# drscotthawley/flocoder

Measured on AMD Instinct MI355X. Metric: latent samples/sec (64-step Euler, SD-VAE 4x32x32), higher is better.
Workload: dtype f32; 1 GPU; flowers_sd.yaml shape: 64-step legacy Euler, batch 64 per GPU, latents 4x32x32, U-Net dim=32 dim_mults [1,2,4,8] n_classes=102, class-conditional, no CFG, ODE loop only (no VAE decode); global_batch=64, parallelism=sample-shard x1, weights broadcast once, plan_entries_per_forward=59, kernel_launches_per_forward=68, kernel_launches_per_euler_step=66, plan=exclusive device (cross-workgroup Block tails)

## Files before the change

### flocoder_amd/_binding.py

```python
from __future__ import annotations

import ctypes as C
import os
from typing import Optional

_HERE = os.path.dirname(os.path.abspath(__file__))
LIB_PATH = os.environ.get("FLOCODER_AMD_LIB") or os.path.join(_HERE, "_lib", "libflocoder_amd.so")

FC_OK, FC_E_ARG, FC_E_SHAPE, FC_E_ARCH, FC_E_HIP, FC_E_STATE = 0, -1, -2, -3, -4, -5
FC_METHOD_EULER, FC_METHOD_RK4 = 0, 1
FC_JACOBIAN_IDENTITY, FC_JACOBIAN_EXACT = 0, 1
FC_SDE_EULER_MARUYAMA, FC_SDE_HEUN = 0, 1
FC_LL_MAX_PROBES = 64
FC_PROBE_RADEMACHER, FC_PROBE_GAUSSIAN = 0, 1
FC_HIST_LDS_BINS = 8192
TILE_AUTO = -1
TILES = {"M128N32": 0, "M128N64": 1, "M64N32K2": 2, "M32N32K4": 3, "M64N64K2": 4, "M256N64": 5}


class fc_unet_config(C.Structure):
    _fields_ = [("dim", C.c_int), ("channels", C.c_int), ("n_levels", C.c_int), ("dim_mults", C.c_int * 8),
                ("groups", C.c_int), ("n_classes", C.c_int), ("mask_cond", C.c_int)]


_vp, _i, _f, _i64 = C.c_void_p, C.c_int, C.c_float, C.c_int64
_pi, _pf = C.POINTER(C.c_int), C.POINTER(C.c_float)

SIGNATURES = {
    "fc_abi_version": (_i, []),
    "fc_last_error": (C.c_char_p, []),
    "fc_check_device": (_i, [_i]),
    "fc_unet_create": (_i, [C.POINTER(fc_unet_config), _i, C.POINTER(_vp)]),
    "fc_unet_destroy": (None, [_vp]),
    "fc_unet_param_count": (_i, [_vp]),
    "fc_unet_param_info": (_i, [_vp, _i, C.POINTER(C.c_char_p), C.POINTER(_i64 * 4), C.POINTER(_i64)]),
    "fc_unet_param_numel": (_i64, [_vp]),
    "fc_unet_load_params": (_i, [_vp, _vp, _i64, _i, _vp]),
    "fc_unet_reserve": (_i, [_vp, _i, _i, _i]),
    "fc_unet_reserved": (_i, [_vp, _pi, _pi, _pi]),
    "fc_unet_forward": (_i, [_vp, _vp, _vp, _vp, _vp, _i, _vp, _i, _i, _i, _vp]),
    "fc_unet_integrate": (_i, [_vp, _i, _vp, _i, _i, _i, _pf, _i, _f, _f, _vp, _f, _vp, _i, _vp]),
    "fc_unet_integrate_rk45": (_i, [_vp, _vp, _i, _i, _i, C.c_double, C.c_double, C.c_double, C.c_double, _f, _vp, _f, _vp, _i, _pi, _vp]),
    "fc_unet_integrate_rk45_per_sample": (_i, [_vp, _vp, _i, _i, _i, C.c_double, C.c_double, C.c_double, C.c_double, _f, _vp, _f, _vp, _i,
                                              _pi, _vp]),
    "fc_unet_integrate_rk45_dense": (_i, [_vp, _i, _vp, _i, _i, _i, C.c_double, C.c_double, C.c_double, C.c_double, _f, _vp, _f, _vp, _i,
                                         C.POINTER(C.c_double), _i, _vp, _pi, _vp]),
    "fc_unet_chains": (_i, [_vp, _pi]),
    "fc_unet_plan_launches": (_i, [_vp]),
    "fc_unet_flops_per_sample": (C.c_double, [_vp]),
    "fc_unet_op_info": (_i, [_vp, _i, C.POINTER(C.c_char_p), C.POINTER(C.c_char_p), C.POINTER(C.c_double)]),
    "fc_unet_profile_ops": (_i, [_vp, _i, _i, _pf, _i, _vp]),
    "fc_unet_set_time_freqs": (_i, [_vp, _pf, _i]),
    "fc_unet_debug_tensor": (_i, [_vp, C.c_char_p, C.POINTER(_vp), _pi, _pi, _pi]),
    "fc_debug_copy": (_i, [_vp, _vp, _i64, _vp]),
    "fc_debug_set_poison": (_i, [_i]),
    "fc_debug_poison_check": (_i, [_pi, _pi]),
    "fc_debug_set_conv_stamps": (_i, [_vp]),
    "fc_debug_set_stamp_op": (_i, [_i, _vp]),
    "fc_debug_conv_routes": (_i, [_i]),
    "fc_debug_conv_routes_read": (_i, [C.c_char_p, _i]),
    "fc_debug_conv": (_i, [_vp, _i, _vp, _i, _vp, _vp, _vp, _vp, _vp, _i, _pi, _pf, _i, _i, _i, _i, _i, _i, _i, _i, _i, _i, _i, _pf, _vp]),
    "fc_debug_set_fused_tail": (_i, [_i]),
    "fc_unet_fused_tail_errors": (_i, [_vp, C.POINTER(_i)]),
    "fc_unet_set_shared": (_i, [_vp, _i]),
    "fc_unet_meeting_launches": (_i, [_vp]),
    "fc_unet_check": (_i, [_vp, _vp, _i]),
    "fc_debug_unet_break_meeting": (_i, [_vp]),
    "fc_debug_unet_break_meeting_kind": (_i, [_vp, _i]),
    "fc_unet_train_reserve": (_i, [_vp, _i, _i, _i]),
    "fc_unet_backward": (_i, [_vp, _vp, _vp, _vp, _vp, _vp, _i64, _i, _i, _i, _vp]),
    "fc_unet_backward_ex": (_i, [_vp, _vp, _vp, _vp, _vp, _i, _vp, _vp, _i64, _vp, _vp, _i, _i, _i, _vp]),
    "fc_unet_backward_parts": (_i, [_vp, _vp, _vp, _vp, _vp, _i, _vp, _vp, _i64, _vp, _vp, _i, _i, _i, _i, _i, _vp]),
    "fc_unet_backward_accumulate": (_i, [_vp, _vp, _vp, _vp, _vp, _i, _vp, _vp, _i64, _vp, _vp, _i, _i, _i, _i, _i, _vp]),
    "fc_unet_grad_buckets": (_i, [_vp, C.POINTER(_i64)]),
    "fc_unet_set_grad_buckets": (_i, [_vp, _i]),
    "fc_unet_backward_launches": (_i, [_vp]),
    "fc_unet_backward_op_info": (_i, [_vp, _i, C.POINTER(C.c_char_p), C.POINTER(C.c_char_p)]),
    "fc_unet_vjp_x": (_i, [_vp, _vp, _vp, _vp, _vp, _i, _vp, _vp, _i, _i, _i, _vp]),
    "fc_unet_vjp_launches": (_i, [_vp]),
    "fc_unet_train_form": (_i, [_vp]),
    "fc_unet_train_release": (_i, [_vp]),
    "fc_unet_vjp_op_info": (_i, [_vp, _i, C.POINTER(C.c_char_p), C.POINTER(C.c_char_p)]),
    "fc_unet_log_likelihood": (_i, [_vp, _vp, _i, _i, _i, _pf, _i, _f, _vp, _vp, _i, _vp, _vp, _vp, _vp]),
    "fc_unet_log_likelihood_rk45": (_i, [_vp, _vp, _i, _i, _i, C.c_double, C.c_double, C.c_double, C.c_double, _f, _vp, _vp, _i, _vp, _i, _vp,
                                         _vp, _pi, _vp]),
    "fc_unet_log_likelihood_probes": (_i, [_vp, _vp, _i, _i, _i, _pf, _i, _f, _vp, _vp, _i, _vp, _i, _vp, _vp, _vp, _vp, _vp]),
    "fc_unet_log_likelihood_rk45_probes": (_i, [_vp, _vp, _i, _i, _i, C.c_double, C.c_double, C.c_double, C.c_double, _f, _vp, _vp, _i, _vp,
                                                _i, _i, _vp, _vp, _vp, _vp, _pi, _vp]),
    "fc_ode_probe_field": (_i, [_vp, _i, C.c_uint64, _i64, _vp, _i, _i64, _vp]),
    "fc_debug_probe_dot": (_i, [_vp, _vp, _vp, _i, _i64, _vp]),
    "fc_unet_integrate_guided": (_i, [_vp, _vp, _i, _i, _i, _pf, _i, _f, _vp, _f, _vp, _i, _vp, _vp, _f, _f, _i, _vp]),
    "fc_ode_guided_correct": (_i, [_vp, _vp, _vp, _vp, _i64, _f, _f, _f, _vp, _vp]),
    "fc_unet_integrate_sde": (_i, [_vp, _i, _vp, _i, _i, _i, _pf, _i, _f, _vp, _f, _vp, _i, _f, C.c_uint64, _vp, _vp, _vp]),
    "fc_ode_normal_field": (_i, [_vp, C.c_uint64, _i64, _vp, _i, _i64, _vp]),
    "fc_inpaint_masks": (_i, [_vp, _vp, C.c_uint64, _vp, _i, _i, _i, _pi, C.POINTER(C.c_double), _i, _i, _vp]),
    "fc_note_confusion": (_i, [_vp, _i, _vp, _i, _vp, _i, _i, _i, _f, C.c_double, _i, C.c_double, _i, _i, _vp, _vp, _vp, _vp, _vp]),
    "fc_index_histogram": (_i, [_vp, _i64, _i, _i, _vp, _vp, _vp, _vp]),
    "fc_debug_unet_guided_buffers": (_i, [_vp, C.POINTER(_vp), C.POINTER(_vp), C.POINTER(_vp), C.POINTER(_vp)]),
    "fc_unet_arena_serial": (C.c_uint64, [_vp]),
    "fc_unet_class_param_range": (_i, [_vp, C.POINTER(_i64), C.POINTER(_i64)]),
    "fc_flow_interp": (_i, [_vp, _vp, _vp, _vp, _vp, _i, _i64, _vp]),
    "fc_flow_prepare": (_i, [_vp, _vp, _vp, _vp, _f, _f, _f, _vp, _i, _vp, _vp, _vp, _vp, _vp, _i, _i64, _vp]),
    "fc_flow_prepare_rows": (_i, [_vp, _vp, _vp, _vp, _f, _f, _f, _vp, _i, _vp, _vp, _vp, _vp, _vp, _i, _i, _i, _i64, _vp]),
    "fc_mse_loss_grad_scaled": (_i, [_vp, _vp, _vp, _vp, _vp, _i64, _f, _vp]),
    "fc_mse_loss_grad": (_i, [_vp, _vp, _vp, _vp, _vp, _i64, _vp]),
    "fc_grad_clip_coef": (_i, [_vp, _i64, _vp, _i64, C.c_float, _vp, _vp, _vp]),
    "fc_adam_ema_step": (_i, [_vp, _vp, _vp, _vp, _vp, _i64, _vp, C.c_float, C.c_float, C.c_float, C.c_float, _i, C.c_float, _i, _vp]),
    "fc_adam_ema_step_guarded": (_i, [_vp, _vp, _vp, _vp, _vp, _i64, _vp, C.c_float, C.c_float, C.c_float, C.c_float, _i, C.c_float, _i, _vp, _vp]),
    "fc_debug_conv_wgrad": (_i, [_vp, _i, _vp, _i, _vp, _i, _i, _i, _i, _i, _i, _i, _i, _vp, _vp, _vp]),
    "fc_vae_create": (_i, [_i, C.POINTER(_vp)]),
    "fc_vae_destroy": (None, [_vp]),
    "fc_vae_param_count": (_i, [_vp]),
    "fc_vae_param_numel": (_i64, [_vp]),
    "fc_vae_param_info": (_i, [_vp, _i, C.POINTER(C.c_char_p), C.POINTER(_i64 * 4), C.POINTER(_i64)]),
    "fc_vae_load_params": (_i, [_vp, _vp, _i64, _i, _vp]),
    "fc_vae_reserve_encode": (_i, [_vp, _i, _i, _i]),
    "fc_vae_reserve_decode": (_i, [_vp, _i, _i, _i]),
    "fc_vae_encode": (_i, [_vp, _vp, _vp, _i, _i, _i, _vp]),
    "fc_vae_decode": (_i, [_vp, _vp, _vp, _i, _i, _i, _vp]),
    "fc_vae_flops_per_sample": (C.c_double, [_vp, _i]),
    "fc_vae_plan_launches": (_i, [_vp, _i]),
    "fc_vqvae_create": (_i, [_i, _i, _i, _i, _i, _i, _i, C.POINTER(_vp)]),
    "fc_vqvae_create_ex": (_i, [_i, _i, _i, _i, _i, _i, _i, _i, C.POINTER(_vp)]),
    "fc_na2d": (_i, [_vp, _vp, _vp, _i, _i, _i, _i, _i, _i, _i, _vp]),
    "fc_vqvae_destroy": (None, [_vp]),
    "fc_vqvae_param_count": (_i, [_vp]),
    "fc_vqvae_param_numel": (_i64, [_vp]),
    "fc_vqvae_param_info": (_i, [_vp, _i, C.POINTER(C.c_char_p), C.POINTER(_i64 * 4), C.POINTER(_i64)]),
    "fc_vqvae_load_params": (_i, [_vp, _vp, _i64, _i, _vp]),
    "fc_vqvae_reserve_encode": (_i, [_vp, _i, _i, _i]),
    "fc_vqvae_reserve_decode": (_i, [_vp, _i, _i, _i]),
    "fc_vqvae_encode": (_i, [_vp, _vp, _vp, _i, _i, _i, _vp]),
    "fc_vqvae_decode": (_i, [_vp, _vp, _vp, _i, _i, _i, _vp]),
    "fc_vqvae_flops_per_sample": (C.c_double, [_vp, _i]),
    "fc_vae_op_info": (_i, [_vp, _i, _i, C.POINTER(C.c_char_p), C.POINTER(C.c_char_p), C.POINTER(C.c_double)]),
    "fc_vae_set_precision": (_i, [_vp, _i]),
    "fc_vqvae_set_precision": (_i, [_vp, _i]),
    "fc_vae_debug_taps": (_i, [_vp, _i]),
    "fc_vae_debug_tensor": (_i, [_vp, _i, C.c_char_p, C.POINTER(_vp), _pi, _pi, _pi]),
    "fc_vqvae_debug_taps": (_i, [_vp, _i]),
    "fc_vqvae_debug_tensor": (_i, [_vp, _i, C.c_char_p, C.POINTER(_vp), _pi, _pi, _pi]),
    "fc_debug_set_conv_precision": (_i, [_i]),
    "fc_vae_op_bytes": (_i, [_vp, _i, _i, C.POINTER(C.c_double), C.POINTER(C.c_double)]),
# ... 68 lines not shown
```

### flocoder_amd/csrc/common.h

```cpp
#pragma once
#include <hip/hip_runtime.h>
#include <stdint.h>
#include <string>
#include <vector>

#include "../../include/flocoder_amd.h"

namespace fc {

void set_error(const std::string& msg);
int fail(int code, const std::string& msg);

#define FC_HIP(expr)                                                                              \
    do {                                                                                          \
        hipError_t _e = (expr);                                                                   \
        if (_e != hipSuccess)                                                                     \
            return ::fc::fail(FC_E_HIP, std::string(#expr) + ": " + hipGetErrorString(_e));       \
    } while (0)

#define FC_TRY(expr)                \
    do {                            \
        int _r = (expr);            \
        if (_r != FC_OK) return _r; \
    } while (0)
// ... 99 lines not shown
    float* y = nullptr;
    float* stats_out = nullptr;
    int B = 0, HW = 0, C = 0;
};
int finalize_blocks_per_sample(int HW, int C);
int finalize_launch(const FinalizeArgs& a, hipStream_t s);
size_t finalize_lds_bytes(const FinalizeArgs& a);
int finalize_table_launch(const FinalizeArgs* jobs_dev, const int* bps_dev, const int2* blocks_dev, int nblocks, size_t lds_bytes, hipStream_t s);
int gn_stats_launch(const float* x_nhwc, float* stats , int B, int HW, int C, int G, hipStream_t s);
int gn_fold_launch(const float* in, float* out, int B, int G, int T, float n_t, hipStream_t s);

struct CondFetch {
    const float* all = nullptr;
    const int* evalc = nullptr;
    float* dst = nullptr;
    int n4 = 0;
};

int init_conv_launch(const CondFetch& fetch, const float* x_nchw, int x_batch_mod, const float* w , const float* bias, float* out_nhwc,
                     int B, int Cin, int HW, int Cout, hipStream_t s);
struct EulerTail {
    int* evalc = nullptr;
    float* y = nullptr;
    float dt = 0.f;
    int* step = nullptr;
    const float* ts = nullptr;
    float t_scale = 1.f;
    float* sc = nullptr;
    float* tvec = nullptr;
    int rows = 0;
};
int final_conv_launch(const float* x_nhwc, const float* w , const float* bias, float* out_nchw, int B, int Cin,
                      int HW, int Cout, const EulerTail& tail, hipStream_t s);
int nchw_to_nhwc_launch(const float* src, float* dst, int B, int C, int HW, int Cpad, int src_batch_mod, hipStream_t s);
int nhwc_to_nchw_launch(const float* src, float* dst, int B, int C, int HW, int Cpad, hipStream_t s);
int pixel_shuffle2_nhwc_launch(const float* src, float* dst, int B, int H, int W, int C, hipStream_t s);
int bilinear_nhwc_launch(const float* src, float* dst, int B, int C, int Hs, int Ws, int Hd, int Wd, hipStream_t s);

struct TembArgs {
    const float* time = nullptr;
    const int64_t* class_ids = nullptr;
    int class_batch_mod = 0;
    int null_from = 0;
    int rows_per_eval = 0;
    const float* freqs = nullptr;
    const float *w1t, *b1, *w2t, *b2;
    const float *emb, *cw1t, *cb1, *cw2t, *cb2;
    int n_classes = 0;
    float* t_out = nullptr;
    int B = 0, dim = 0, td = 0;
};
int temb_init();
int temb_launch(const TembArgs& a, float* h, float* c1, hipStream_t s);
int ss_launch(const float* t, const float* wt, const float* bias, float* ss, int B, int td, int S, hipStream_t s);

int linattn_ctx_launch(const float* qkv, float* ctx , int B, int n, int heads, hipStream_t s);
int linattn_apply_launch(const float* qkv, const float* ctx, float* out , int B, int n, int heads,
                         hipStream_t s);
struct LaArgs {
    const float* x = nullptr;
    SrcXform xf;
    const float* wqkv = nullptr;
    const float* wout = nullptr;
    const float* wqkv4 = nullptr;
    const float* bout = nullptr;
    float* ctx = nullptr;
    float* y = nullptr;
    float* stats_out = nullptr;
    int B = 0, n = 0, C = 0, heads = 4;
    const float* g2 = nullptr;
    const float* b2 = nullptr;
    float eps2 = 1e-5f;
    float* out = nullptr;
    float* part = nullptr;
    unsigned long long* gran = nullptr;
    unsigned* sync = nullptr;
    int* err = nullptr;
};
int linattn_fused_init();
bool linattn_fused_supported(int n, int C, int heads);
int linattn_fused_tiles(int n);
float linattn_fused_nt(int n, int C);
int linattn_fused_launch(const LaArgs& a, hipStream_t s);
bool linattn_fused_meeting_ok(int B, int n, int C);
int linattn_sample_init();
bool linattn_sample_supported(int n, int C, int heads);
int linattn_sample_launch(const LaArgs& a, hipStream_t s);
bool attn_sample_supported(int n, int C, int heads);
int attn_sample_launch(const LaArgs& a, hipStream_t s);
int rope_attn_launch(const float* x, const float* wq, const float* bq, const float* wk, const float* bk, const float* wv, const float* bv,
                     const float* wo, const float* bo, float* out, int B, int n, int C, int Cr, hipStream_t s);
int attn_small_launch(const float* qkv, float* out, int B, int n, int heads, hipStream_t s);

int na2d_launch(const float* qkv, float* out, const float* gamma, int B, int H, int W, int C, int heads, int ksize, int mode, hipStream_t s);

int ode_all_times_launch(const float* ts, int n_steps, int rk4 , float t_scale, float* tv_out, hipStream_t s);
int ode_time_launch(int* step, const float* ts, float t_scale, int rk4, float* sc, float* tvec, int rows, hipStream_t s);
int ode_euler_update_launch(float* x, const float* v2, int n, int cfg_on, float cfg, float dt, hipStream_t s);
struct Rk4Guide { const float *gsc, *xin, *ym, *keep, *q; int tcur; };
int ode_rk4_stage_launch(const float* sc, const float* y, float* xs, float* k_out, const float* v2, int n, int cfg_on, float cfg,
                         int full, int tsel, float t_scale, float* tvec, int rows, const Rk4Guide* g, hipStream_t s);
int ode_rk4_final_launch(const float* sc, float* y, const float* k1, const float* k2, const float* k3, const float* v2, int n,
                         int cfg_on, float cfg, const Rk4Guide* g, hipStream_t s);
int ode_guide_w_launch(const float* sc, const float* gsc, const float* v, const float* xin, const float* ym, const float* keep, float* w,
                       int n, int tcur, hipStream_t s);
int ode_guided_correct_launch(const float* v, const float* x, const float* ym, const float* keep, float* out, int n, float t, float s2,
                              float gamma, hipStream_t s);
int ode_ll_stage_launch(const float* sc, const float* y, float* xs, float* k_out, const float* v, const float* g, const float* eps,
                        double* dst, int slot, int B, int m, int full, int tsel, float t_scale, float* tvec, int K, hipStream_t s);
int ode_ll_final_launch(const float* sc, float* y, const float* k1, const float* k2, const float* k3, const float* v, const float* g,
                        const float* eps, const double* dst, double* a, int B, int m, int K, hipStream_t s);
int ode_ll_logp_launch(const float* z, const double* a, double* logp, int B, int m, hipStream_t s);
int ode_ll_dot_launch(const float* eps, const float* g, double* out, double* dk, int B, int m, int K, hipStream_t s);
int ode_ll_mean_launch(const double* ak, int K, int B, double* abar, double* se, int mean_given, hipStream_t s);
int ode_probe_normal_field_launch(float* out, unsigned long long seed, unsigned probe, const int64_t* sids, int n, int m, hipStream_t s);
int ode_rademacher_field_launch(float* out, unsigned long long seed, unsigned probe, const int64_t* sids, int n, int m, hipStream_t s);
struct SdeParams { unsigned long long seed; const float* noise; };
int ode_sde_update_launch(const int* step, const float* ts, const SdeParams* prm, const int64_t* sids, float* y, float* xs, float* b1,
                          const float* v2, int n, int m, int cfg_on, float cfg, float sigma, int stage, int use_noise, float t_scale,
                          float* tvec, int rows, hipStream_t s);
int ode_normal_field_launch(float* out, unsigned long long seed, unsigned draw, const int64_t* sids, int n, int m, hipStream_t s);
int ode_iota_launch(int64_t* ids, int B, hipStream_t s);

struct Rk45State {
    double t, t_new, t_bound, dir, h, h_abs, rtol, atol, h0, d1, err, t_old;
    int nfev, accepted, rejected, attempts, done, failed, step_rejected, accepted_last, max_attempts, ev_cursor, ev_first, ev_end;
};
struct Rk45K { float* k[7]; };
struct Rk45Eval { float* frames; int n_eval, pad; };
__host__ __device__ inline const double* rk45_eval_times(const Rk45Eval* ev) { return reinterpret_cast<const double*>(ev + 1); }
struct Rk45Status { int unfinished, failed, pad0, pad1; };
struct Rk45Groups { int G, spg, m, chunks; };
struct Rk45LL { double *a, *d; int B; int K = 1; double *dk = nullptr, *ak = nullptr; };
int rk45_chunks(int m, int cap);
int rk45_setup_launch(const Rk45Groups& g, const float* x, double* y, float* xs, Rk45State* st, double t0, double t1, double rtol,
                      double atol, int max_attempts, float t_scale, float* tvec, int cfg_on, hipStream_t s);
int rk45_d01_launch(const Rk45Groups& g, const Rk45State* st, const double* y, float* k0, const float* v2, int cfg_on, float cfg,
                    double* part, hipStream_t s);
int rk45_h0_launch(const Rk45Groups& g, Rk45State* st, const double* part, float t_scale, float* tvec, int cfg_on, const Rk45LL* ll,
                   hipStream_t s);
int rk45_y1_launch(const Rk45Groups& g, const Rk45State* st, const double* y, const float* k0, float* xs, hipStream_t s);
int rk45_d2_launch(const Rk45Groups& g, const Rk45State* st, const double* y, const float* k0, const float* v2, int cfg_on, float cfg,
                   double* part, hipStream_t s);
int rk45_h1_launch(const Rk45Groups& g, Rk45State* st, const double* part, const Rk45LL* ll, hipStream_t s);
int rk45_stage_launch(const Rk45Groups& g, const Rk45State* st, int stage, const double* y, Rk45K kk, const float* v2, int cfg_on,
                      float cfg, float* xs, float t_scale, float* tvec, hipStream_t s);
int rk45_finish_launch(const Rk45Groups& g, const Rk45State* st, const double* y, double* y_new, Rk45K kk, const float* v2, int cfg_on,
                       float cfg, float* xs, float t_scale, float* tvec, hipStream_t s);
int rk45_error_launch(const Rk45Groups& g, const Rk45State* st, const double* y, const double* y_new, Rk45K kk, const float* v2,
                      int cfg_on, float cfg, double* part, hipStream_t s);
int rk45_control_launch(const Rk45Groups& g, Rk45State* st, const double* part, const Rk45Eval* ev, const Rk45LL* ll, hipStream_t s);
int rk45_dense_launch(const Rk45Groups& g, const Rk45State* st, const Rk45Eval* ev, const double* y, Rk45K kk, hipStream_t s);
int rk45_commit_launch(const Rk45Groups& g, const Rk45State* st, double* y, const double* y_new, float* k0, const float* k6,
                       hipStream_t s);
int rk45_status_launch(const Rk45Groups& g, const Rk45State* st, Rk45Status* out, hipStream_t s);
int rk45_out_launch(const double* y, float* x, int n, hipStream_t s);

struct PackJob { const float* src; float* dst; int kind, a, b, c, d, e; size_t total; };
constexpr int kPackPerBlock = 4096;
struct PackTable {
    PackJob* jobs = nullptr;
    int2* blocks = nullptr;
    int nblocks = 0;
    void release();
};
int pack_conv_launch(const float* oihw, float* dst , int O, int I, int KH, int KW, hipStream_t s);
// ... 105 lines not shown
```

### flocoder_amd/csrc/conv_dev.h

```cpp
#pragma once
#include "common.h"

namespace fc {

typedef float f32x16 __attribute__((ext_vector_type(16)));
typedef __attribute__((address_space(1))) unsigned long long gu64;
typedef __attribute__((address_space(1))) unsigned gu32;

struct ConvDev {
    ConvArgs a;
    int TWl, THl, TB, PH, PW, P;
    int tiles_x, tiles_y, ntiles, nblocks;
    int cpg, cpgt, NPG, rps;
    int gsz, o_fin;
    int fin_local;
    int act0, act1, any_xf;
    int o_pixoff, o_pixtb, o_gstat, o_aff, o_patch, o_wl, o_wres, o_red, o_part;
    int txl, tyl;
    unsigned magic_nt;
    int loader_prio;
    int o_out;
    int o_epoch, o_gran;
    const float* zeros16;
    int patch_stride, wl_stride;
    int nchunks, nwb;
    unsigned magic_phw, magic_pw;
    unsigned long long* stamps;
    int bf3;
};

__device__ __forceinline__ void conv_stamp(const ConvDev& p, int slot) {
    if (p.stamps) {
        const unsigned long long t = __builtin_amdgcn_s_memtime();
        if ((threadIdx.x & 63) == 0 && (threadIdx.x >> 6) < 8) {
            p.stamps[((size_t)blockIdx.x * 8 + (threadIdx.x >> 6)) * 16 + slot] = t;
            if (slot == 0) p.stamps[((size_t)blockIdx.x * 8 + (threadIdx.x >> 6)) * 16 + 15] = __builtin_amdgcn_s_memrealtime();
        }
    }
}

struct TileInfo { int BM, BN, CC, WK, MTNT, WMWN; };

__device__ __forceinline__ int fastdiv(int x, unsigned magic) { return magic ? (int)__umulhi((unsigned)x, magic) : x; }

__device__ __forceinline__ float silu_f(float z) { return z / (1.0f + __expf(-z)); }
__device__ __forceinline__ void lds_only_barrier() { asm volatile("s_waitcnt lgkmcnt(0)\n\ts_barrier" ::: "memory"); }

__device__ __forceinline__ int xcd_remap(int bid, int nwg) {
    const int q = nwg >> 3, r = nwg & 7, xcd = bid & 7;
    return (xcd < r ? xcd * (q + 1) : r * (q + 1) + (xcd - r) * q) + (bid >> 3);
}
__device__ __forceinline__ int conv_parity_select(ConvDev& p, int bid) {
    if (!p.a.par4) return bid;
    const int nb1 = p.nblocks >> 2, par = bid >= 2 * nb1 ? (bid >= 3 * nb1 ? 3 : 2) : (bid >= nb1 ? 1 : 0);
    p.a.w += (size_t)par * 4 * p.a.Cin * p.a.Cout;
    if (p.a.w_b3) p.a.w_b3 += (size_t)par * 4 * (16 * p.nchunks) * p.a.Cout;
    p.a.pad_y = 1 - (par >> 1); p.a.pad_x = 1 - (par & 1);
    p.a.out_oy = par >> 1; p.a.out_ox = par & 1;
    p.a.stats_toff = par;
    return bid - par * nb1;
}


template <class T>
__device__ __forceinline__ T* as_global(T* q) {
    typedef __attribute__((address_space(1))) T* gp;
    return (T*)(gp)(size_t)q;
}
__device__ __forceinline__ void conv_params_from_lanes(ConvDev& p) {
    constexpr int ND = (int)(sizeof(ConvDev) / 4);
    static_assert(sizeof(ConvDev) % 4 == 0 && ND <= 256, "ConvDev must fit four lane-loads");
    const unsigned* ka = (const unsigned*)as_global((const unsigned*)__builtin_amdgcn_kernarg_segment_ptr());
    const int lane = threadIdx.x & 63;
    unsigned w[(ND + 63) / 64];
#pragma unroll
    for (int j = 0; j < (ND + 63) / 64; ++j) w[j] = (64 * j + lane < ND) ? ka[64 * j + lane] : 0u;
    unsigned* d = reinterpret_cast<unsigned*>(&p);
#pragma unroll
    for (int i = 0; i < ND; ++i) d[i] = __builtin_amdgcn_readlane(w[i / 64], i % 64);
    ConvArgs& a = p.a;
    a.s0.p = as_global(a.s0.p); a.s0.xf.stats = as_global(a.s0.xf.stats); a.s0.xf.gamma = as_global(a.s0.xf.gamma);
    a.s0.xf.beta = as_global(a.s0.xf.beta); a.s0.xf.ss = as_global(a.s0.xf.ss);
    a.s1.p = as_global(a.s1.p); a.s1.xf.stats = as_global(a.s1.xf.stats); a.s1.xf.gamma = as_global(a.s1.xf.gamma);
    a.s1.xf.beta = as_global(a.s1.xf.beta); a.s1.xf.ss = as_global(a.s1.xf.ss);
    a.w4 = as_global(a.w4); a.res_w4 = as_global(a.res_w4);
    a.w = as_global(a.w); a.bias = as_global(a.bias); a.out = as_global(a.out); a.add = as_global(a.add);
    a.stats_out = as_global(a.stats_out); a.res_w = as_global(a.res_w); a.res_b = as_global(a.res_b); a.res_out = as_global(a.res_out);
    a.fin.gamma = as_global(a.fin.gamma); a.fin.beta = as_global(a.fin.beta); a.fin.res = as_global(a.fin.res);
    a.fin.gn1_out = as_global(a.fin.gn1_out); a.fin.sync = as_global(a.fin.sync); a.fin.gran = as_global(a.fin.gran); a.fin.err = as_global(a.fin.err);
    p.zeros16 = as_global(p.zeros16); p.stamps = as_global(p.stamps);
}

constexpr int FL_FIN = 1, FL_RES = 2, FL_POST = 4, FL_XF = 8, FL_CAT = 16, FL_STAMP = 32, FL_STATS = 64, FL_GN1 = 128, FL_POSTOP = 256,
              FL_NARROW = 512, FL_MULTI = 1024, FL_MEET = 2048, FL_ALL = 4095, FL_W4 = 4096;
constexpr int FL_WW = 8192;
constexpr int GEO_PAIR = 1, GEO_FAST = 2;
constexpr int geo_log2(int v) { return v <= 1 ? 0 : 1 + geo_log2(v >> 1); }
constexpr int geo_key(int form, int TB, int TW, int cpg, int Tst) { return form | ((TB == 2 ? 1 : 0) << 2) | (geo_log2(TW) << 3) | (geo_log2(cpg) << 6) | (Tst << 10); }
constexpr int geo_form(int k) { return k & 3; }
constexpr int geo_TB(int k) { return 1 + ((k >> 2) & 1); }
constexpr int geo_TWl(int k) { return (k >> 3) & 7; }
constexpr int geo_cpg(int k) { return 1 << ((k >> 6) & 15); }
constexpr int geo_Tst(int k) { return (k >> 10) & 63; }

template <int WM, int WN, int WK, int MT, int NT, int FL = FL_ALL, int GEO = 0>
__device__ __forceinline__ void conv_epilogue(const ConvDev& p, f32x16 (&acc)[MT][NT], f32x16 (&accr)[MT][NT], float* smem, int tid, int lane,
                                              int wave, int b0, int y0, int x0, int n0, int tx, int ty, bool active = true,
                                              int nthr = 256, const float* pre = nullptr, bool staged_dead = false) {
    constexpr int BM = 32 * MT * WM, BN = 32 * NT * WN;
    const ConvArgs& a = p.a;
    const int half = lane >> 5, l31 = lane & 31;
    const int wk = wave % WK, wn = (wave / WK) % WN, wm = wave / (WK * WN);
    constexpr bool GEOC = GEO != 0;
    static_assert(!GEOC || (FL != FL_ALL && (FL & FL_FIN) && (FL & FL_STATS) && !(FL & (FL_MULTI | FL_POST | FL_RES))), "a geometry key belongs to a lean Block-closing flavour");
    static_assert(!GEOC || (geo_Tst(GEO) >= 1 && geo_TB(GEO) * (geo_cpg(GEO) >= BN ? 1 : BN / geo_cpg(GEO)) * geo_Tst(GEO) * 2 <= 512), "one granule per thread");
    const int g_TB = GEOC ? geo_TB(GEO) : p.TB;
    const int g_TWl = GEOC ? geo_TWl(GEO) : p.TWl;
    const int g_tbsh = GEOC ? geo_log2(BM / geo_TB(GEO)) : p.TWl + p.THl;
    const int g_THl = GEOC ? geo_log2(BM / geo_TB(GEO)) - geo_TWl(GEO) : p.THl;
    const int g_rps = GEOC ? BM / geo_TB(GEO) : p.rps;
    const int g_cpg = GEOC ? geo_cpg(GEO) : p.cpg;
    const int g_cpgt = GEOC ? (geo_cpg(GEO) < BN ? geo_cpg(GEO) : BN) : p.cpgt;
    const int g_NPG = GEOC ? (geo_cpg(GEO) >= BN ? geo_cpg(GEO) / BN : 1) : p.NPG;
    const int g_mt = GEOC ? (geo_TB(GEO) > 1 ? 1 : geo_Tst(GEO) / (geo_cpg(GEO) >= BN ? geo_cpg(GEO) / BN : 1)) : (p.TB > 1 ? 1 : p.tiles_x * p.tiles_y);
    const int TW = 1 << g_TWl, TH = 1 << g_THl, Cout = a.Cout;
    constexpr bool LEAN = FL != FL_ALL;
    const bool has_res = LEAN ? bool(FL & FL_RES) : a.res_out != nullptr;
    const bool stats_post = (FL & FL_POST) && a.stats_post;
    if (WK > 1) {
        if (!staged_dead) __syncthreads();
        float* red = smem + p.o_red;
        constexpr int TILE = 16 * 64;
        const int slot = ((wm * WN + wn) * (WK - 1) + (wk - 1)) * MT * NT * (has_res ? 2 : 1);
        if (active && wk > 0) {
#pragma unroll
            for (int mt = 0; mt < MT; ++mt)
#pragma unroll
                for (int nt = 0; nt < NT; ++nt) {
                    float* d = red + (size_t)(slot + mt * NT + nt) * TILE + lane;
#pragma unroll
                    for (int r = 0; r < 16; ++r) d[r * 64] = acc[mt][nt][r];
                    if (has_res) {
                        float* dr = red + (size_t)(slot + MT * NT + mt * NT + nt) * TILE + lane;
#pragma unroll
                        for (int r = 0; r < 16; ++r) dr[r * 64] = accr[mt][nt][r];
                    }
                }
        }
        __syncthreads();
        if (active && wk == 0) {
            for (int k2 = 1; k2 < WK; ++k2) {
                const int sl = ((wm * WN + wn) * (WK - 1) + (k2 - 1)) * MT * NT * (has_res ? 2 : 1);
#pragma unroll
                for (int mt = 0; mt < MT; ++mt)
#pragma unroll
                    for (int nt = 0; nt < NT; ++nt) {
                        const float* d = red + (size_t)(sl + mt * NT + nt) * TILE + lane;
#pragma unroll
                        for (int r = 0; r < 16; ++r) acc[mt][nt][r] += d[r * 64];
                        if (has_res) {
                            const float* dr = red + (size_t)(sl + MT * NT + mt * NT + nt) * TILE + lane;
#pragma unroll
                            for (int r = 0; r < 16; ++r) accr[mt][nt][r] += dr[r * 64];
                        }
                    }
            }
        }
    }

    auto pix_of = [&](int mt, int r) {
        const int m = (wm * MT + mt) * 32 + (r & 3) + 8 * (r >> 2) + 4 * half;
        const int tw = m & (TW - 1), th = (m >> g_TWl) & (TH - 1), tb = m >> g_tbsh;
        const int b = b0 + tb;
        return b < a.B ? (b * (a.H << a.out_sh) + ((y0 + th) << a.out_sh) + a.out_oy) * (a.W << a.out_sh) + ((x0 + tw) << a.out_sh) + a.out_ox : -1;
    };
    if (FL & FL_STAMP) conv_stamp(p, 6);
    const bool owner = active && (wk == 0);
    const bool fin = LEAN ? bool(FL & FL_FIN) : a.fin.gamma != nullptr;
    const bool meeting = LEAN ? bool(FL & FL_MEET) : (fin && !p.fin_local);
    const unsigned epoch = meeting ? __float_as_uint(smem[p.o_epoch]) : 0u;
    float* partS = smem + p.o_part;
    float* partQ = partS + (BM / 16) * BN;
    const bool do_stats = LEAN ? bool(FL & FL_STATS) : a.stats_out != nullptr;
    if (do_stats && !staged_dead) __syncthreads();

    auto block_sums = [&]() {
        if (owner) {
#pragma unroll
            for (int mt = 0; mt < MT; ++mt)
#pragma unroll
                for (int nt = 0; nt < NT; ++nt) {
                    const int ncol = (wn * NT + nt) * 32 + l31;
#pragma unroll
                    for (int hh = 0; hh < 2; ++hh) {
                        float s = 0.f, q = 0.f;
#pragma unroll
                        for (int r = 8 * hh; r < 8 * hh + 8; ++r) { const float v = acc[mt][nt][r]; s += v; q += v * v; }
                        s += __shfl_xor(s, 32);
                        q += __shfl_xor(q, 32);
                        if (half == 0) {
                            const int hb = (wm * MT + mt) * 2 + hh;
                            partS[hb * BN + ncol] = s;
                            partQ[hb * BN + ncol] = q;
                        }
                    }
                }
        }
    };
    auto publish = [&](float* dst, int G, int cpg, int cpgt, int NPG, bool coherent, bool ltab_on, int tb, int gl, float s, float q, bool whole = false) {
        const int b = b0 + tb;
        const float n = (float)(g_rps * cpgt), mean = s / n;
        const int g = whole ? 0 : n0 / cpg + (cpg >= BN ? 0 : gl);
        const int nsub = whole ? n0 / BN : ((cpg >= BN) ? (n0 % cpg) / BN : 0);
        const int msub = (g_TB > 1) ? 0 : ty * p.tiles_x + tx;
        const int T = g_mt * NPG;
        float* d = dst + (((size_t)(b * G + g) * a.stats_tmul + a.stats_toff) * T + msub * NPG + nsub) * 2;
        if (ltab_on) {
            float* ltab = smem + p.o_fin;
            const int ngt = cpg >= BN ? 1 : BN / cpg;
            ltab[2 * (tb * ngt + gl)] = mean;
            ltab[2 * (tb * ngt + gl) + 1] = 1.0f / sqrtf((q - s * mean) / n + a.fin.eps);
        }
        if (coherent) {
            gu64* gp = (gu64*)(a.fin.gran + (size_t)(d - dst));
            const unsigned long long tag = (unsigned long long)epoch << 32;
            __hip_atomic_store(gp, tag | __float_as_uint(mean), __ATOMIC_RELAXED, __HIP_MEMORY_SCOPE_AGENT);
            __hip_atomic_store(gp + 1, tag | __float_as_uint(q - s * mean), __ATOMIC_RELAXED, __HIP_MEMORY_SCOPE_AGENT);
        } else {
            d[0] = mean;
            d[1] = q - s * mean;
        }
    };
    auto emit = [&](float* dst, int G, int cpg, int cpgt, int NPG, bool coherent, bool ltab) {
        const int hb_per = p.rps >> 4;
        const int ncols = min(BN, Cout - n0);
        for (int i0 = 0; i0 < p.TB * BN; i0 += nthr) {
            const int i = i0 + tid;
            const bool live = i < p.TB * BN;
            const int tb = live ? i / BN : 0, col = live ? i - tb * BN : 0;
            float s = 0.f, q = 0.f;
            if (live) {
#pragma unroll 8
                for (int h = 0; h < hb_per; ++h) { s += partS[(tb * hb_per + h) * BN + col]; q += partQ[(tb * hb_per + h) * BN + col]; }
            }
            for (int o = cpgt >> 1; o > 0; o >>= 1) { s += __shfl_xor(s, o); q += __shfl_xor(q, o); }
            if (live && (col & (cpgt - 1)) == 0 && col < ncols && b0 + tb < a.B) publish(dst, G, cpg, cpgt, NPG, coherent, ltab, tb, col / cpgt, s, q);
        }
    };
    auto stats_fast = [&](float* dst, int G, int cpg, int cpgt, int NPG, bool coherent, bool ltab, bool whole = false) {
        const int lanes = cpgt < 32 ? cpgt : 32;
        const int per = cpgt <= 32 ? 1 : cpgt / 32;
        if (owner) {
            float sv[NT], qv[NT];
#pragma unroll
            for (int nt = 0; nt < NT; ++nt) {
                float s_ = 0.f, q_ = 0.f;
// ... 181 lines not shown
        }
        if ((FL & FL_STAMP) && active) conv_stamp(p, 2);
        if (LEAN ? bool(FL & FL_GN1) : a.fin.gn1_out != nullptr) {
            lds_only_barrier();
            const int cpg1 = Cout, cpgt1 = GEOC ? BN : (Cout < BN ? Cout : BN), NPG1 = GEOC ? p.ntiles : (Cout >= BN ? Cout / BN : 1);
            if (pair_stats) stats_pair(a.fin.gn1_out, 1, cpg1, cpgt1, NPG1, false, false, GEOC);
            else if (fast_stats) stats_fast(a.fin.gn1_out, 1, cpg1, cpgt1, NPG1, false, false, GEOC);
            else {
                block_sums();
                lds_only_barrier();
                emit(a.fin.gn1_out, 1, cpg1, cpgt1, NPG1, false, false);
            }
        }
        if ((FL & FL_STAMP) && active) conv_stamp(p, 13);
    }

    const bool post = !stats_post && !fin;
    const bool act = (FL & FL_POSTOP) && post && a.out_act;
    const float* addp = ((FL & FL_POSTOP) && post) ? a.add : nullptr;
    if (owner) {
#pragma unroll
        for (int mt = 0; mt < MT; ++mt) {
            int pix[16];
#pragma unroll
            for (int r = 0; r < 16; ++r) pix[r] = pix_of(mt, r);
#pragma unroll
            for (int nt = 0; nt < NT; ++nt) {
                const int ncol = (wn * NT + nt) * 32 + l31, n = n0 + ncol;
                if (n >= Cout) continue;
                float* op = a.out + n;
                if (addp) {
                    float ad[16];
#pragma unroll
                    for (int r = 0; r < 16; ++r) ad[r] = pix[r] >= 0 ? addp[(size_t)pix[r] * Cout + n] : 0.f;
#pragma unroll
                    for (int r = 0; r < 16; ++r) acc[mt][nt][r] = (act ? silu_f(acc[mt][nt][r]) : acc[mt][nt][r]) + ad[r];
                } else if (act) {
#pragma unroll
                    for (int r = 0; r < 16; ++r) acc[mt][nt][r] = silu_f(acc[mt][nt][r]);
                }
                if (!LEAN && p.o_out < 0) {
#pragma unroll
                    for (int r = 0; r < 16; ++r)
                        if (pix[r] >= 0) op[(size_t)pix[r] * Cout] = acc[mt][nt][r];
                    if (has_res) {
                        const float rbias = pre ? pre[NT + nt] : (a.res_b ? a.res_b[n] : 0.f);
                        float* rp = a.res_out + n;
#pragma unroll
                        for (int r = 0; r < 16; ++r)
                            if (pix[r] >= 0) rp[(size_t)pix[r] * Cout] = accr[mt][nt][r] + rbias;
                    }
                }
            }
        }
    }
    if ((FL & FL_STAMP) && active) conv_stamp(p, 3);
    if (LEAN || p.o_out >= 0) {
        constexpr int OS = BN + 4, Q4 = BN / 4;
        float* ot = smem + p.o_out;
        for (int pass = 0; pass < (has_res ? 2 : 1); ++pass) {
            if (pass) lds_only_barrier();
            if (owner) {
#pragma unroll
                for (int mt = 0; mt < MT; ++mt)
#pragma unroll
                    for (int nt = 0; nt < NT; ++nt) {
                        const int ncol = (wn * NT + nt) * 32 + l31;
                        const float rbias = pass ? (pre ? pre[NT + nt] : ((a.res_b && n0 + ncol < Cout) ? a.res_b[n0 + ncol] : 0.f)) : 0.f;
#pragma unroll
                        for (int r = 0; r < 16; ++r) {
                            const int m = (wm * MT + mt) * 32 + (r & 3) + 8 * (r >> 2) + 4 * half;
                            ot[m * OS + ncol] = pass ? accr[mt][nt][r] + rbias : acc[mt][nt][r];
                        }
                    }
            }
            if (active && !pass) conv_stamp(p, 9);
            lds_only_barrier();
            if (active && !pass) conv_stamp(p, 10);
            float* gout = pass ? a.res_out : a.out;
            for (int i = tid; i < BM * Q4; i += nthr) {
                const int m = i / Q4, c4 = (i - m * Q4) * 4, n = n0 + c4;
                const int tw = m & (TW - 1), th = (m >> g_TWl) & (TH - 1), tb = m >> g_tbsh;
                const int b = b0 + tb;
                if (b < a.B && n < Cout) {
                    const float4 v = *reinterpret_cast<const float4*>(ot + m * OS + c4);
                    *reinterpret_cast<float4*>(gout + (size_t)((b * (a.H << a.out_sh) + ((y0 + th) << a.out_sh) + a.out_oy) * (a.W << a.out_sh) + ((x0 + tw) << a.out_sh) + a.out_ox) * Cout + n) = v;
                }
            }
        }
    }
    if (FL & FL_STAMP) conv_stamp(p, 8);
}

int conv_pipe_launch(const ConvDev& d, int tile, int grid, size_t lds, hipStream_t s);
int conv_pipe_blocks_per_cu(const ConvDev& d, int tile, size_t lds);
int conv_pipe_init();
bool conv_pipe_supports_ks(int ks);
const float* conv_zeros16();

}
```

### flocoder_amd/csrc/conv_pipe.hip

```cpp
#include <cstdlib>
#include <map>
#include <mutex>
#include <string>
#include <tuple>
#include "conv_dev.h"
#include "stats_dev.h"

namespace fc {

typedef __attribute__((address_space(3))) void* lptr_t;

__device__ __forceinline__ void lds_dma16(const float* gsrc, unsigned lds_byte) {
    const unsigned dst = __builtin_amdgcn_readfirstlane(lds_byte);
    unsigned keep;
    asm volatile("s_mov_b32 %0, m0\n\ts_mov_b32 m0, %2\n\ts_nop 0\n\tglobal_load_lds_dwordx4 %1, off\n\ts_mov_b32 m0, %0"
                 : "=&s"(keep) : "v"(gsrc), "s"(dst) : "memory");
}
typedef float f32x4 __attribute__((ext_vector_type(4)));
__device__ __forceinline__ void hidden_load16(f32x4& dst, const float* gsrc) {
    asm volatile("global_load_dwordx4 %0, %1, off" : "=v"(dst) : "v"(gsrc) : "memory");
}
__device__ __forceinline__ void wait_vmcnt(int n) {
    switch (__builtin_amdgcn_readfirstlane(n)) {
        case 0: asm volatile("s_waitcnt vmcnt(0)" ::: "memory"); break;
        case 1: asm volatile("s_waitcnt vmcnt(1)" ::: "memory"); break;
        case 2: asm volatile("s_waitcnt vmcnt(2)" ::: "memory"); break;
        case 3: asm volatile("s_waitcnt vmcnt(3)" ::: "memory"); break;
        case 4: asm volatile("s_waitcnt vmcnt(4)" ::: "memory"); break;
        case 5: asm volatile("s_waitcnt vmcnt(5)" ::: "memory"); break;
        case 6: asm volatile("s_waitcnt vmcnt(6)" ::: "memory"); break;
        case 7: asm volatile("s_waitcnt vmcnt(7)" ::: "memory"); break;
        case 8: asm volatile("s_waitcnt vmcnt(8)" ::: "memory"); break;
        case 9: asm volatile("s_waitcnt vmcnt(9)" ::: "memory"); break;
        case 10: asm volatile("s_waitcnt vmcnt(10)" ::: "memory"); break;
        case 11: asm volatile("s_waitcnt vmcnt(11)" ::: "memory"); break;
        case 12: asm volatile("s_waitcnt vmcnt(12)" ::: "memory"); break;
        case 13: asm volatile("s_waitcnt vmcnt(13)" ::: "memory"); break;
        case 14: asm volatile("s_waitcnt vmcnt(14)" ::: "memory"); break;
        case 15: asm volatile("s_waitcnt vmcnt(15)" ::: "memory"); break;
        case 16: asm volatile("s_waitcnt vmcnt(16)" ::: "memory"); break;
        case 17: asm volatile("s_waitcnt vmcnt(17)" ::: "memory"); break;
        case 18: asm volatile("s_waitcnt vmcnt(18)" ::: "memory"); break;
        case 19: asm volatile("s_waitcnt vmcnt(19)" ::: "memory"); break;
        case 20: asm volatile("s_waitcnt vmcnt(20)" ::: "memory"); break;
        default: asm volatile("s_waitcnt vmcnt(0)" ::: "memory"); break;
    }
    __builtin_amdgcn_sched_barrier(0);
}
__device__ __forceinline__ void loader_handover() {
    asm volatile("s_waitcnt lgkmcnt(0)\n\ts_barrier" ::: "memory");
}

typedef __bf16 bf16x8_t __attribute__((ext_vector_type(8)));
typedef __bf16 bf16x2_t __attribute__((ext_vector_type(2)));
typedef float f32x2_t __attribute__((ext_vector_type(2)));

__device__ __forceinline__ void split_bf16x4(const f32x4& x, uint2& hi, uint2& lo) {
    union { bf16x2_t p; unsigned u; } H0, H1, L0, L1;
    f32x2_t a; a[0] = x.x; a[1] = x.y;
    f32x2_t b; b[0] = x.z; b[1] = x.w;
    H0.p = __builtin_convertvector(a, bf16x2_t);
    H1.p = __builtin_convertvector(b, bf16x2_t);
    f32x2_t ra; ra[0] = x.x - __uint_as_float(H0.u << 16); ra[1] = x.y - __uint_as_float(H0.u & 0xffff0000u);
    f32x2_t rb; rb[0] = x.z - __uint_as_float(H1.u << 16); rb[1] = x.w - __uint_as_float(H1.u & 0xffff0000u);
    L0.p = __builtin_convertvector(ra, bf16x2_t);
    L1.p = __builtin_convertvector(rb, bf16x2_t);
    hi = make_uint2(H0.u, H1.u); lo = make_uint2(L0.u, L1.u);
}

constexpr int kFinGeomGroups = 4, kWWSlots = 8;

template <int WM, int WN, int WK, int MT, int NT, int CC, int NPL, int KS, int NL, int FL = FL_ALL, int PREC = 0, int GEO = 0>
__global__ void __launch_bounds__(256 + 64 * NL) conv_pipe_kernel(const ConvDev p_kernarg) {
    ConvDev p;
    conv_params_from_lanes(p);
    constexpr int NTHR = 256 + 64 * NL, LT = 64 * NL;
    constexpr int BN = 32 * NT * WN, KSTEPS = CC / 2, KPW = KSTEPS / WK, Q = CC / 4, PIXSTEP = LT / Q, KK = KS * KS;
    static_assert(WM * WN * WK == 4, "4 consumer waves per workgroup");
    constexpr bool DB = (WM * WN == 1 && MT == 1 && NT == 1 && KS == 3);
    constexpr bool DB4 = DB && (FL & FL_W4) != 0;
#ifndef FC_DB4_CHAINS
#define FC_DB4_CHAINS 2
#endif
    constexpr int DB4_CHAINS = FC_DB4_CHAINS;
    constexpr bool WW = (FL & FL_WW) != 0;
    static_assert(!WW || (DB4 && FL != FL_ALL && (FL & FL_FIN) && (FL & FL_XF) && !(FL & (FL_CAT | FL_RES))), "whole-window staging: register-fed Block-closing flavours");
    constexpr bool BF3 = PREC == 1;
    static_assert(!BF3 || (!DB && CC == 16 && FL == FL_ALL), "split-bf16: LDS-fed tiles, one 16-channel k-step per chunk, the all-in-one flavour");
    constexpr int CS = (DB4 || BF3) ? CC + 4 : CC + 1;
    extern __shared__ __attribute__((aligned(16))) float smem[];
    const ConvArgs& a = p.a;
    float* gstat = smem + p.o_gstat;
    float2* aff = reinterpret_cast<float2*>(smem + p.o_aff);
    float* patch0 = smem + p.o_patch;
    float* wl0 = smem + p.o_wl;
    const unsigned smem_lds = (unsigned)(size_t)(lptr_t)smem;

    const int tid = threadIdx.x, lane = tid & 63, wave8 = tid >> 6;
    const bool consumer = wave8 < 4;
    const int wave = wave8 & 3;
    const int lw = (wave8 - 4) & (NL - 1), ltid = (tid - 256) & (LT - 1);
    const int half = lane >> 5, l31 = lane & 31;
    const int wk = wave % WK, wn = (wave / WK) % WN, wm = wave / (WK * WN);

    const int bid = conv_parity_select(p, xcd_remap(blockIdx.x, p.nblocks));
    const int mt_i = p.ntiles == 1 ? bid : (p.magic_nt ? (int)__umulhi((unsigned)bid, p.magic_nt) : bid / p.ntiles);
    const int nt_i = bid - mt_i * p.ntiles;
    const int tx = mt_i & (p.tiles_x - 1), ty = (mt_i >> p.txl) & (p.tiles_y - 1), bg = mt_i >> (p.txl + p.tyl);
    constexpr bool GEOC = GEO != 0;
    constexpr int BM = 32 * MT * WM;
    static_assert(!GEOC || (!(FL & FL_CAT) && (FL & FL_XF) && geo_Tst(GEO) <= kPartPre), "geometry flavours: transform loader, one source");
    const int g_TB = GEOC ? geo_TB(GEO) : p.TB;
    const int g_TWl = GEOC ? geo_TWl(GEO) : p.TWl;
    const int g_tbsh = GEOC ? geo_log2(BM / geo_TB(GEO)) : p.TWl + p.THl;
    const int g_THl = GEOC ? geo_log2(BM / geo_TB(GEO)) - geo_TWl(GEO) : p.THl;
    const int TW = 1 << g_TWl, TH = 1 << g_THl;
    const int b0 = bg * g_TB, y0 = ty * TH, x0 = tx * TW, n0 = nt_i * BN;
    const int PW = p.PW, PHW = p.PH * p.PW;
    const int C0 = a.s0.C, C1 = a.s1.C, Cin = a.Cin, Cout = a.Cout;
    constexpr bool LEAN = FL != FL_ALL;
    const bool has_res = LEAN ? bool(FL & FL_RES) : a.res_out != nullptr;
    const bool xf_on = LEAN ? bool(FL & FL_XF) : p.any_xf != 0;
    const int nchunks = p.nchunks;
    if (FL & FL_STAMP) conv_stamp(p, 0);
    const bool meet = LEAN ? bool(FL & FL_MEET) : (a.fin.gamma != nullptr && !p.fin_local);
    unsigned arrival = 0;
    if (meet && tid == 0) {
        const gu32* cnt = (const gu32*)(a.fin.sync + b0 / g_TB);
        asm volatile("global_atomic_add %0, %1, %2, off sc0" : "=v"(arrival) : "v"(cnt), "v"(1u) : "memory");
    }

    auto gn_tables = [&](const bool worker, const int id, const int nthr) {
      if (xf_on) {
        const int G0 = a.s0.xf.mode ? a.s0.xf.G : 0, G1 = ((FL & FL_CAT) && a.s1.xf.mode) ? a.s1.xf.G : 0;
        float pg = 1.f, pbt = 0.f, psc = 0.f, psh = 0.f;
        bool p_on = false, p_ss = false;
        int p_gs = 0;
       if (worker) {
        if (id < g_TB * Cin) {
            const int tb = GEOC ? ((geo_TB(GEO) > 1 && id >= Cin) ? 1 : 0) : id / Cin, c = id - tb * Cin, b = b0 + tb;
            const bool first = !(FL & FL_CAT) || c < C0;
            const SrcXform& xf = first ? a.s0.xf : a.s1.xf;
            if (b < a.B && xf.mode) {
                const int cs = first ? c : c - C0, Cs = first ? C0 : C1;
                p_on = true;
                p_gs = 2 * ((first ? 0 : p.TB * G0) + tb * xf.G + (GEOC ? cs / geo_cpg(GEO) : cs / (Cs / xf.G)));
                pg = xf.gamma[cs];
                pbt = xf.beta[cs];
                if (xf.ss) {
                    p_ss = true;
                    psc = xf.ss[(size_t)b * xf.ss_stride + cs];
                    psh = xf.ss[(size_t)b * xf.ss_stride + Cs + cs];
                }
            }
        }
        for (int i = id; i < g_TB * (G0 + G1); i += nthr) {
            const bool first = !(FL & FL_CAT) || i < p.TB * G0;
            const SrcXform& xf = first ? a.s0.xf : a.s1.xf;
            const int j = first ? i : i - p.TB * G0;
            const int tb = GEOC ? ((geo_TB(GEO) > 1 && j >= xf.G) ? 1 : 0) : j / xf.G, g = j - tb * xf.G, b = b0 + tb;
            float mean = 0.f, rstd = 0.f;
            if (b < a.B) {
                if constexpr (GEOC) combine_partials_fixed<geo_Tst(GEO)>(xf, b, g, &mean, &rstd);
                else combine_partials(xf, b, g, &mean, &rstd);
            }
            gstat[2 * i] = mean;
            gstat[2 * i + 1] = rstd;
            if (GEOC) break;
        }
       }
        if ((FL & FL_STAMP) && worker) conv_stamp(p, 2);
        lds_only_barrier();
        if ((FL & FL_STAMP) && worker) conv_stamp(p, 4);
       if (worker) {
        if (id < g_TB * Cin) {
            float A = 1.f, Bv = 0.f;
            if (p_on) {
                A = gstat[p_gs + 1] * pg;
                Bv = pbt - gstat[p_gs] * A;
                if (p_ss) {
                    const float sc = psc + 1.0f;
                    A *= sc;
                    Bv = Bv * sc + psh;
                }
            }
            aff[id] = make_float2(A, Bv);
        }
        if (!GEOC)
        for (int i = id + nthr; i < p.TB * Cin; i += nthr) {
            const int tb = i / Cin, c = i - tb * Cin, b = b0 + tb;
            float A = 1.f, Bv = 0.f;
            const bool first = !(FL & FL_CAT) || c < C0;
            const SrcXform& xf = first ? a.s0.xf : a.s1.xf;
            if (b < a.B && xf.mode) {
                const int cs = first ? c : c - C0, Cs = first ? C0 : C1;
                const float* gs = gstat + 2 * ((first ? 0 : p.TB * G0) + tb * xf.G + cs / (Cs / xf.G));
                A = gs[1] * xf.gamma[cs];
                Bv = xf.beta[cs] - gs[0] * A;
                if (xf.ss) {
                    const float sc = xf.ss[(size_t)b * xf.ss_stride + cs] + 1.0f;
                    A *= sc;
// ... 22 lines not shown
    if (consumer) {
#pragma unroll
        for (int nt = 0; nt < NT; ++nt) {
            const int n = n0 + (wn * NT + nt) * 32 + l31;
            if (n < Cout) {
                if (a.bias) pre[nt] = a.bias[n];
                if (has_res && a.res_b) pre[NT + nt] = a.res_b[n];
                if (a.fin.gamma) { pre[2 * NT + nt] = a.fin.gamma[n]; pre[3 * NT + nt] = a.fin.beta[n]; }
            }
        }
    }

    constexpr int WW_CQ = GEOC ? geo_cpg(GEO) * kFinGeomGroups / 4 : 0, WW_PW = GEOC ? (1 << geo_TWl(GEO)) + 2 : 0;
    constexpr int WW_PHW = GEOC ? (BM / geo_TB(GEO) / (1 << geo_TWl(GEO)) + 2) * WW_PW : 0, WW_E = GEOC ? geo_TB(GEO) * WW_PHW * WW_CQ : 0;
    constexpr int WWK = !WW ? 1 : (GEOC ? (WW_E + NTHR - 1) / NTHR : kWWSlots);
    f32x4 wv[WWK];
    int w_lds[WWK], w_aff[WWK];
    const int ww_cq = GEOC ? WW_CQ : Cin >> 2, ww_pw = GEOC ? WW_PW : PW, ww_phw = GEOC ? WW_PHW : PHW, ww_E = GEOC ? WW_E : p.P * (Cin >> 2);
    const int ww_nk = GEOC ? WWK : __builtin_amdgcn_readfirstlane((ww_E + NTHR - 1) / NTHR);
    auto ww_request = [&]() {
        const int Hin = a.Hs << a.ups, Win = a.Ws << a.ups;
        const float rcq = __builtin_amdgcn_rcpf((float)ww_cq);
#pragma unroll
        for (int k = 0; k < WWK; ++k) {
            if (!GEOC && k >= ww_nk) break;
            const int e = tid + k * NTHR;
            w_lds[k] = -1; w_aff[k] = -1;
            const float* src = p.zeros16;
            if (e < ww_E) {
                const int pix = GEOC ? e / ww_cq : (int)(((float)e + 0.5f) * rcq), cq = e - pix * ww_cq;
                const int tb = GEOC ? pix / ww_phw : fastdiv(pix, p.magic_phw), r = pix - tb * ww_phw;
                const int py = GEOC ? r / ww_pw : fastdiv(r, p.magic_pw), px = r - py * ww_pw;
                const int iy = y0 * a.stride - (a.pad_y >= 0 ? a.pad_y : a.pad) + py, ix = x0 * a.stride - (a.pad_x >= 0 ? a.pad_x : a.pad) + px, b = b0 + tb;
                if (b < a.B && iy >= 0 && iy < Hin && ix >= 0 && ix < Win) {
                    src = a.s0.p + (size_t)((b * a.Hs + (iy >> a.ups)) * a.Ws + (ix >> a.ups)) * C0 + 4 * cq;
                    w_aff[k] = tb * Cin + 4 * cq;
                }
                w_lds[k] = (cq >> 3) * p.patch_stride + pix * CS + 8 * ((cq & 7) >> 1) + 2 * (cq & 1);
            }
            wv[k] = *reinterpret_cast<const f32x4*>(src);
        }
    };
    auto ww_store = [&]() {
#pragma unroll
        for (int k = 0; k < WWK; ++k) {
            if (!GEOC && k >= ww_nk) break;
            if (w_lds[k] < 0) continue;
            f32x4 x = wv[k];
            if (w_aff[k] >= 0) {
                const float2* ab = aff + w_aff[k];
                x.x = ab[0].x * x.x + ab[0].y; x.y = ab[1].x * x.y + ab[1].y;
                x.z = ab[2].x * x.z + ab[2].y; x.w = ab[3].x * x.w + ab[3].y;
                if (p.act0) { x.x = silu_f(x.x); x.y = silu_f(x.y); x.z = silu_f(x.z); x.w = silu_f(x.w); }
            }
            float* d = patch0 + w_lds[k];
            d[0] = x.x; d[1] = x.z; d[4] = x.y; d[5] = x.w;
        }
    };

    if (!consumer) {
      if constexpr (WW) {
        ww_request();
        if (FL & FL_STAMP) conv_stamp(p, 1);
        gn_tables(true, ltid, LT);
        ww_store();
        if (FL & FL_STAMP) conv_stamp(p, 3);
        loader_handover();
      } else {
        {
            const int lp = __builtin_amdgcn_readfirstlane(p.loader_prio);
            if (lp == 1) __builtin_amdgcn_s_setprio(1);
            else if (lp == 2) __builtin_amdgcn_s_setprio(2);
            else if (lp == 3) __builtin_amdgcn_s_setprio(3);
        }
        const float* wbase = a.w + (size_t)b0 * a.w_batch_stride;
        const int q4 = (ltid % Q) * 4;
        int e_po[NPL], e_lds[NPL], e_tb[NPL];
        {
            const int Hin = a.Hs << a.ups, Win = a.Ws << a.ups;
#pragma unroll
            for (int k = 0; k < NPL; ++k) {
                const int pix = ltid / Q + k * PIXSTEP;
                e_po[k] = -1; e_lds[k] = -1; e_tb[k] = 0;
                if (pix < p.P) {
                    const int tb = fastdiv(pix, p.magic_phw), r = pix - tb * PHW, py = fastdiv(r, p.magic_pw), px = r - py * PW;
                    const int iy = y0 * a.stride - (a.pad_y >= 0 ? a.pad_y : a.pad) + py, ix = x0 * a.stride - (a.pad_x >= 0 ? a.pad_x : a.pad) + px, b = b0 + tb;
                    if (b < a.B && iy >= 0 && iy < Hin && ix >= 0 && ix < Win) e_po[k] = (b * a.Hs + (iy >> a.ups)) * a.Ws + (ix >> a.ups);
                    e_lds[k] = pix * CS + (DB4 ? 8 * ((ltid % Q) >> 1) + 2 * ((ltid % Q) & 1) : q4);
                    e_tb[k] = tb;
                }
            }
        }
        if (FL & FL_STAMP) conv_stamp(p, 1);
        const int nwb = p.nwb;
        constexpr int MAXP = ((KK + 1) * CC * BN / 256 + NL - 1) / NL;
        const int rows_main = KK * CC, npieces = (rows_main + (has_res ? CC : 0)) * BN / 256;
        const int my_pieces = __builtin_amdgcn_readfirstlane(npieces > lw ? (npieces - lw + NL - 1) / NL : 0);
        const float* d_ptr[MAXP];
        int d_row[MAXP];
#pragma unroll
        for (int m = 0; m < MAXP; ++m) {
            const int j = lw + NL * m, f = j * 256 + lane * 4, row = f / BN, n = n0 + (f % BN);
            if constexpr (BF3) {
                const int e = j * 64 + lane, r = e / BN, nn = n0 + e % BN, part = r / (2 * KK), tap = (r >> 1) % KK, c8l = r & 1;
                d_row[m] = 0;
                d_ptr[m] = (nn >= Cout || part > 1) ? nullptr
                         : a.w_b3 + (size_t)part * ((size_t)KK * nchunks * 8 * Cout) + ((size_t)(tap * 2 * nchunks + c8l) * Cout + nn) * 4;
                continue;
            }
            const bool res = row >= rows_main;
            d_row[m] = res ? row - rows_main : row % CC;
            d_ptr[m] = n >= Cout ? nullptr : (res ? a.res_w + (size_t)d_row[m] * Cout + n : wbase + ((size_t)(row / CC) * Cin + d_row[m]) * Cout + n);
        }
        auto dma_weights = [&](int i) {
            const int c0 = i * CC;
            const size_t adv = BF3 ? (size_t)i * 8 * Cout : (size_t)c0 * Cout;
            const unsigned wb = smem_lds + 4u * (unsigned)(p.o_wl + (i % nwb) * p.wl_stride + lw * 256);
            const bool tail = !BF3 && c0 + CC > Cin;
#pragma unroll
            for (int m = 0; m < MAXP; ++m) {
                if (m >= my_pieces) break;
                const bool ok = d_ptr[m] != nullptr && (!tail || c0 + d_row[m] < Cin);
                lds_dma16(ok ? d_ptr[m] + adv : p.zeros16, wb + 4u * (unsigned)(m * (NL * 256)));
            }
        };
        f32x4 pv[NPL];
        const int nk = __builtin_amdgcn_readfirstlane((p.P * Q + LT - 1) / LT);
        auto issue_patch = [&](int i, f32x4 (&pv)[NPL]) {
            const int c = i * CC + q4;
            const bool live = c < Cin, first = !(FL & FL_CAT) || c < C0;
            const float* base = first ? a.s0.p + c : a.s1.p + (c - C0);
            const int Cs = first ? C0 : C1;
#pragma unroll
            for (int k = 0; k < NPL; ++k) {
                if (k >= nk) break;
                hidden_load16(pv[k], (live && e_po[k] >= 0) ? base + (size_t)e_po[k] * Cs : p.zeros16);
            }
        };
        auto store_patch = [&](int i, f32x4 (&pv)[NPL]) {
            const int c = i * CC + q4;
            float* pb = patch0 + (i & 1) * p.patch_stride;
            const bool live = c < Cin, act = (c < C0) ? p.act0 : p.act1;
#pragma unroll
            for (int k = 0; k < NPL; ++k) {
                if (k >= nk) break;
                if (e_lds[k] < 0) continue;
                f32x4 x = pv[k];
                if (xf_on && live && e_po[k] >= 0) {
                    const float2* ab = aff + e_tb[k] * Cin + c;
                    x.x = ab[0].x * x.x + ab[0].y; x.y = ab[1].x * x.y + ab[1].y;
                    x.z = ab[2].x * x.z + ab[2].y; x.w = ab[3].x * x.w + ab[3].y;
                    if (act) { x.x = silu_f(x.x); x.y = silu_f(x.y); x.z = silu_f(x.z); x.w = silu_f(x.w); }
                }
                float* d = pb + e_lds[k];
                if (BF3) {
                    uint2 h2, l2;
                    split_bf16x4(x, h2, l2);
                    char* pc = reinterpret_cast<char*>(pb + (e_lds[k] - q4)) + 2 * q4;
                    *reinterpret_cast<uint2*>(pc) = h2;
                    *reinterpret_cast<uint2*>(pc + 2 * CC) = l2;
                }
                else if (DB4) { d[0] = x.x; d[1] = x.z; d[4] = x.y; d[5] = x.w; }
                else { d[0] = x.x; d[1] = x.y; d[2] = x.z; d[3] = x.w; }
            }
        };
        unsigned long long dbg_mem = 0, dbg_store = 0, dbg_bar = 0, dbg_issue = 0, dbg_dma = 0;
        if (!DB) {
            dma_weights(0);
            if (nwb == 3 && nchunks > 1) dma_weights(1);
        }
        {
            const int c = q4;
            const bool live = c < Cin, first = !(FL & FL_CAT) || c < C0;
            const float* base = first ? a.s0.p + c : a.s1.p + (c - C0);
            const int Cs = first ? C0 : C1;
#pragma unroll
            for (int k = 0; k < NPL; ++k) {
                if (k >= nk) break;
                pv[k] = *reinterpret_cast<const f32x4*>((live && e_po[k] >= 0) ? base + (size_t)e_po[k] * Cs : p.zeros16);
            }
        }
        gn_tables(true, ltid, LT);
        store_patch(0, pv);
        if (FL & FL_STAMP) conv_stamp(p, 3);
        __builtin_amdgcn_s_waitcnt(0x0F70);
        loader_handover();
        for (int g = 0; g < nchunks; ++g) {
            const bool next = g + 1 < nchunks;
            int ahead = 0;
            unsigned long long ta = ((FL & FL_STAMP) && p.stamps) ? __builtin_amdgcn_s_memtime() : 0ull;
            if (!DB && next && nwb == 2) dma_weights(g + 1);
            if (next) issue_patch(g + 1, pv);
            unsigned long long tb_ = ((FL & FL_STAMP) && p.stamps) ? __builtin_amdgcn_s_memtime() : 0ull;
            if (!DB && nwb == 3 && g + 2 < nchunks) { dma_weights(g + 2); ahead = my_pieces; }
            unsigned long long t0 = ((FL & FL_STAMP) && p.stamps) ? __builtin_amdgcn_s_memtime() : 0ull;
            if ((FL & FL_STAMP) && p.stamps) { dbg_issue += tb_ - ta; dbg_dma += t0 - tb_; }
            wait_vmcnt(ahead);
            unsigned long long t1 = ((FL & FL_STAMP) && p.stamps) ? __builtin_amdgcn_s_memtime() : 0ull;
            if (next) store_patch(g + 1, pv);
            unsigned long long t2 = ((FL & FL_STAMP) && p.stamps) ? __builtin_amdgcn_s_memtime() : 0ull;
            loader_handover();
            if ((FL & FL_STAMP) && p.stamps) { dbg_mem += t1 - t0; dbg_store += t2 - t1; dbg_bar += __builtin_amdgcn_s_memtime() - t2; }
        }
        if ((FL & FL_STAMP) && p.stamps && lane == 0) {
            unsigned long long* d = p.stamps + ((size_t)blockIdx.x * 8 + (wave8 < 8 ? wave8 : 7)) * 16;
            d[9] = dbg_mem; d[10] = dbg_store; d[11] = dbg_bar; d[12] = dbg_issue; d[13] = dbg_dma;
        }
        __builtin_amdgcn_s_setprio(0);
      }
    } else {
        int abase[MT];
#pragma unroll
        for (int mt = 0; mt < MT; ++mt) {
            const int m = (wm * MT + mt) * 32 + l31;
            const int tw = m & (TW - 1), th = (m >> g_TWl) & (TH - 1), tb = m >> g_tbsh;
            abase[mt] = (tb * PHW + th * a.stride * PW + tw * a.stride) * CS + half;
        }
        const int bbase = half * BN + wn * NT * 32 + l31;
        const int kk0 = wk * KPW;
        const int abase4 = abase[0] - half + 8 * wk + 4 * half;
        unsigned long long dbg_cbar = 0;
        constexpr int NB = (DB && !DB4) ? KK * KPW : 1, NR = (DB && !DB4) ? KPW : 1;
        float wcur[NB], wnxt[NB], rcur[NR], rnxt[NR];
        const int ncol = n0 + l31;
        const bool colok = ncol < Cout;
        const float* wq = colok ? a.w + (size_t)b0 * a.w_batch_stride + ncol : p.zeros16;
        const float* rq = (colok && has_res) ? a.res_w + ncol : p.zeros16;
        const size_t wcs = colok ? (size_t)Cout : 0, wts = colok ? (size_t)Cin * Cout : 0;
        auto fetch_w = [&](int i, float (&w)[NB], float (&r)[NR]) {
#pragma unroll
            for (int kk = 0; kk < KPW; ++kk) {
                int c = i * CC + 2 * (kk0 + kk) + half;
                c = c < Cin ? c : Cin - 1;
                const float* q = wq + (size_t)c * wcs;
#pragma unroll
                for (int tap = 0; tap < KK; ++tap) w[tap * KPW + kk] = q[(size_t)tap * wts];
                if (has_res) r[kk] = rq[(size_t)c * wcs];
            }
        };
        constexpr int NQ = DB4 ? KK : 1;
        f32x4 wA[NQ], wB[NQ], rA, rB;
        const unsigned lane_off4 = DB4 ? (unsigned)(half * Cout + ncol) * 4u : 0u;
        const int wk_u = __builtin_amdgcn_readfirstlane(wk);
        auto fetch4 = [&](int i, f32x4 (&w)[NQ], f32x4& r) {
            const size_t blk = (size_t)((i * (CC / 8) + wk_u) * 2) * (size_t)Cout * 4;
            const float* ub = a.w4 + blk;
#pragma unroll
            for (int tap = 0; tap < NQ; ++tap) w[tap] = *reinterpret_cast<const f32x4*>(ub + (size_t)tap * ((size_t)Cin * Cout) + lane_off4);
            if (has_res) r = *reinterpret_cast<const f32x4*>(a.res_w4 + blk + lane_off4);
        };
        if (DB4) fetch4(0, wA, rA);
        else if (DB) fetch_w(0, wcur, rcur);
        if constexpr (WW) ww_request();
        if (FL & FL_STAMP) conv_stamp(p, 1);
        gn_tables(false, 0, 1);
        if constexpr (WW) ww_store();
        if (meet && tid == 0) {
            asm volatile("s_waitcnt vmcnt(0)" : "+v"(arrival) :: "memory");
            smem[p.o_epoch] = __uint_as_float(arrival / (unsigned)p.gsz + 1u);
        }
        __syncthreads();
        if (FL & FL_STAMP) conv_stamp(p, 4);
        f32x16 acc2;
#pragma unroll
        for (int r = 0; r < 16; ++r) acc2[r] = 0.f;
        if constexpr (DB4) {
            auto chunk = [&](int i, f32x4 (&wc)[NQ], f32x4& rc, f32x4 (&wn)[NQ], f32x4& rn) {
                const float* patch = patch0 + (WW ? i : (i & 1)) * p.patch_stride;
                fetch4(i + 1 < nchunks ? i + 1 : i, wn, rn);
                __builtin_amdgcn_sched_barrier(0);
                static_assert(!DB4 || KPW == 4, "one 16-byte operand read = the four k-steps of a wave");
                (void)patch;
                const unsigned pl = smem_lds + 4u * (unsigned)(p.o_patch + (WW ? i : (i & 1)) * p.patch_stride + abase4);
                const unsigned prow = 4u * (unsigned)(PW * CS);
                auto lds_quad = [&](f32x4& dst, int tapn) {
                    const unsigned ad = pl + (unsigned)(tapn / KS) * prow;
                    switch (tapn % KS) {
                        case 0: asm volatile("ds_read_b128 %0, %1" : "=v"(dst) : "v"(ad) : "memory"); break;
                        case 1: asm volatile("ds_read_b128 %0, %1 offset:%2" : "=v"(dst) : "v"(ad), "n"(4 * CS) : "memory"); break;
                        default: asm volatile("ds_read_b128 %0, %1 offset:%2" : "=v"(dst) : "v"(ad), "n"(8 * CS) : "memory"); break;
                    }
                };
                f32x4 av, an;
                lds_quad(av, 0);
                asm volatile("s_waitcnt lgkmcnt(0)" : "+v"(av) :: "memory");
                an = av;
#pragma unroll
                for (int tap = 0; tap < KK; ++tap) {
                    if (tap + 1 < KK || has_res) lds_quad(an, tap + 1 < KK ? tap + 1 : KK / 2);
                    __builtin_amdgcn_sched_barrier(0);
                    if (DB4_CHAINS == 2) {
                        acc[0][0] = __builtin_amdgcn_mfma_f32_32x32x2f32(av[0], wc[tap][0], acc[0][0], 0, 0, 0);
                        acc2 = __builtin_amdgcn_mfma_f32_32x32x2f32(av[1], wc[tap][1], acc2, 0, 0, 0);
                        acc[0][0] = __builtin_amdgcn_mfma_f32_32x32x2f32(av[2], wc[tap][2], acc[0][0], 0, 0, 0);
                        acc2 = __builtin_amdgcn_mfma_f32_32x32x2f32(av[3], wc[tap][3], acc2, 0, 0, 0);
                    } else {
#pragma unroll
                        for (int kk = 0; kk < KPW; ++kk) acc[0][0] = __builtin_amdgcn_mfma_f32_32x32x2f32(av[kk], wc[tap][kk], acc[0][0], 0, 0, 0);
                    }
                    __builtin_amdgcn_sched_barrier(0);
                    if (tap + 1 < KK || has_res) asm volatile("s_waitcnt lgkmcnt(0)" : "+v"(an) :: "memory");
                    av = an;
                }
                if (has_res) {
#pragma unroll
                    for (int kk = 0; kk < KPW; ++kk) accr[0][0] = __builtin_amdgcn_mfma_f32_32x32x2f32(av[kk], rc[kk], accr[0][0], 0, 0, 0);
                }
                if constexpr (!WW) {
                unsigned long long t0 = ((FL & FL_STAMP) && p.stamps) ? __builtin_amdgcn_s_memtime() : 0ull;
                loader_handover();
                if ((FL & FL_STAMP) && p.stamps) dbg_cbar += __builtin_amdgcn_s_memtime() - t0;
                }
            };
            for (int i = 0; i < nchunks; i += 2) {
                chunk(i, wA, rA, wB, rB);
                if (i + 1 < nchunks) chunk(i + 1, wB, rB, wA, rA);
            }
            if (DB4_CHAINS == 2) {
#pragma unroll
                for (int r = 0; r < 16; ++r) acc[0][0][r] += acc2[r];
            }
        } else if constexpr (BF3) {
            int ab3[MT];
#pragma unroll
            for (int mt = 0; mt < MT; ++mt) ab3[mt] = abase[mt] - half + 4 * half;
            const int bb3 = 4 * (half * BN + wn * NT * 32 + l31);
            static_assert(CC == 16, "one k-step of sixteen channels per tap");
            typedef union { uint4 u; bf16x8_t v; } opnd_t;
            for (int i = 0; i < nchunks; ++i) {
                const float* patch = patch0 + (i & 1) * p.patch_stride;
                const float* wl = wl0 + (i % p.nwb) * p.wl_stride + bb3;
#pragma unroll
                for (int tap = 0; tap < KK; ++tap) {
                    const int tapoff = ((tap / KS) * PW + (tap % KS)) * CS;
                    opnd_t A[MT][2], Bq[NT][2];
#pragma unroll
                    for (int mt = 0; mt < MT; ++mt) {
                        const char* pc = reinterpret_cast<const char*>(patch + ab3[mt] + tapoff);
                        A[mt][0].u = *reinterpret_cast<const uint4*>(pc);
                        A[mt][1].u = *reinterpret_cast<const uint4*>(pc + 2 * CC);
                    }
#pragma unroll
                    for (int nt = 0; nt < NT; ++nt) {
                        Bq[nt][0].u = *reinterpret_cast<const uint4*>(wl + 4 * ((tap * 2) * BN + nt * 32));
                        Bq[nt][1].u = *reinterpret_cast<const uint4*>(wl + 4 * (((KK + tap) * 2) * BN + nt * 32));
                    }
#pragma unroll
                    for (int mt = 0; mt < MT; ++mt)
#pragma unroll
                        for (int nt = 0; nt < NT; ++nt) {
                            acc[mt][nt] = __builtin_amdgcn_mfma_f32_32x32x16_bf16(A[mt][1].v, Bq[nt][0].v, acc[mt][nt], 0, 0, 0);
                            acc[mt][nt] = __builtin_amdgcn_mfma_f32_32x32x16_bf16(A[mt][0].v, Bq[nt][1].v, acc[mt][nt], 0, 0, 0);
                            acc[mt][nt] = __builtin_amdgcn_mfma_f32_32x32x16_bf16(A[mt][0].v, Bq[nt][0].v, acc[mt][nt], 0, 0, 0);
                        }
                }
                __syncthreads();
            }
        } else {
        for (int i = 0; i < nchunks; ++i) {
            const float* patch = patch0 + (i & 1) * p.patch_stride;
            const float* wl = wl0 + (i % p.nwb) * p.wl_stride + bbase;
            if (DB && i + 1 < nchunks) fetch_w(i + 1, wnxt, rnxt);
#pragma unroll
            for (int tap = 0; tap < KK; ++tap) {
                const int tapoff = ((tap / KS) * PW + (tap % KS)) * CS;
#pragma unroll
                for (int kk = 0; kk < KPW; ++kk) {
                    const int k = 2 * (kk0 + kk);
                    float av[MT], bv[NT];
#pragma unroll
                    for (int mt = 0; mt < MT; ++mt) av[mt] = patch[abase[mt] + tapoff + k];
#pragma unroll
                    for (int nt = 0; nt < NT; ++nt) bv[nt] = DB ? wcur[tap * KPW + kk] : wl[(tap * CC + k) * BN + nt * 32];
#pragma unroll
                    for (int mt = 0; mt < MT; ++mt)
#pragma unroll
                        for (int nt = 0; nt < NT; ++nt)
                            acc[mt][nt] = __builtin_amdgcn_mfma_f32_32x32x2f32(av[mt], bv[nt], acc[mt][nt], 0, 0, 0);
                }
            }
            if (has_res) {
                const int tapoff = (a.pad * PW + a.pad) * CS;
#pragma unroll
                for (int kk = 0; kk < KPW; ++kk) {
                    const int k = 2 * (kk0 + kk);
                    float av[MT], bv[NT];
#pragma unroll
                    for (int mt = 0; mt < MT; ++mt) av[mt] = patch[abase[mt] + tapoff + k];
#pragma unroll
                    for (int nt = 0; nt < NT; ++nt) bv[nt] = DB ? rcur[kk] : wl[(KK * CC + k) * BN + nt * 32];
#pragma unroll
                    for (int mt = 0; mt < MT; ++mt)
#pragma unroll
                        for (int nt = 0; nt < NT; ++nt)
                            accr[mt][nt] = __builtin_amdgcn_mfma_f32_32x32x2f32(av[mt], bv[nt], accr[mt][nt], 0, 0, 0);
                }
            }
            unsigned long long t0 = ((FL & FL_STAMP) && p.stamps) ? __builtin_amdgcn_s_memtime() : 0ull;
            if (DB) {
                loader_handover();
#pragma unroll
                for (int j = 0; j < NB; ++j) wcur[j] = wnxt[j];
#pragma unroll
                for (int j = 0; j < NR; ++j) rcur[j] = rnxt[j];
            } else {
                __syncthreads();
            }
            if ((FL & FL_STAMP) && p.stamps) dbg_cbar += __builtin_amdgcn_s_memtime() - t0;
        }
        }
        if ((FL & FL_STAMP) && p.stamps && lane == 0) p.stamps[((size_t)blockIdx.x * 8 + wave8) * 16 + 11] = dbg_cbar;
        if (FL & FL_STAMP) conv_stamp(p, 5);
    }
    if constexpr (WW) loader_handover();
    conv_epilogue<WM, WN, WK, MT, NT, FL, GEO>(p, acc, accr, smem, tid, lane, wave, b0, y0, x0, n0, tx, ty, consumer, NTHR, pre, true);
}

static float* g_zeros16 = nullptr;
const float* conv_zeros16() { return g_zeros16; }

#define FC_PIPE_TILES(X, KS)               \
    X(TILE_M128N32, 4, 1, 1, 1, 1, 16, KS, 4)  \
    X(TILE_M128N64, 4, 1, 1, 1, 2, 16, KS, 4)  \
    X(TILE_M64N32K2, 2, 1, 2, 1, 1, 32, KS, (KS == 1 ? 4 : 8)) \
    X(TILE_M32N32K4, 1, 1, 4, 1, 1, 32, KS, (KS == 1 ? 4 : 8)) \
    X(TILE_M64N64K2, 2, 1, 2, 1, 2, 16, KS, 4) \
    X(TILE_M256N64, 4, 1, 1, 2, 2, 16, KS, 4)

template <int KS>
static int pipe_attr_ks() {
#define X(T, WM, WN, WK, MT, NT, CC, K, NL)                                                                               \
    FC_HIP(hipFuncSetAttribute(reinterpret_cast<const void*>(&conv_pipe_kernel<WM, WN, WK, MT, NT, CC, 8, K, NL>),        \
                               hipFuncAttributeMaxDynamicSharedMemorySize, 160 * 1024));
    FC_PIPE_TILES(X, KS)
#undef X
    return FC_OK;
}

#define FC_LEAN_TILES(X, KS)               \
    X(TILE_M128N32, 4, 1, 1, 1, 1, 16, KS, 4)  \
    X(TILE_M64N32K2, 2, 1, 2, 1, 1, 32, KS, (KS == 1 ? 4 : 8)) \
    X(TILE_M32N32K4, 1, 1, 4, 1, 1, 32, KS, (KS == 1 ? 4 : 8))

#define FC_LEAN_FLAVOURS_3(X) X(0) X(FL_POSTOP) X(FL_STATS) X(FL_STATS | FL_STAMP) X(FL_STATS | FL_CAT | FL_STAMP) X(FL_STATS | FL_RES) X(FL_STATS | FL_CAT) X(FL_STATS | FL_RES | FL_CAT) X(FL_STATS | FL_XF) \
    X(FL_STATS | FL_XF | FL_FIN) X(FL_STATS | FL_XF | FL_FIN | FL_GN1) X(FL_STATS | FL_XF | FL_FIN | FL_MEET) X(FL_STATS | FL_XF | FL_FIN | FL_GN1 | FL_MEET) \
    X(FL_STATS | FL_XF | FL_FIN | FL_STAMP) X(FL_STATS | FL_XF | FL_FIN | FL_GN1 | FL_STAMP) X(FL_STATS | FL_XF | FL_FIN | FL_MEET | FL_STAMP) X(FL_STATS | FL_XF | FL_FIN | FL_GN1 | FL_MEET | FL_STAMP)
#define FC_LEAN_FLAVOURS_1(X) X(0) X(FL_POSTOP) X(FL_XF) X(FL_STATS) X(FL_STATS | FL_XF)

#define FC_LEAN_TILES_WIDE1(X)             \
    X(TILE_M128N64, 4, 1, 1, 1, 2, 16, 1, 4)   \
    X(TILE_M256N64, 4, 1, 1, 2, 2, 16, 1, 4)

constexpr int kLeanNPL = 4;
template <int KS, int FL>
static int lean_attr() {
#define X(T, WM, WN, WK, MT, NT, CC, K, NL)                                                                               \
    FC_HIP(hipFuncSetAttribute(reinterpret_cast<const void*>(&conv_pipe_kernel<WM, WN, WK, MT, NT, CC, kLeanNPL, K, NL, FL>),  \
                               hipFuncAttributeMaxDynamicSharedMemorySize, 160 * 1024));
    FC_LEAN_TILES(X, KS)
#undef X
    return FC_OK;
}

constexpr bool ww_flavour(int FL) { return (FL & FL_FIN) && (FL & FL_XF) && !(FL & (FL_CAT | FL_RES)); }
template <int FL>
static int lean_attr_db4() {
    FC_HIP(hipFuncSetAttribute(reinterpret_cast<const void*>(&conv_pipe_kernel<1, 1, 4, 1, 1, 32, kLeanNPL, 3, 8, FL | FL_W4>),
                               hipFuncAttributeMaxDynamicSharedMemorySize, 160 * 1024));
    if constexpr (ww_flavour(FL))
        FC_HIP(hipFuncSetAttribute(reinterpret_cast<const void*>(&conv_pipe_kernel<1, 1, 4, 1, 1, 32, kLeanNPL, 3, 8, FL | FL_W4 | FL_WW>),
                                   hipFuncAttributeMaxDynamicSharedMemorySize, 160 * 1024));
    return FC_OK;
}

template <int FL>
static int lean_attr_wide1() {
#define X(T, WM, WN, WK, MT, NT, CC, K, NL)                                                                               \
    FC_HIP(hipFuncSetAttribute(reinterpret_cast<const void*>(&conv_pipe_kernel<WM, WN, WK, MT, NT, CC, kLeanNPL, K, NL, FL>),  \
                               hipFuncAttributeMaxDynamicSharedMemorySize, 160 * 1024));
    FC_LEAN_TILES_WIDE1(X)
#undef X
    return FC_OK;
}

template <class K>
static int launch_or_query(K kernel, int nthr, const ConvDev& d, int grid, size_t lds, hipStream_t s, int* occ) {
    if (occ) {
        FC_HIP(hipOccupancyMaxActiveBlocksPerMultiprocessor(occ, kernel, nthr, lds));
        return FC_OK;
    }
    hipLaunchKernelGGL(kernel, dim3(grid), dim3(nthr), lds, s, d);
    FC_HIP(hipGetLastError());
    return FC_OK;
}
static std::mutex g_route_mu;
static bool g_route_on = false;
static std::string g_route_log;
void conv_route_log_set(bool on) { std::lock_guard<std::mutex> lk(g_route_mu); g_route_on = on; if (on) g_route_log.clear(); }
std::string conv_route_log_get() { std::lock_guard<std::mutex> lk(g_route_mu); return g_route_log; }

template <int WM, int WN, int WK, int MT, int NT, int CC, int NPL, int KS, int NL, int FL = FL_ALL, int PREC = 0, int GEO = 0>
static int launch_pipe(const ConvDev& d, int grid, size_t lds, hipStream_t s, int* occ) {
    if (!occ && g_route_on) {
        std::lock_guard<std::mutex> lk(g_route_mu);
        const int v[12] = {WM, WN, WK, MT, NT, CC, NPL, KS, NL, FL, PREC, GEO};
        for (int i = 0; i < 12; ++i) g_route_log += std::to_string(v[i]) + (i < 11 ? " " : "\n");
    }
    return launch_or_query((conv_pipe_kernel<WM, WN, WK, MT, NT, CC, NPL, KS, NL, FL, PREC, GEO>), 256 + 64 * NL, d, grid, lds, s, occ);
}

template <int FL>
static int lean_launch_wide1(const ConvDev& d, int tile, int grid, size_t lds, hipStream_t s, int* occ) {
    switch (tile) {
#define X(T, WM, WN, WK, MT, NT, CC, K, NL)                                                                                       \
    case T:                                                                                                                       \
        if (d.P * (CC / 4) > 64 * NL * kLeanNPL) return -1;                                                                       \
        return launch_pipe<WM, WN, WK, MT, NT, CC, kLeanNPL, K, NL, FL>(d, grid, lds, s, occ);
        FC_LEAN_TILES_WIDE1(X)
#undef X
        default: return -1;
    }
}

template <int FL>
static int lean_launch_db4(const ConvDev& d, int tile, int grid, size_t lds, hipStream_t s, int* occ) {
    if (tile != TILE_M32N32K4 || d.P * (32 / 4) > 64 * 8 * kLeanNPL) return -1;
    return launch_pipe<1, 1, 4, 1, 1, 32, kLeanNPL, 3, 8, FL | FL_W4>(d, grid, lds, s, occ);
}

static int g_pipe_cus = 0;
static size_t ww_lds(const ConvDev& d, int tile, size_t lds) {
    const ConvArgs& a = d.a;
    if (tile != TILE_M32N32K4 || a.KS != 3 || !a.fin.gamma || a.s1.C || !a.s0.xf.mode || a.res_out || a.stride != 1) return 0;
    if ((long)d.P * (a.Cin / 4) > (long)kWWSlots * 768 || d.nblocks > g_pipe_cus) return 0;
    const size_t win = (size_t)(d.o_patch + d.nchunks * d.patch_stride) * sizeof(float), tot = win > lds ? win : lds;
    return tot <= 160 * 1024 ? tot : 0;
}

template <int FL>
static int lean_launch_ww(const ConvDev& d, int tile, int grid, size_t lds_ww, hipStream_t s, int* occ) {
    if constexpr (ww_flavour(FL)) return launch_pipe<1, 1, 4, 1, 1, 32, kLeanNPL, 3, 8, FL | FL_W4 | FL_WW>(d, grid, lds_ww, s, occ);
    else return -1;
}

template <int KS, int FL>
static int lean_launch(const ConvDev& d, int tile, int grid, size_t lds, hipStream_t s, int* occ) {
    switch (tile) {
#define X(T, WM, WN, WK, MT, NT, CC, K, NL)                                                                                       \
    case T:                                                                                                                       \
        if (d.P * (CC / 4) > 64 * NL * kLeanNPL) return -1;     \
        return launch_pipe<WM, WN, WK, MT, NT, CC, kLeanNPL, K, NL, FL>(d, grid, lds, s, occ);
        FC_LEAN_TILES(X, KS)
#undef X
        default: return -1;
    }
}

#define FC_FIN_GEOMS(X)                                                                                      \
    X(TILE_M128N32, 4, 1, 1, 1, 1, 16, 4, 0, FL_MEET, geo_key(GEO_FAST, 1, 16, 8, 8))         \
    X(TILE_M128N32, 4, 1, 1, 1, 1, 16, 4, 0, FL_MEET, geo_key(GEO_FAST, 1, 16, 16, 2))        \
    X(TILE_M64N32K2, 2, 1, 2, 1, 1, 32, 8, 0, FL_MEET, geo_key(GEO_FAST, 1, 16, 8, 4))        \
    X(TILE_M64N32K2, 2, 1, 2, 1, 1, 32, 8, 0, 0, geo_key(GEO_FAST, 1, 8, 32, 1))             \
    X(TILE_M32N32K4, 1, 1, 4, 1, 1, 32, 8, FL_W4, FL_MEET, geo_key(GEO_FAST, 1, 8, 16, 2))      \
    X(TILE_M32N32K4, 1, 1, 4, 1, 1, 32, 8, FL_W4, 0, geo_key(GEO_PAIR, 2, 4, 32, 1))         \
    X(TILE_M32N32K4, 1, 1, 4, 1, 1, 32, 8, FL_W4, FL_MEET, geo_key(GEO_PAIR, 2, 4, 64, 2))
#define FC_FIN_VARIANTS(Y) Y(0) Y(FL_GN1) Y(FL_STAMP) Y(FL_GN1 | FL_STAMP)
constexpr int kFinBase = FL_STATS | FL_XF | FL_FIN;

static int fin_geo_key(const ConvDev& d, int BM, int BN, int nthr, bool pair_tile) {
    const ConvArgs& a = d.a;
    if (!a.fin.gamma || !a.stats_out || a.par4 || a.stats_tmul != 1 || a.stats_toff != 0 || a.s1.C || !a.s0.xf.mode) return 0;
    if (d.TB != 1 && d.TB != 2) return 0;
    if (d.rps != BM / d.TB || (1 << (d.TWl + d.THl)) * d.TB != BM) return 0;
    const int form = (pair_tile && d.TB == 2 && d.rps == 16) ? GEO_PAIR : (d.TB == 1 ? GEO_FAST : 0);
    if (!form) return 0;
    const int cpg = d.cpg, NPG = cpg >= BN ? cpg / BN : 1, ngt = cpg >= BN ? 1 : BN / cpg;
    if (cpg < 1 || (cpg & (cpg - 1)) || cpg > (1 << 15) || d.cpgt != (cpg < BN ? cpg : BN) || d.NPG != NPG) return 0;
    const int Tst = (d.TB > 1 ? 1 : d.tiles_x * d.tiles_y) * NPG;
    if (Tst < 1 || Tst > kPartPre) return 0;
    if (a.Cout % BN || a.Cin != a.Cout || a.s0.xf.G <= 0 || a.s0.C != a.s0.xf.G * cpg || a.s0.xf.T != Tst) return 0;
    if (d.TB * a.Cin > nthr - 256 || d.TB * a.s0.xf.G > nthr - 256 || d.TB * ngt * Tst * 2 > nthr) return 0;
    return geo_key(form, d.TB, 1 << d.TWl, cpg, Tst);
}

template <int WM, int WN, int WK, int MT, int NT, int CC, int NL, int W4, int MEET, int GEO>
static int fin_geom_row_attr() {
#define Y(V) FC_HIP(hipFuncSetAttribute(reinterpret_cast<const void*>(&conv_pipe_kernel<WM, WN, WK, MT, NT, CC, kLeanNPL, 3, NL, kFinBase | W4 | MEET | (V), 0, GEO>), \
                                        hipFuncAttributeMaxDynamicSharedMemorySize, 160 * 1024));
    FC_FIN_VARIANTS(Y)
#undef Y
    if constexpr (W4 != 0) {
#define Y(V) FC_HIP(hipFuncSetAttribute(reinterpret_cast<const void*>(&conv_pipe_kernel<WM, WN, WK, MT, NT, CC, kLeanNPL, 3, NL, kFinBase | W4 | FL_WW | MEET | (V), 0, GEO>), \
                                        hipFuncAttributeMaxDynamicSharedMemorySize, 160 * 1024));
        FC_FIN_VARIANTS(Y)
#undef Y
    }
    return FC_OK;
}
static int fin_geom_attr() {
#define X(T, WM, WN, WK, MT, NT, CC, NL, W4, MEET, GEO) FC_TRY((fin_geom_row_attr<WM, WN, WK, MT, NT, CC, NL, W4, MEET, GEO>()));
    FC_FIN_GEOMS(X)
#undef X
    return FC_OK;
}

template <int WM, int WN, int WK, int MT, int NT, int CC, int NL, int W4, int MEET, int GEO>
static int fin_geom_row_launch(const ConvDev& d, int need, int grid, size_t lds, size_t lds_ww, hipStream_t s, int* occ) {
    if constexpr (W4 != 0) {
        if (lds_ww && d.a.Cin == kFinGeomGroups * geo_cpg(GEO)) {
#define Y(V) if (need == (kFinBase | MEET | (V))) return launch_pipe<WM, WN, WK, MT, NT, CC, kLeanNPL, 3, NL, kFinBase | W4 | FL_WW | MEET | (V), 0, GEO>(d, grid, lds_ww, s, occ);
            FC_FIN_VARIANTS(Y)
#undef Y
        }
    }
#define Y(V) if (need == (kFinBase | MEET | (V))) return launch_pipe<WM, WN, WK, MT, NT, CC, kLeanNPL, 3, NL, kFinBase | W4 | MEET | (V), 0, GEO>(d, grid, lds, s, occ);
    FC_FIN_VARIANTS(Y)
#undef Y
    return -1;
}

static int fin_geom_launch(const ConvDev& d, int tile, bool w4, int need, int grid, size_t lds, size_t lds_ww, hipStream_t s, int* occ) {
#define X(T, WM, WN, WK, MT, NT, CC, NL, W4, MEET, GEO)                                                         \
    if (tile == T && (w4 ? FL_W4 : 0) == (W4) && d.P * (CC / 4) <= 64 * NL * kLeanNPL &&                        \
        fin_geo_key(d, 32 * MT * WM, 32 * NT * WN, 256 + 64 * NL, WM * MT == 1 && WN * NT == 1) == (GEO))       \
        return fin_geom_row_launch<WM, WN, WK, MT, NT, CC, NL, W4, MEET, GEO>(d, need, grid, lds, lds_ww, s, occ);
    FC_FIN_GEOMS(X)
#undef X
    return -1;
}

#define FC_BF3_TILES(X, KS)                \
    X(TILE_M128N32, 4, 1, 1, 1, 1, 16, KS, 4)  \
    X(TILE_M128N64, 4, 1, 1, 1, 2, 16, KS, 4)  \
    X(TILE_M256N64, 4, 1, 1, 2, 2, 16, KS, 4)
template <int KS>
static int bf3_attr_ks() {
#define X(T, WM, WN, WK, MT, NT, CC, K, NL)                                                                                  \
    FC_HIP(hipFuncSetAttribute(reinterpret_cast<const void*>(&conv_pipe_kernel<WM, WN, WK, MT, NT, CC, 8, K, NL, FL_ALL, 1>), \
                               hipFuncAttributeMaxDynamicSharedMemorySize, 160 * 1024));
    FC_BF3_TILES(X, KS)
#undef X
    return FC_OK;
}
template <int KS>
static int bf3_launch_ks(const ConvDev& d, int tile, int grid, size_t lds, hipStream_t s, int* occ) {
    switch (tile) {
#define X(T, WM, WN, WK, MT, NT, CC, K, NL) \
    case T: return launch_pipe<WM, WN, WK, MT, NT, CC, 8, K, NL, FL_ALL, 1>(d, grid, lds, s, occ);
        FC_BF3_TILES(X, KS)
#undef X
        default: return fail(FC_E_ARG, "conv: no split-bf16 form of this tile");
    }
}

int conv_pipe_init() {
    static bool done = false;
    if (done) return FC_OK;
    FC_TRY(bf3_attr_ks<1>());
    FC_TRY(bf3_attr_ks<2>());
    FC_TRY(bf3_attr_ks<3>());
    {
        int dev = 0;
        hipDeviceProp_t prop;
        FC_HIP(hipGetDevice(&dev));
        FC_HIP(hipGetDeviceProperties(&prop, dev));
        g_pipe_cus = prop.multiProcessorCount;
    }
    FC_HIP(hipMalloc(reinterpret_cast<void**>(&g_zeros16), 256));
    FC_HIP(hipMemset(g_zeros16, 0, 256));
    FC_TRY(pipe_attr_ks<1>());
    FC_TRY(pipe_attr_ks<2>());
    FC_TRY(pipe_attr_ks<3>());
    FC_TRY(pipe_attr_ks<5>());
#define X(F) FC_TRY((lean_attr<3, (F)>())); FC_TRY((lean_attr_db4<(F)>()));
    FC_LEAN_FLAVOURS_3(X)
#undef X
#define X(F) FC_TRY((lean_attr<1, (F)>())); FC_TRY((lean_attr_wide1<(F)>()));
    FC_LEAN_FLAVOURS_1(X)
#undef X
    FC_TRY((lean_attr<2, 0>()));
    FC_TRY(fin_geom_attr());
    done = true;
    return FC_OK;
}

bool conv_pipe_supports_ks(int ks) { return ks == 1 || ks == 2 || ks == 3 || ks == 5; }

template <int KS>
static int pipe_launch_ks(const ConvDev& d, int tile, int grid, size_t lds, hipStream_t s, int* occ) {
    switch (tile) {
#define X(T, WM, WN, WK, MT, NT, CC, K, NL) \
    case T: return launch_pipe<WM, WN, WK, MT, NT, CC, 8, K, NL>(d, grid, lds, s, occ);
        FC_PIPE_TILES(X, KS)
#undef X
        default: return fail(FC_E_ARG, "conv: bad tile id");
    }
}

static int conv_pipe_dispatch(const ConvDev& d, int tile, int grid, size_t lds, hipStream_t s, int* occ) {
    if (d.bf3) return d.a.KS == 1 ? bf3_launch_ks<1>(d, tile, grid, lds, s, occ) : d.a.KS == 2 ? bf3_launch_ks<2>(d, tile, grid, lds, s, occ) : bf3_launch_ks<3>(d, tile, grid, lds, s, occ);
    static const bool lean = [] { const char* e = std::getenv("FLOCODER_AMD_LEAN_KERNELS"); return !(e && std::string(e) == "0"); }();
    if (lean) {
        const bool small_tile = tile == TILE_M32N32K4;
        const int need = (d.a.fin.gamma ? FL_FIN : 0) | (d.a.res_out ? FL_RES : 0) | (d.a.stats_post ? FL_POST : 0) | (d.any_xf ? FL_XF : 0) |
                         (d.a.s1.C ? FL_CAT : 0) | (d.stamps ? FL_STAMP : 0) | (d.a.stats_out ? FL_STATS : 0) | (d.a.fin.gn1_out ? FL_GN1 : 0) |
                         ((d.a.out_act || d.a.add) ? FL_POSTOP : 0) | (d.o_out < 0 ? FL_NARROW : 0) |
                         ((d.TB > 1 && !small_tile) ? FL_MULTI : 0) |
                         ((d.a.fin.gamma && !d.fin_local) ? FL_MEET : 0);
        int r = -1;
        if (d.a.KS == 3) {
            const bool w4 = small_tile && d.a.w4 && d.a.Cin % 32 == 0 && d.a.Cout % 32 == 0 && d.a.pad == 1 && !d.a.w_batch_stride &&
                            (!d.a.res_out || d.a.res_w4);
            const size_t lds_ww = (w4 && (need & FL_FIN)) ? ww_lds(d, tile, lds) : 0;
            if (need & FL_FIN) r = fin_geom_launch(d, tile, w4, need, grid, lds, lds_ww, s, occ);
            if (lds_ww) {
#define X(F) if (r == -1 && need == (F)) r = lean_launch_ww<(F)>(d, tile, grid, lds_ww, s, occ);
                FC_LEAN_FLAVOURS_3(X)
#undef X
            }
            if (w4) {
#define X(F) if (r == -1 && need == (F)) r = lean_launch_db4<(F)>(d, tile, grid, lds, s, occ);
                FC_LEAN_FLAVOURS_3(X)
#undef X
            }
#define X(F) if (r == -1 && need == (F)) r = lean_launch<3, (F)>(d, tile, grid, lds, s, occ);
            FC_LEAN_FLAVOURS_3(X)
#undef X
        } else if (d.a.KS == 1) {
#define X(F) if (r == -1 && need == (F)) { r = lean_launch<1, (F)>(d, tile, grid, lds, s, occ); if (r == -1) r = lean_launch_wide1<(F)>(d, tile, grid, lds, s, occ); }
            FC_LEAN_FLAVOURS_1(X)
#undef X
        } else if (d.a.KS == 2 && need == 0) {
            r = lean_launch<2, 0>(d, tile, grid, lds, s, occ);
        }
        if (r != -1) return r;
    }
    switch (d.a.KS) {
        case 1: return pipe_launch_ks<1>(d, tile, grid, lds, s, occ);
        case 2: return pipe_launch_ks<2>(d, tile, grid, lds, s, occ);
        case 3: return pipe_launch_ks<3>(d, tile, grid, lds, s, occ);
        case 5: return pipe_launch_ks<5>(d, tile, grid, lds, s, occ);
    }
    return fail(FC_E_SHAPE, "conv: kernel size not instantiated in the pipelined kernel");
}

int conv_pipe_launch(const ConvDev& d, int tile, int grid, size_t lds, hipStream_t s) { return conv_pipe_dispatch(d, tile, grid, lds, s, nullptr); }

int conv_pipe_blocks_per_cu(const ConvDev& d, int tile, size_t lds) {
    static std::map<std::tuple<int, int, int, size_t, int, int>, int> cache;
    static std::mutex mu;
    const int mask = (d.a.fin.gamma ? FL_FIN : 0) | (d.a.res_out ? FL_RES : 0) | (d.a.stats_post ? FL_POST : 0) | (d.any_xf ? FL_XF : 0) |
                     (d.a.s1.C ? FL_CAT : 0) | (d.stamps ? FL_STAMP : 0) | (d.a.stats_out ? FL_STATS : 0) | (d.a.fin.gn1_out ? FL_GN1 : 0) |
                     ((d.a.out_act || d.a.add) ? FL_POSTOP : 0) | (d.o_out < 0 ? FL_NARROW : 0) | (d.TB > 1 ? FL_MULTI : 0) |
                     ((d.a.fin.gamma && !d.fin_local) ? FL_MEET : 0);
    const int ww = (d.a.KS == 3 && d.a.w4 && ww_lds(d, tile, lds)) ? d.a.Cin : 0;
    const auto key = std::make_tuple(tile, d.a.KS, mask | (d.a.w4 ? FL_W4 : 0), lds, d.cpg, d.TB * 4096 + (d.TWl << 8) + d.tiles_x * d.tiles_y * d.NPG + (ww << 13));
    std::lock_guard<std::mutex> lk(mu);
    auto it = cache.find(key);
    if (it != cache.end()) return it->second;
    int occ = 0;
    if (conv_pipe_dispatch(d, tile, 1, lds, nullptr, &occ) != FC_OK) occ = 0;
    cache[key] = occ;
    return occ;
}

}
```

### flocoder_amd/csrc/linattn_fused.hip

```cpp
#include <cstdlib>
#include <string>

#include "common.h"
#include "stats_dev.h"

namespace fc {

typedef float f32x16 __attribute__((ext_vector_type(16)));
#define FC_MFMA(a, b, c) __builtin_amdgcn_mfma_f32_32x32x2f32((a), (b), (c), 0, 0, 0)

constexpr int LDH = 32, LHEADS = 4, LHID = LHEADS * LDH, LC3 = 3 * LHID, PS = 33;

__device__ __forceinline__ int acc_row(int r, int half) { return (r & 3) + 8 * (r >> 2) + 4 * half; }

__device__ __forceinline__ void stage_x(const LaArgs& a, const float* Ab, const float* Bb, float* xw, int XS, int b, int r0, int c0, int cl, int lane) {
    const int q4 = cl >> 2;
    for (int idx = lane; idx < 32 * q4; idx += 64) {
        const int row = idx / q4, q = idx - row * q4, nn = r0 + row, c = c0 + 4 * q;
        float4 v = make_float4(0.f, 0.f, 0.f, 0.f);
        if (nn < a.n) {
            v = *reinterpret_cast<const float4*>(a.x + ((size_t)b * a.n + nn) * a.C + c);
            v.x = Ab[c] * v.x + Bb[c]; v.y = Ab[c + 1] * v.y + Bb[c + 1]; v.z = Ab[c + 2] * v.z + Bb[c + 2]; v.w = Ab[c + 3] * v.w + Bb[c + 3];
        }
        float* d = xw + row * XS + 4 * q;
        d[0] = v.x; d[1] = v.y; d[2] = v.z; d[3] = v.w;
    }
}

__global__ void __launch_bounds__(256) la_ctx_kernel(const LaArgs a) {
    extern __shared__ __attribute__((aligned(16))) float sm[];
    const int C = a.C, CC = C < 64 ? C : 64, XS = CC + 1;
    float* Ab = sm;
    float* Bb = Ab + C;
    float* Wl = Bb + C;
    float* xt = Wl + C * 64;
    float* Et = xt + 4 * 32 * XS;
    float* Vt = Et + 4 * 32 * PS;
    float* sct = Vt + 4 * 32 * PS;
    float* mz = sct + 128;
    const int h = blockIdx.x, b = blockIdx.y, tid = threadIdx.x, lane = tid & 63, wave = tid >> 6, half = lane >> 5, l31 = lane & 31;
    float mean, rstd;
    combine_partials(a.xf, b, 0, &mean, &rstd);
    for (int c = tid; c < C; c += 256) {
        const float s = rstd * a.xf.gamma[c];
        Ab[c] = s;
        Bb[c] = a.xf.beta[c] - mean * s;
    }
    for (int i = tid; i < C * 64; i += 256) {
        const int c = i >> 6, j = i & 63;
        Wl[i] = a.wqkv[(size_t)c * LC3 + (j < 32 ? LHID + h * LDH + j : 2 * LHID + h * LDH + (j - 32))];
    }
    float* xw = xt + wave * 32 * XS;
    float* Ew = Et + wave * 32 * PS;
    float* Vw = Vt + wave * 32 * PS;
    float* scw = sct + wave * 32;
    const int nblk = (a.n + 31) >> 5, iters = (nblk + 3) >> 2;
    f32x16 cacc;
#pragma unroll
    for (int r = 0; r < 16; ++r) cacc[r] = 0.f;
    float m_run = -INFINITY, z_run = 0.f;
    for (int it = 0; it < iters; ++it) {
        const int rb = it * 4 + wave, r0 = rb * 32;
        const bool active = rb < nblk;
        f32x16 ak, av;
#pragma unroll
        for (int r = 0; r < 16; ++r) { ak[r] = 0.f; av[r] = 0.f; }
        for (int c0 = 0; c0 < C; c0 += CC) {
            const int cl = C - c0 < CC ? C - c0 : CC;
            __syncthreads();
            if (active) stage_x(a, Ab, Bb, xw, XS, b, r0, c0, cl, lane);
            __syncthreads();
            if (active) {
                for (int s = 0; s < (cl >> 1); ++s) {
                    const float xa = xw[l31 * XS + 2 * s + half];
                    const float* wr = Wl + (c0 + 2 * s + half) * 64 + l31;
                    ak = FC_MFMA(xa, wr[0], ak);
                    av = FC_MFMA(xa, wr[32], av);
                }
            }
        }
        if (active) {
            float bm = -INFINITY;
#pragma unroll
// ... 89 lines not shown
            const float xa = xw[l31 * XS + 2 * s + half];
            const float* wr = Wc + (2 * s + half) * LHID + l31;
#pragma unroll
            for (int hh = 0; hh < LHEADS; ++hh) q[hh] = FC_MFMA(xa, wr[hh * 32], q[hh]);
        }
    }
    const float scale = 0.17677669529663687f;
#pragma unroll
    for (int hh = 0; hh < LHEADS; ++hh)
#pragma unroll
        for (int r = 0; r < 16; ++r) {
            const float v = q[hh][r];
            float m = v;
            m = fmaxf(m, __shfl_xor(m, 1)); m = fmaxf(m, __shfl_xor(m, 2)); m = fmaxf(m, __shfl_xor(m, 4));
            m = fmaxf(m, __shfl_xor(m, 8)); m = fmaxf(m, __shfl_xor(m, 16));
            const float e = __expf(v - m);
            float s = e;
            s += __shfl_xor(s, 1); s += __shfl_xor(s, 2); s += __shfl_xor(s, 4); s += __shfl_xor(s, 8); s += __shfl_xor(s, 16);
            q[hh][r] = e * (scale / s);
        }
    f32x16 y[CT];
#pragma unroll
    for (int ct = 0; ct < CT; ++ct)
#pragma unroll
        for (int r = 0; r < 16; ++r) y[ct][r] = 0.f;
#pragma unroll
    for (int hh = 0; hh < LHEADS; ++hh) {
        __syncthreads();
        for (int i = tid; i < 32 * WO; i += 256) {
            const int k = i / WO, c = i - k * WO;
            Wc[i] = c < C ? a.wout[(size_t)(hh * LDH + k) * C + c] : 0.f;
        }
#pragma unroll
        for (int r = 0; r < 16; ++r) Pw[acc_row(r, half) * PS + l31] = q[hh][r];
        __syncthreads();
        f32x16 o;
#pragma unroll
        for (int r = 0; r < 16; ++r) o[r] = 0.f;
#pragma unroll 4
        for (int s = 0; s < 16; ++s) o = FC_MFMA(Pw[l31 * PS + 2 * s + half], ctxl[(hh * LDH + 2 * s + half) * PS + l31], o);
        __syncthreads();
#pragma unroll
        for (int r = 0; r < 16; ++r) Pw[acc_row(r, half) * PS + l31] = o[r];
        __syncthreads();
#pragma unroll 2
        for (int s = 0; s < 16; ++s) {
            const float oa = Pw[l31 * PS + 2 * s + half];
            const float* wr = Wc + (2 * s + half) * WO + l31;
#pragma unroll
            for (int ct = 0; ct < CT; ++ct) y[ct] = FC_MFMA(oa, wr[ct * 32], y[ct]);
        }
    }
    float S = 0.f, Q = 0.f;
#pragma unroll
    for (int ct = 0; ct < CT; ++ct) {
        const int c = ct * 32 + l31;
        const float bias = (c < C && a.bout) ? a.bout[c] : 0.f;
#pragma unroll
        for (int r = 0; r < 16; ++r) {
            const float v = y[ct][r] + bias;
            y[ct][r] = v;
            if (r0 + acc_row(r, half) < a.n && c < C) { S += v; Q += v * v; }
        }
    }
    const float St = block_sum(S, red);
    const float Qt = block_sum(Q, red);
    if (tid == 0) {
        const float mt = St / n_t;
        float* d = a.stats_out + ((size_t)b * T + tile) * 2;
        d[0] = mt;
        d[1] = Qt - St * mt;
    }
#pragma unroll
    for (int ct = 0; ct < CT; ++ct) {
        const int c = ct * 32 + l31;
#pragma unroll
        for (int r = 0; r < 16; ++r) {
            const int nn = r0 + acc_row(r, half);
            if (nn < a.n && c < C) a.y[((size_t)b * a.n + nn) * C + c] = y[ct][r];
        }
    }
}

template <int NQ>
__device__ __forceinline__ void fetch_xh(const LaArgs& a, int b, int r0, int lane, float4 (&pre)[NQ]) {
    const int nn = r0 + (lane & 31);
    const float* p = a.x + ((size_t)b * a.n + nn) * (NQ * 8) + (lane >> 5) * (NQ * 4);
#pragma unroll
    for (int j = 0; j < NQ; ++j) {
        pre[j] = make_float4(0.f, 0.f, 0.f, 0.f);
        if (nn < a.n) pre[j] = *reinterpret_cast<const float4*>(p + 4 * j);
    }
}
template <int NQ>
__device__ __forceinline__ void norm_xh(const LaArgs& a, const float* Ab, const float* Bb, int r0, int lane, const float4 (&pre)[NQ], float (&xn)[NQ * 4]) {
    const bool in = r0 + (lane & 31) < a.n;
    const float* ap = Ab + (lane >> 5) * (NQ * 4);
    const float* bp = Bb + (lane >> 5) * (NQ * 4);
#pragma unroll
    for (int j = 0; j < NQ; ++j) {
        const float4 A = *reinterpret_cast<const float4*>(ap + 4 * j), Bv = *reinterpret_cast<const float4*>(bp + 4 * j);
        float4 v = pre[j];
        if (in) { v.x = A.x * v.x + Bv.x; v.y = A.y * v.y + Bv.y; v.z = A.z * v.z + Bv.z; v.w = A.w * v.w + Bv.w; }
        xn[4 * j] = v.x; xn[4 * j + 1] = v.y; xn[4 * j + 2] = v.z; xn[4 * j + 3] = v.w;
    }
}

template <int NQ, int NW>
__global__ void __launch_bounds__(64 * NW) la_ctx_fast_kernel(const LaArgs a) {
    extern __shared__ __attribute__((aligned(16))) float sm[];
    constexpr int C = NQ * 8, H2 = C / 2, NT = 64 * NW;
    float* Ab = sm;
    float* Bb = Ab + C;
    float* Et = Bb + C;
    float* sct = Et + NW * 32 * PS;
    float* mz = sct + NW * 32;
    const int h = blockIdx.x, b = blockIdx.y, tid = threadIdx.x, lane = tid & 63, wave = tid >> 6, half = lane >> 5, l31 = lane & 31;
    const int nblk = (a.n + 31) >> 5;
    float4 pre[NQ];
    if (wave < nblk) fetch_xh<NQ>(a, b, wave * 32, lane, pre);
    PartPre pp;
    partials_request(a.xf, b, 0, pp);
    const float pg = tid < C ? a.xf.gamma[tid] : 0.f, pbt = tid < C ? a.xf.beta[tid] : 0.f;
    float wk[H2], wv[H2];
#pragma unroll
    for (int s = 0; s < H2; ++s) {
        const float* wr = a.wqkv + (size_t)(s + half * H2) * LC3 + h * LDH + l31;
        wk[s] = wr[LHID];
        wv[s] = wr[2 * LHID];
    }
    float mean, rstd;
    partials_finish(a.xf, b, 0, pp, &mean, &rstd);
    if (tid < C) {
        const float s = rstd * pg;
        Ab[tid] = s;
        Bb[tid] = pbt - mean * s;
    }
    __syncthreads();
    f32x16 cacc;
#pragma unroll
    for (int r = 0; r < 16; ++r) cacc[r] = 0.f;
    float m_run = -INFINITY, z_run = 0.f;
    for (int rb = wave; rb < nblk; rb += NW) {
        const int r0 = rb * 32;
        float xn[H2];
        norm_xh<NQ>(a, Ab, Bb, r0, lane, pre, xn);
        if (rb + NW < nblk) fetch_xh<NQ>(a, b, r0 + 32 * NW, lane, pre);
        f32x16 ak, av;
#pragma unroll
        for (int r = 0; r < 16; ++r) { ak[r] = 0.f; av[r] = 0.f; }
#pragma unroll
        for (int s = 0; s < H2; ++s) {
            ak = FC_MFMA(xn[s], wk[s], ak);
            av = FC_MFMA(xn[s], wv[s], av);
        }
        float bm = -INFINITY;
#pragma unroll
        for (int r = 0; r < 16; ++r) if (r0 + acc_row(r, half) < a.n) bm = fmaxf(bm, ak[r]);
        bm = fmaxf(bm, __shfl_xor(bm, 32));
        const float m_new = fmaxf(m_run, bm);
        const float sc = __expf(m_run - m_new);
        float zs = 0.f;
#pragma unroll
        for (int r = 0; r < 16; ++r) {
            const float e = (r0 + acc_row(r, half) < a.n) ? __expf(ak[r] - m_new) : 0.f;
            zs += e;
            ak[r] = e;
        }
        zs += __shfl_xor(zs, 32);
        z_run = z_run * sc + zs;
        m_run = m_new;
#pragma unroll
        for (int r = 0; r < 16; ++r) cacc[r] *= sc;
#pragma unroll
        for (int r = 0; r < 16; ++r) cacc = FC_MFMA(av[r], ak[r], cacc);
    }
    if (half == 0) { mz[(wave * 2) * 32 + l31] = m_run; mz[(wave * 2 + 1) * 32 + l31] = z_run; }
    __syncthreads();
    if (tid < 32 * NW) {
        const int w = tid >> 5, d = tid & 31;
        float M = mz[d];
        for (int k = 1; k < NW; ++k) M = fmaxf(M, mz[(k * 2) * 32 + d]);
        float Z = 0.f;
        for (int k = 0; k < NW; ++k) Z += mz[(k * 2 + 1) * 32 + d] * __expf(mz[(k * 2) * 32 + d] - M);
        sct[w * 32 + d] = __expf(mz[(w * 2) * 32 + d] - M) / Z;
    }
    __syncthreads();
    const float fw = sct[wave * 32 + l31];
#pragma unroll
    for (int r = 0; r < 16; ++r) Et[(wave * 32 + l31) * PS + acc_row(r, half)] = cacc[r] * fw;
    __syncthreads();
    for (int i = tid; i < LDH * LDH; i += NT) {
        const int d = i >> 5, e = i & 31;
        float v = (Et[d * PS + e] + Et[(32 + d) * PS + e]) + (Et[(64 + d) * PS + e] + Et[(96 + d) * PS + e]);
        if (NW == 8) v += (Et[(128 + d) * PS + e] + Et[(160 + d) * PS + e]) + (Et[(192 + d) * PS + e] + Et[(224 + d) * PS + e]);
        a.ctx[((size_t)(b * LHEADS + h) * LDH + d) * LDH + e] = v;
    }
}

constexpr int AS = 20;
__device__ __forceinline__ int acc_reg(int row) { return (row & 3) + 4 * (row >> 3); }
template <int NQ, int CT>
__global__ void __launch_bounds__(256) la_apply_fast_kernel(const LaArgs a, int T, float n_t) {
    extern __shared__ __attribute__((aligned(16))) float sm[];
    constexpr int C = NQ * 8, H2 = C / 2, SQ = H2 + 4, WO = CT * 32;
    float* Ab = sm;
    float* Bb = Ab + C;
    float* WqL = Bb + C;
    float* ctxL = WqL + LHEADS * 64 * SQ;
    float* WoL = ctxL + LHEADS * 64 * AS;
    __shared__ float red[4];
    __shared__ unsigned epoch_s;
    __shared__ float gv[2 * kPartPre];
    const int tile = blockIdx.x, b = blockIdx.y, tid = threadIdx.x, lane = tid & 63, wave = tid >> 6, half = lane >> 5, l31 = lane & 31;
    const int r0 = tile * 128 + wave * 32, nn = r0 + l31;
    const bool in = nn < a.n;
    unsigned arrival = 0;
    if (a.gran && tid == 0) arrival = __hip_atomic_fetch_add(a.sync + b, 1u, __ATOMIC_RELAXED, __HIP_MEMORY_SCOPE_AGENT);
    float4 pre[NQ];
    fetch_xh<NQ>(a, b, r0, lane, pre);
    PartPre pp;
    partials_request(a.xf, b, 0, pp);
    const float pg = tid < C ? a.xf.gamma[tid] : 0.f, pbt = tid < C ? a.xf.beta[tid] : 0.f;
    constexpr int NWO = WO / 2;
    float4 wq[NQ], cx[4];
    float wo[NWO];
#pragma unroll
    for (int k = 0; k < NQ; ++k) {
        const int i = tid + 256 * k, cc = (i >> 7) * 4 + (i & 3), j = ((i >> 2) & 31) * 4;
        wq[k] = *reinterpret_cast<const float4*>(a.wqkv + (size_t)cc * LC3 + j);
    }
#pragma unroll
    for (int k = 0; k < NWO; ++k) {
        const int i = tid + 256 * k, kk = i / WO, c = i - kk * WO;
        wo[k] = c < C ? a.wout[(size_t)kk * C + c] : 0.f;
    }
#pragma unroll
    for (int k = 0; k < 4; ++k) cx[k] = *reinterpret_cast<const float4*>(a.ctx + (size_t)b * LHEADS * LDH * LDH + 4 * (tid + 256 * k));
#pragma unroll
    for (int k = 0; k < NQ; ++k) {
        const int i = tid + 256 * k, cc = (i >> 7) * 4 + (i & 3), j = ((i >> 2) & 31) * 4;
        const int hf = cc / H2, s = cc - hf * H2;
        float* d = WqL + (((j >> 5) * 2 + hf) * 32 + (j & 31)) * SQ + s;
        d[0] = wq[k].x; d[SQ] = wq[k].y; d[2 * SQ] = wq[k].z; d[3 * SQ] = wq[k].w;
    }
#pragma unroll
    for (int k = 0; k < NWO; ++k) {
        const int i = tid + 256 * k, kk = i / WO, c = i - kk * WO, e = kk & 31;
        WoL[((((kk >> 5) * CT + (c >> 5)) * 2 + ((e >> 2) & 1)) * 32 + (c & 31)) * AS + acc_reg(e)] = wo[k];
    }
#pragma unroll
    for (int k = 0; k < 4; ++k) {
        const int i = 4 * (tid + 256 * k), d0 = (i >> 5) & 31;
        float* d = ctxL + (((i >> 10) * 2 + ((d0 >> 2) & 1)) * 32 + (i & 31)) * AS + acc_reg(d0);
        d[0] = cx[k].x; d[AS] = cx[k].y; d[2 * AS] = cx[k].z; d[3 * AS] = cx[k].w;
    }
    {
        float mean, rstd;
        partials_finish(a.xf, b, 0, pp, &mean, &rstd);
        if (tid < C) {
            const float s = rstd * pg;
            Ab[tid] = s;
            Bb[tid] = pbt - mean * s;
        }
        if (a.gran && tid == 0) epoch_s = arrival / (unsigned)T + 1u;
    }
    float4 pbias[CT][4], rs[CT][4];
#pragma unroll
    for (int ct = 0; ct < CT; ++ct)
#pragma unroll
        for (int g = 0; g < 4; ++g) {
            const int c = ct * 32 + 8 * g + 4 * half;
            const float4 z = make_float4(0.f, 0.f, 0.f, 0.f);
            pbias[ct][g] = z; rs[ct][g] = z;
            if (c < C && a.bout) pbias[ct][g] = *reinterpret_cast<const float4*>(a.bout + c);
            if (a.gran && c < C && in) rs[ct][g] = *reinterpret_cast<const float4*>(a.x + ((size_t)b * a.n + nn) * C + c);
        }
    __syncthreads();
    float xn[H2];
    norm_xh<NQ>(a, Ab, Bb, r0, lane, pre, xn);
    const float scale = 0.17677669529663687f;
    f32x16 y[CT];
#pragma unroll
    for (int ct = 0; ct < CT; ++ct)
#pragma unroll
        for (int r = 0; r < 16; ++r) y[ct][r] = 0.f;
#pragma unroll
    for (int hh = 0; hh < LHEADS; ++hh) {
        f32x16 q;
#pragma unroll
        for (int r = 0; r < 16; ++r) q[r] = 0.f;
        const float* wa = WqL + ((hh * 2 + half) * 32 + l31) * SQ;
#pragma unroll
        for (int j = 0; j < NQ; ++j) {
            const float4 w = *reinterpret_cast<const float4*>(wa + 4 * j);
            q = FC_MFMA(w.x, xn[4 * j], q);
            q = FC_MFMA(w.y, xn[4 * j + 1], q);
            q = FC_MFMA(w.z, xn[4 * j + 2], q);
            q = FC_MFMA(w.w, xn[4 * j + 3], q);
        }
        float m = q[0];
#pragma unroll
        for (int r = 1; r < 16; ++r) m = fmaxf(m, q[r]);
        m = fmaxf(m, __shfl_xor(m, 32));
        float sum = 0.f;
#pragma unroll
        for (int r = 0; r < 16; ++r) { q[r] = __expf(q[r] - m); sum += q[r]; }
        sum += __shfl_xor(sum, 32);
        const float f = scale / sum;
#pragma unroll
        for (int r = 0; r < 16; ++r) q[r] *= f;
        f32x16 o;
#pragma unroll
        for (int r = 0; r < 16; ++r) o[r] = 0.f;
        const float* ca = ctxL + ((hh * 2 + half) * 32 + l31) * AS;
#pragma unroll
        for (int j = 0; j < 4; ++j) {
            const float4 w = *reinterpret_cast<const float4*>(ca + 4 * j);
            o = FC_MFMA(w.x, q[4 * j], o);
            o = FC_MFMA(w.y, q[4 * j + 1], o);
            o = FC_MFMA(w.z, q[4 * j + 2], o);
            o = FC_MFMA(w.w, q[4 * j + 3], o);
        }
#pragma unroll
        for (int ct = 0; ct < CT; ++ct) {
            const float* oa = WoL + (((hh * CT + ct) * 2 + half) * 32 + l31) * AS;
#pragma unroll
            for (int j = 0; j < 4; ++j) {
                const float4 w = *reinterpret_cast<const float4*>(oa + 4 * j);
                y[ct] = FC_MFMA(w.x, o[4 * j], y[ct]);
                y[ct] = FC_MFMA(w.y, o[4 * j + 1], y[ct]);
                y[ct] = FC_MFMA(w.z, o[4 * j + 2], y[ct]);
                y[ct] = FC_MFMA(w.w, o[4 * j + 3], y[ct]);
            }
        }
    }
    float S = 0.f, Q = 0.f;
#pragma unroll
    for (int ct = 0; ct < CT; ++ct)
#pragma unroll
        for (int g = 0; g < 4; ++g) {
            const float4 bi = pbias[ct][g];
            const float v0 = y[ct][4 * g] + bi.x, v1 = y[ct][4 * g + 1] + bi.y, v2 = y[ct][4 * g + 2] + bi.z, v3 = y[ct][4 * g + 3] + bi.w;
            y[ct][4 * g] = v0; y[ct][4 * g + 1] = v1; y[ct][4 * g + 2] = v2; y[ct][4 * g + 3] = v3;
            if (in && ct * 32 + 8 * g + 4 * half < C) {
                S += v0; Q += v0 * v0; S += v1; Q += v1 * v1; S += v2; Q += v2 * v2; S += v3; Q += v3 * v3;
            }
        }
    const float St = block_sum(S, red);
    const float Qt = block_sum(Q, red);
    if (a.gran) {
        const unsigned epoch = epoch_s;
        float4 g2[CT][4], b2[CT][4];
#pragma unroll
        for (int ct = 0; ct < CT; ++ct)
#pragma unroll
            for (int g = 0; g < 4; ++g) {
                const int c = ct * 32 + 8 * g + 4 * half;
                g2[ct][g] = make_float4(0.f, 0.f, 0.f, 0.f); b2[ct][g] = g2[ct][g];
                if (c < C) { g2[ct][g] = *reinterpret_cast<const float4*>(a.g2 + c); b2[ct][g] = *reinterpret_cast<const float4*>(a.b2 + c); }
            }
        if (tid == 0) {
            const float mt = St / n_t;
            unsigned long long* gp = a.gran + ((size_t)b * T + tile) * 2;
            const unsigned long long tag = (unsigned long long)epoch << 32;
            __hip_atomic_store(gp, tag | __float_as_uint(mt), __ATOMIC_RELAXED, __HIP_MEMORY_SCOPE_AGENT);
            __hip_atomic_store(gp + 1, tag | __float_as_uint(Qt - St * mt), __ATOMIC_RELAXED, __HIP_MEMORY_SCOPE_AGENT);
        }
        if (tid < 2 * T) {
            const unsigned long long* gp = a.gran + (size_t)b * T * 2 + tid;
            unsigned long long v = __hip_atomic_load(gp, __ATOMIC_RELAXED, __HIP_MEMORY_SCOPE_AGENT);
            int spins = 0;
            while ((unsigned)(v >> 32) != epoch) {
                if (++spins > (1 << 20)) { if (a.err) *a.err = 1; v = 0x7fc00000ull; break; }
                __builtin_amdgcn_s_sleep(2);
                v = __hip_atomic_load(gp, __ATOMIC_RELAXED, __HIP_MEMORY_SCOPE_AGENT);
            }
            gv[tid] = __uint_as_float((unsigned)v);
        }
        __syncthreads();
        float sm2 = 0.f;
        for (int t = 0; t < T; ++t) sm2 += gv[2 * t];
        const float mean = sm2 / (float)T;
        float m2 = 0.f, dv = 0.f;
        for (int t = 0; t < T; ++t) {
            const float d = gv[2 * t] - mean;
            m2 += gv[2 * t + 1];
            dv += d * d;
        }
        const float rstd = 1.0f / sqrtf((m2 + n_t * dv) / (n_t * (float)T) + a.eps2);
#pragma unroll
        for (int ct = 0; ct < CT; ++ct)
#pragma unroll
            for (int g = 0; g < 4; ++g) {
                const int c = ct * 32 + 8 * g + 4 * half;
                const float4 gg = g2[ct][g], bb = b2[ct][g], rr = rs[ct][g];
                float4 ov;
                { const float A = rstd * gg.x, Bc = bb.x - mean * A; ov.x = (A * y[ct][4 * g] + Bc) + rr.x; }
                { const float A = rstd * gg.y, Bc = bb.y - mean * A; ov.y = (A * y[ct][4 * g + 1] + Bc) + rr.y; }
                { const float A = rstd * gg.z, Bc = bb.z - mean * A; ov.z = (A * y[ct][4 * g + 2] + Bc) + rr.z; }
                { const float A = rstd * gg.w, Bc = bb.w - mean * A; ov.w = (A * y[ct][4 * g + 3] + Bc) + rr.w; }
                if (in && c < C) *reinterpret_cast<float4*>(a.out + ((size_t)b * a.n + nn) * C + c) = ov;
            }
        return;
    }
    if (tid == 0) {
        const float mt = St / n_t;
        float* d = a.stats_out + ((size_t)b * T + tile) * 2;
        d[0] = mt;
        d[1] = Qt - St * mt;
    }
#pragma unroll
    for (int ct = 0; ct < CT; ++ct)
#pragma unroll
        for (int g = 0; g < 4; ++g) {
            const int c = ct * 32 + 8 * g + 4 * half;
            if (in && c < C) *reinterpret_cast<float4*>(a.y + ((size_t)b * a.n + nn) * C + c) = make_float4(y[ct][4 * g], y[ct][4 * g + 1], y[ct][4 * g + 2], y[ct][4 * g + 3]);
        }
}

static size_t la_ctx_fast_lds(int C, int NW) { return (size_t)(2 * C + NW * 32 * PS + 32 * NW + 64 * NW) * sizeof(float); }
static int la_ctx_waves(int n) { return n >= 256 ? 8 : 4; }
static size_t la_apply_fast_lds(int C, int CT) { return (size_t)(2 * C + LHEADS * 64 * (C / 2 + 4) + LHEADS * 64 * AS + LHEADS * CT * 64 * AS) * sizeof(float); }
template <int NQ>
static int launch_fast(const LaArgs& a, hipStream_t s) {
    if (la_ctx_waves(a.n) == 8) hipLaunchKernelGGL((la_ctx_fast_kernel<NQ, 8>), dim3(LHEADS, a.B), dim3(512), la_ctx_fast_lds(a.C, 8), s, a);
    else hipLaunchKernelGGL((la_ctx_fast_kernel<NQ, 4>), dim3(LHEADS, a.B), dim3(256), la_ctx_fast_lds(a.C, 4), s, a);
    FC_HIP(hipGetLastError());
    const int T = linattn_fused_tiles(a.n);
    const float n_t = linattn_fused_nt(a.n, a.C);
    const dim3 grid(cdiv(a.n, 128), a.B);
    if (a.C <= 32) hipLaunchKernelGGL((la_apply_fast_kernel<NQ, 1>), grid, dim3(256), la_apply_fast_lds(a.C, 1), s, a, T, n_t);
    else hipLaunchKernelGGL((la_apply_fast_kernel<NQ, 2>), grid, dim3(256), la_apply_fast_lds(a.C, 2), s, a, T, n_t);
    FC_HIP(hipGetLastError());
    return FC_OK;
}
template <int NQ>
static int init_fast() {
    FC_HIP(hipFuncSetAttribute(reinterpret_cast<const void*>(la_ctx_fast_kernel<NQ, 4>), hipFuncAttributeMaxDynamicSharedMemorySize, 160 * 1024));
    FC_HIP(hipFuncSetAttribute(reinterpret_cast<const void*>(la_ctx_fast_kernel<NQ, 8>), hipFuncAttributeMaxDynamicSharedMemorySize, 160 * 1024));
    FC_HIP(hipFuncSetAttribute(reinterpret_cast<const void*>(la_apply_fast_kernel<NQ, 1>), hipFuncAttributeMaxDynamicSharedMemorySize, 160 * 1024 - 256));
    FC_HIP(hipFuncSetAttribute(reinterpret_cast<const void*>(la_apply_fast_kernel<NQ, 2>), hipFuncAttributeMaxDynamicSharedMemorySize, 160 * 1024 - 256));
    return FC_OK;
}

static size_t la_ctx_lds(int C) {
    const int CC = C < 64 ? C : 64;
    return (size_t)(2 * C + C * 64 + 4 * 32 * (CC + 1) + 2 * 4 * 32 * PS + 128 + 256) * sizeof(float);
}
static size_t la_apply_lds(int C, int CT) {
    const int CC = C < 64 ? C : 64, WO = CT * 32;
    const int wc = CC * LHID > 32 * WO ? CC * LHID : 32 * WO;
    return (size_t)(2 * C + wc + 4 * 32 * (CC + 1) + 2 * 4 * 32 * PS) * sizeof(float);
}

int linattn_fused_tiles(int n) { return n >= 128 ? n / 128 : 1; }
float linattn_fused_nt(int n, int C) { return (float)((n >= 128 ? 128 : n) * C); }

int linattn_fused_init() {
    FC_HIP(hipFuncSetAttribute(reinterpret_cast<const void*>(la_ctx_kernel), hipFuncAttributeMaxDynamicSharedMemorySize, 160 * 1024));
    FC_HIP(hipFuncSetAttribute(reinterpret_cast<const void*>(la_apply_kernel<1>), hipFuncAttributeMaxDynamicSharedMemorySize, 160 * 1024 - 256));
    FC_HIP(hipFuncSetAttribute(reinterpret_cast<const void*>(la_apply_kernel<2>), hipFuncAttributeMaxDynamicSharedMemorySize, 160 * 1024 - 256));
    FC_HIP(hipFuncSetAttribute(reinterpret_cast<const void*>(la_apply_kernel<4>), hipFuncAttributeMaxDynamicSharedMemorySize, 160 * 1024 - 256));
    FC_HIP(hipFuncSetAttribute(reinterpret_cast<const void*>(la_apply_kernel<8>), hipFuncAttributeMaxDynamicSharedMemorySize, 160 * 1024 - 256));
    FC_TRY(init_fast<1>()); FC_TRY(init_fast<2>()); FC_TRY(init_fast<4>()); FC_TRY(init_fast<8>());
    return FC_OK;
}

bool linattn_fused_supported(int n, int C, int heads) {
    if (heads != LHEADS || (C & 3) || C > 256 || n < 1) return false;
    if (n >= 128 && (n & 127)) return false;
    return la_ctx_lds(C) <= 160 * 1024;
}

template <int NQ>
static int apply_blocks_per_cu(int C) {
    int nb = 0;
    const hipError_t e = C <= 32 ? hipOccupancyMaxActiveBlocksPerMultiprocessor(&nb, la_apply_fast_kernel<NQ, 1>, 256, la_apply_fast_lds(C, 1))
                                 : hipOccupancyMaxActiveBlocksPerMultiprocessor(&nb, la_apply_fast_kernel<NQ, 2>, 256, la_apply_fast_lds(C, 2));
    return e == hipSuccess ? nb : 0;
}
bool linattn_fused_meeting_ok(int B, int n, int C) {
    if (n < 256 || (n & 127) || !(C == 8 || C == 16 || C == 32 || C == 64)) return false;
    const int T = linattn_fused_tiles(n);
    if (T != n / 128 || T > kPartPre) return false;
    if (linattn_fused_init() != FC_OK) return false;
    int dev = 0, cus = 0;
    if (hipGetDevice(&dev) != hipSuccess || hipDeviceGetAttribute(&cus, hipDeviceAttributeMultiprocessorCount, dev) != hipSuccess) return false;
    const int per = C == 8 ? apply_blocks_per_cu<1>(C) : C == 16 ? apply_blocks_per_cu<2>(C) : C == 32 ? apply_blocks_per_cu<4>(C) : apply_blocks_per_cu<8>(C);
    return (long long)per * cus >= (long long)T * B;
}

int linattn_fused_launch(const LaArgs& a, hipStream_t s) {
    if (!linattn_fused_supported(a.n, a.C, a.heads)) return fail(FC_E_SHAPE, "linattn_fused: unsupported shape");
    if (a.xf.mode != 1 || a.xf.G != 1 || !a.xf.stats) return fail(FC_E_ARG, "linattn_fused: needs GroupNorm(1) statistics of x");
    if (a.gran && (!a.sync || !a.out || !a.g2 || !a.b2 || !(a.C == 8 || a.C == 16 || a.C == 32 || a.C == 64)))
        return fail(FC_E_ARG, "linattn_fused: the fused close needs the fast path, the arrival counters, to_out.1's parameters and the output");
    if (a.C <= 64 && (a.C & 7) == 0 && (a.C == 8 || a.C == 16 || a.C == 32 || a.C == 64)) {
        switch (a.C) {
            case 8: return launch_fast<1>(a, s);
            case 16: return launch_fast<2>(a, s);
            case 32: return launch_fast<4>(a, s);
            default: return launch_fast<8>(a, s);
        }
    }
    hipLaunchKernelGGL(la_ctx_kernel, dim3(LHEADS, a.B), dim3(256), la_ctx_lds(a.C), s, a);
    FC_HIP(hipGetLastError());
    const int T = linattn_fused_tiles(a.n);
    const float n_t = linattn_fused_nt(a.n, a.C);
    const int CT = a.C <= 32 ? 1 : a.C <= 64 ? 2 : a.C <= 128 ? 4 : 8;
    const dim3 grid(cdiv(a.n, 128), a.B);
    const size_t lds = la_apply_lds(a.C, CT);
    switch (CT) {
        case 1: hipLaunchKernelGGL(la_apply_kernel<1>, grid, dim3(256), lds, s, a, T, n_t); break;
        case 2: hipLaunchKernelGGL(la_apply_kernel<2>, grid, dim3(256), lds, s, a, T, n_t); break;
        case 4: hipLaunchKernelGGL(la_apply_kernel<4>, grid, dim3(256), lds, s, a, T, n_t); break;
        default: hipLaunchKernelGGL(la_apply_kernel<8>, grid, dim3(256), lds, s, a, T, n_t); break;
    }
    FC_HIP(hipGetLastError());
    return FC_OK;
}

}
```

### flocoder_amd/csrc/unet.hip

```cpp
#include <algorithm>
#include <cmath>
#include <cstdint>
#include <cstdlib>
#include <cstring>
#include <map>
#include <memory>
#include <mutex>
#include <string>
#include <unordered_map>
#include <vector>

#include "plan.h"
#include "unet_priv.h"
#include "unet_sample.h"

namespace fc {

static thread_local std::string g_err;
void set_error(const std::string& m) { g_err = m; }
int fail(int code, const std::string& m) { g_err = m; return code; }
const char* last_error() { return g_err.c_str(); }

}

// ... 948 lines not shown
    return FC_OK;
}

int fc_unet_op_bytes(const fc_unet* u, int i, double* bytes_per_sample, double* bytes_per_launch) {
    if (!u || i < 0 || i >= (int)u->plan.ops.size()) return fail(FC_E_ARG, "fc_unet_op_bytes: index out of range");
    if (bytes_per_sample) *bytes_per_sample = u->plan.op_bytes_ps[i];
    if (bytes_per_launch) *bytes_per_launch = u->plan.op_bytes_fixed[i];
    return FC_OK;
}

int fc_unet_chains(const fc_unet* u, int* rows_per_chain) {
    if (!u) return 0;
    if (rows_per_chain) *rows_per_chain = u->maxB;
    return 1;
}

int fc_unet_fused_tail_errors(const fc_unet* u, int* count) {
    if (!u || !count) return fail(FC_E_ARG, "fc_unet_fused_tail_errors: null argument");
    *count = 0;
    if (u->device < 0 || !u->dev_err) return FC_OK;
    int v = 0;
    FC_HIP(hipMemcpy(&v, u->dev_err, sizeof(int), hipMemcpyDeviceToHost));
    *count = (v != 0 || u->tail_failed) ? 1 : 0;
    return FC_OK;
}

int fc_unet_plan_launches(const fc_unet* u) { return u ? (int)u->plan.ops.size() : 0; }
double fc_unet_flops_per_sample(const fc_unet* u) { return u ? u->plan.flops : 0.0; }

int fc_unet_train_form(const fc_unet* u) { return (u && u->keep_all) ? 1 : 0; }

int fc_unet_train_release(fc_unet* u) {
    if (!u) return fail(FC_E_ARG, "fc_unet_train_release: null handle");
    if (u->device < 0 || !u->keep_all) return FC_OK;
    FC_HIP(hipSetDevice(u->device));
    FC_HIP(hipDeviceSynchronize());
    free_plan(u);
    u->keep_all = false;
    u->arena_touched(0);
    return FC_OK;
}

int fc_unet_debug_tensor(const fc_unet* u, const char* name, const float** ptr, int* C, int* H, int* W) {
    if (!u || !name) return fail(FC_E_ARG, "fc_unet_debug_tensor: null argument");
    auto it = u->plan.named.find(name);
    if (it == u->plan.named.end()) {
        it = u->bwd.named.find(name);
        if (it == u->bwd.named.end()) return fail(FC_E_ARG, std::string("fc_unet_debug_tensor: no tap named ") + name);
    }
    *ptr = it->second.p; *C = it->second.C; *H = it->second.H; *W = it->second.W;
    return FC_OK;
}

int fc_debug_unet_break_meeting(fc_unet* u) {
    if (!u || u->plan.fin_sync.empty()) return fail(FC_E_STATE, "fc_debug_unet_break_meeting: the plan has no meeting launch");
    FC_HIP(hipDeviceSynchronize());
    unsigned v = 0;
    FC_HIP(hipMemcpy(&v, u->plan.fin_sync[0], sizeof(unsigned), hipMemcpyDeviceToHost));
    ++v;
    FC_HIP(hipMemcpy(u->plan.fin_sync[0], &v, sizeof(unsigned), hipMemcpyHostToDevice));
    return FC_OK;
}

int fc_debug_unet_break_meeting_kind(fc_unet* u, int kind) {
    if (!u) return fail(FC_E_ARG, "fc_debug_unet_break_meeting_kind: null handle");
    const Plan& pl = u->plan;
    for (size_t i = 0; i < pl.fin_sync.size(); ++i)
        if (pl.fin_kind[i] == kind) {
            FC_HIP(hipDeviceSynchronize());
            unsigned v = 0;
            FC_HIP(hipMemcpy(&v, pl.fin_sync[i], sizeof(unsigned), hipMemcpyDeviceToHost));
            ++v;
            FC_HIP(hipMemcpy(pl.fin_sync[i], &v, sizeof(unsigned), hipMemcpyHostToDevice));
            return FC_OK;
        }
    return fail(FC_E_STATE, "fc_debug_unet_break_meeting_kind: the plan has no meeting launch of that kind");
}

int fc_debug_set_fused_tail(int on) {
    fc::g_fused_tail = on < 0 ? -1 : (on ? 1 : 0);
    return FC_OK;
}

int fc_debug_conv_routes(int on) { conv_route_log_set(on != 0); return FC_OK; }
int fc_debug_conv_routes_read(char* buf, int cap) {
    const std::string r = conv_route_log_get();
    if (buf && cap > 0) { const size_t n = r.size() < (size_t)cap - 1 ? r.size() : (size_t)cap - 1; memcpy(buf, r.data(), n); buf[n] = 0; }
    return (int)r.size();
}

int fc_debug_set_conv_stamps(void* buf_dev) {
    conv_set_stamp_buffer(static_cast<unsigned long long*>(buf_dev));
    return FC_OK;
}

int fc_debug_copy(void* dst_dev, const void* src_dev, int64_t bytes, void* stream) {
    FC_HIP(hipMemcpyAsync(dst_dev, src_dev, (size_t)bytes, hipMemcpyDeviceToDevice, static_cast<hipStream_t>(stream)));
    return FC_OK;
}

static int g_debug_conv_prec = 0;
int fc_debug_set_conv_precision(int mode) { g_debug_conv_prec = mode == 1 ? 1 : 0; return FC_OK; }

int fc_debug_conv(const float* src0, int c0, const float* src1, int c1, const float* w_oihw, const float* bias, const float* add,
                  float* out, float* stats_out, int groups_out, int* stats_T, float* stats_nt, int batch, int hs, int ws, int cout,
                  int ksize, int pad, int stride, int upsample, int out_act, int tile_cfg, int repeats, float* ms_out, void* stream) {
    hipStream_t s = static_cast<hipStream_t>(stream);
    FC_TRY(conv_init());
    ConvArgs a;
    a.s0.p = src0; a.s0.C = c0; a.s1.p = src1; a.s1.C = src1 ? c1 : 0;
    a.Cin = a.s0.C + a.s1.C; a.Cout = cout; a.B = batch; a.Hs = hs; a.Ws = ws;
    a.KS = ksize; a.pad = pad; a.stride = stride; a.ups = upsample;
    a.H = upsample ? hs * 2 : (hs + 2 * pad - ksize) / stride + 1;
    a.W = upsample ? ws * 2 : (ws + 2 * pad - ksize) / stride + 1;
    a.bias = bias; a.add = add; a.out = out; a.out_act = out_act;
    a.stats_out = stats_out; a.Gout = groups_out;
    a.prec = g_debug_conv_prec;
    float* wp = nullptr;
    FC_HIP(hipMalloc(reinterpret_cast<void**>(&wp), (size_t)cout * a.Cin * ksize * ksize * sizeof(float)));
    int r = pack_conv_launch(w_oihw, wp, cout, a.Cin, ksize, ksize, s);
    a.w = wp;
    float* wp8 = nullptr;
    if (r == FC_OK && ksize == 3 && a.Cin % 32 == 0 && cout % 32 == 0) {
        FC_HIP(hipMalloc(reinterpret_cast<void**>(&wp8), (size_t)cout * a.Cin * 9 * sizeof(float)));
        r = pack_conv_k8_launch(w_oihw, wp8, cout, a.Cin, 9, s);
        a.w4 = wp8;
    }
    float* wp3 = nullptr;
    if (r == FC_OK && a.prec == 1 && (ksize == 3 || ksize == 1)) {
        const int ipad = (a.Cin + 15) / 16 * 16;
        FC_HIP(hipMalloc(reinterpret_cast<void**>(&wp3), (size_t)cout * ipad * ksize * ksize * sizeof(float)));
        r = pack_conv_b3_launch(w_oihw, wp3, cout, a.Cin, ksize * ksize, ipad, s);
        a.w_b3 = wp3;
    }
    ConvGeom g;
    if (r == FC_OK) r = conv_plan(a, tile_cfg, &g);
    if (r == FC_OK) { if (stats_T) *stats_T = g.T; if (stats_nt) *stats_nt = g.n_t; r = conv_launch(a, g.tile, s); }
    if (r == FC_OK && repeats > 0 && ms_out) {
        hipEvent_t e0, e1;
        (void)hipEventCreate(&e0); (void)hipEventCreate(&e1);
        (void)hipEventRecord(e0, s);
        for (int i = 0; i < repeats && r == FC_OK; ++i) r = conv_launch(a, g.tile, s);
        (void)hipEventRecord(e1, s);
        (void)hipEventSynchronize(e1);
        float ms = 0.f;
        (void)hipEventElapsedTime(&ms, e0, e1);
        *ms_out = ms / repeats;
        (void)hipEventDestroy(e0); (void)hipEventDestroy(e1);
    }
    (void)hipStreamSynchronize(s);
    (void)hipFree(wp);
    if (wp8) (void)hipFree(wp8);
    if (wp3) (void)hipFree(wp3);
    return r;
}

int fc_debug_conv_wgrad(const float* src0, int c0, const float* src1, int c1, const float* dy, int cout, int batch, int hs, int ws, int ksize,
                        int pad, int stride, int upsample, float* dw_out, float* db_out, void* stream) {
    hipStream_t s = static_cast<hipStream_t>(stream);
    FC_TRY(conv_wgrad_init());
    WgradArgs a;
    a.x0 = src0; a.C0 = c0; a.x1 = src1; a.C1 = src1 ? c1 : 0; a.Cin = a.C0 + a.C1; a.Cout = cout; a.dy = dy;
    a.B = batch; a.Hs = hs; a.Ws = ws; a.KS = ksize; a.pad = pad; a.stride = stride; a.ups = upsample;
    a.H = upsample ? hs * 2 : (hs + 2 * pad - ksize) / stride + 1;
    a.W = upsample ? ws * 2 : (ws + 2 * pad - ksize) / stride + 1;
    a.dw = dw_out; a.db = db_out;
    const size_t need = conv_wgrad_workspace(a);
    float* wsp = nullptr;
    if (need) FC_HIP(hipMalloc(reinterpret_cast<void**>(&wsp), need * sizeof(float)));
// ... 63 lines not shown
```

### include/flocoder_amd.h

```cpp
#ifndef FLOCODER_AMD_H
#define FLOCODER_AMD_H

#include <stdint.h>

#ifdef __cplusplus
extern "C" {
#endif

#define FC_OK 0
#define FC_E_ARG (-1)
#define FC_E_SHAPE (-2)
#define FC_E_ARCH (-3)
#define FC_E_HIP (-4)
#define FC_E_STATE (-5)

#define FC_ABI_VERSION 1

int fc_abi_version(void);
const char* fc_last_error(void);
int fc_check_device(int device);

typedef struct fc_unet fc_unet;

typedef struct fc_unet_config {
// ... 46 lines not shown
int fc_unet_plan_launches(const fc_unet* u);
int fc_unet_fused_tail_errors(const fc_unet* u, int* count);
int fc_unet_set_shared(fc_unet* u, int shared);
int fc_unet_meeting_launches(const fc_unet* u);
int fc_unet_check(fc_unet* u, void* stream, int synchronize);
int fc_debug_unet_break_meeting(fc_unet* u);
int fc_debug_unet_break_meeting_kind(fc_unet* u, int kind);
int fc_debug_set_fused_tail(int on);
double fc_unet_flops_per_sample(const fc_unet* u);
int fc_unet_op_info(const fc_unet* u, int i, const char** kernel, const char** module, double* flops_per_sample);
int fc_unet_op_bytes(const fc_unet* u, int i, double* bytes_per_sample, double* bytes_per_launch);
int fc_unet_profile_ops(fc_unet* u, int batch, int repeats, float* ms_out, int n_out, void* stream);

int fc_unet_set_time_freqs(fc_unet* u, const float* freqs_host, int n);

int fc_unet_log_likelihood(fc_unet* u, float* x_inout_dev, int batch, int height, int width, const float* ts_host, int n_points,
                           float t_scale, const int64_t* class_ids_dev, const float* mask_dev, int mask_is_ones, const float* probe_dev,
                           double* a_out_dev, double* logp_out_dev, void* stream);

int fc_unet_log_likelihood_rk45(fc_unet* u, float* x_inout_dev, int batch, int height, int width, double t0, double t1, double rtol,
                                double atol, float t_scale, const int64_t* class_ids_dev, const float* mask_dev, int mask_is_ones,
                                const float* probe_dev, int per_sample, double* a_out_dev, double* logp_out_dev, int* counters,
                                void* stream);

#define FC_LL_MAX_PROBES 64
int fc_unet_log_likelihood_probes(fc_unet* u, float* x_inout_dev, int batch, int height, int width, const float* ts_host, int n_points,
                                  float t_scale, const int64_t* class_ids_dev, const float* mask_dev, int mask_is_ones,
                                  const float* probes_dev, int n_probes, double* a_out_dev, double* logp_out_dev,
                                  double* a_probes_out_dev, double* stderr_out_dev, void* stream);
int fc_unet_log_likelihood_rk45_probes(fc_unet* u, float* x_inout_dev, int batch, int height, int width, double t0, double t1, double rtol,
                                       double atol, float t_scale, const int64_t* class_ids_dev, const float* mask_dev, int mask_is_ones,
                                       const float* probes_dev, int n_probes, int per_sample, double* a_out_dev, double* logp_out_dev,
                                       double* a_probes_out_dev, double* stderr_out_dev, int* counters, void* stream);
#define FC_PROBE_RADEMACHER 0
#define FC_PROBE_GAUSSIAN 1
#define FC_PROBE_KEY_OFFSET 0x50524F4245464C44ULL
int fc_ode_probe_field(float* out_dev, int kind, uint64_t seed, int64_t probe_index, const int64_t* sample_ids_dev, int batch,
                       int64_t per_sample, void* stream);

#define FC_JACOBIAN_IDENTITY 0
#define FC_JACOBIAN_EXACT 1
int fc_unet_integrate_guided(fc_unet* u, float* x_dev, int batch, int height, int width, const float* ts_host, int n_points, float t_scale,
                             const int64_t* class_ids_dev, float cfg_strength, const float* mask_dev, int mask_is_ones,
                             const float* y_meas_dev, const float* keep_dev, float sigma_y, float gamma, int jacobian, void* stream);
int fc_ode_guided_correct(const float* v_dev, const float* x_dev, const float* y_dev, const float* a_dev, int64_t n, float t, float sigma_y,
                          float gamma, float* out_dev, void* stream);

#define FC_SDE_EULER_MARUYAMA 0
#define FC_SDE_HEUN 1
int fc_unet_integrate_sde(fc_unet* u, int scheme, float* x_dev, int batch, int height, int width, const float* ts_host, int n_points,
                          float t_scale, const int64_t* class_ids_dev, float cfg_strength, const float* mask_dev, int mask_is_ones,
                          float sigma, uint64_t seed, const int64_t* sample_ids_dev, const float* noise_dev, void* stream);
int fc_ode_normal_field(float* out_dev, uint64_t seed, int64_t draw_index, const int64_t* sample_ids_dev, int batch, int64_t per_sample,
                        void* stream);

#define FC_MASK_TOTAL 0
#define FC_MASK_BRUSH 1
#define FC_MASK_RECTANGLES 2
#define FC_MASK_NOISE 3
#define FC_MASK_NOTHING 4
#define FC_MASK_MIN_SIZE 16
#define FC_MASK_MAX_SIZE 1024
#define FC_MASK_KEY_OFFSET 0x4D41534B464C4431ULL
int fc_inpaint_masks(float* masks_out_dev, int* types_out_dev, uint64_t seed, const int64_t* sample_ids_dev, int batch, int height, int width,
                     const int* choice_types_host, const double* probs_host, int n_choices, int forced_type, void* stream);

int fc_note_confusion(const float* pred_dev, int pred_channels, const float* target_dev, int target_channels, const float* region_dev, int batch,
                      int height, int width, float threshold, double minval, int derive_min, double maxval, int derive_max, int keep_gray,
                      void* ws_dev, int64_t* counts_out_dev, float* masks_out_dev, float* overlay_out_dev, void* stream);

#define FC_HIST_LDS_BINS 8192
int fc_index_histogram(const int64_t* indices_dev, int64_t n, int levels, int codebook_size, int64_t* counts_inout_dev, int64_t* keys_out_dev,
                       int64_t* bad_rows_inout_dev, void* stream);

int fc_debug_unet_guided_buffers(const fc_unet* u, const float** stage_x, const float** stage_time, const float** w, const float** q);
int fc_debug_probe_dot(const float* probe_dev, const float* g_dev, double* out_dev, int batch, int64_t per_sample, void* stream);
int fc_unet_debug_tensor(const fc_unet* u, const char* name, const float** ptr, int* channels, int* height, int* width);
int fc_debug_copy(void* dst_dev, const void* src_dev, int64_t bytes, void* stream);
int fc_debug_set_poison(int on);
int fc_debug_poison_check(int* corrupted, int* live);
int fc_debug_set_conv_stamps(void* buf_dev);
int fc_debug_conv_routes(int on);
int fc_debug_conv_routes_read(char* buf, int cap);
int fc_debug_set_stamp_op(int op_index, void* buf_dev);
int fc_debug_set_conv_precision(int mode);
int fc_debug_conv(const float* src0_nhwc, int c0, const float* src1_nhwc, int c1, const float* w_oihw_dev, const float* bias_dev,
                  const float* add_nhwc, float* out_nhwc, float* stats_out, int groups_out, int* stats_T, float* stats_nt, int batch,
                  int hs, int ws, int cout, int ksize, int pad, int stride, int upsample, int out_act, int tile_cfg, int repeats,
                  float* ms_out, void* stream);

int fc_unet_train_reserve(fc_unet* u, int max_batch, int height, int width);
int fc_unet_backward(fc_unet* u, const float* x_dev, const float* time_dev, const int64_t* class_ids_dev, const float* d_out_dev,
                     float* grads_flat_dev, int64_t numel, int batch, int height, int width, void* stream);
int fc_unet_backward_ex(fc_unet* u, const float* x_dev, const float* time_dev, const int64_t* class_ids_dev, const float* mask_dev,
                        int mask_is_ones, const float* d_out_dev, float* grads_flat_dev, int64_t numel, float* dx_out_dev,
                        float* dmask_out_dev, int batch, int height, int width, void* stream);
int fc_unet_backward_parts(fc_unet* u, const float* x_dev, const float* time_dev, const int64_t* class_ids_dev, const float* mask_dev,
                           int mask_is_ones, const float* d_out_dev, float* grads_flat_dev, int64_t numel, float* dx_out_dev,
                           float* dmask_out_dev, int batch, int height, int width, int first_part, int last_part, void* stream);
int fc_unet_backward_accumulate(fc_unet* u, const float* x_dev, const float* time_dev, const int64_t* class_ids_dev, const float* mask_dev,
                                int mask_is_ones, const float* d_out_dev, float* grads_flat_dev, int64_t numel, float* dx_out_dev,
                                float* dmask_out_dev, int batch, int height, int width, int first_part, int last_part, void* stream);
int fc_unet_set_grad_buckets(fc_unet* u, int on);
int fc_unet_grad_buckets(const fc_unet* u, int64_t* split_offset);
int fc_unet_backward_launches(const fc_unet* u);
int fc_unet_backward_op_info(const fc_unet* u, int i, const char** kernel, const char** module);
int fc_unet_train_form(const fc_unet* u);
int fc_unet_train_release(fc_unet* u);
int fc_unet_vjp_x(fc_unet* u, const float* x_dev, const float* time_dev, const int64_t* class_ids_dev, const float* mask_dev,
                  int mask_is_ones, const float* d_out_dev, float* dx_out_dev, int batch, int height, int width, void* stream);
int fc_unet_vjp_launches(const fc_unet* u);
int fc_unet_vjp_op_info(const fc_unet* u, int i, const char** kernel, const char** module);
uint64_t fc_unet_arena_serial(const fc_unet* u);
int fc_unet_class_param_range(const fc_unet* u, int64_t* lo, int64_t* hi);
int fc_flow_interp(const float* source_dev, const float* target_dev, const float* t_dev, float* x_out_dev, float* v_out_dev, int batch,
                   int64_t per_sample, void* stream);
int fc_flow_prepare(const float* source_dev, const float* target_dev, const int64_t* pairing_dev, const float* u_dev, float t_eps, float warp_s,
                    float t_scale, const int64_t* class_ids_dev, int n_classes, float* t_out_dev, float* time_out_dev, float* x_out_dev,
                    float* v_out_dev, int* id_flag_dev, int batch, int64_t per_sample, void* stream);
int fc_flow_prepare_rows(const float* source_dev, const float* target_dev, const int64_t* pairing_dev, const float* u_dev, float t_eps, float warp_s,
                         float t_scale, const int64_t* class_ids_dev, int n_classes, float* t_out_dev, float* time_out_dev, float* x_out_dev,
                         float* v_out_dev, int* id_flag_dev, int batch, int first_row, int target_rows, int64_t per_sample, void* stream);
int fc_mse_loss_grad_scaled(const float* v_dev, const float* target_dev, float* dv_out_dev, float* loss_acc_dev, float* ws256_dev, int64_t numel,
                            float scale, void* stream);
int fc_mse_loss_grad(const float* v_dev, const float* target_dev, float* dv_out_dev, float* loss_out_dev, float* ws256_dev, int64_t numel,
                     void* stream);
int fc_grad_clip_coef(const float* grads_dev, int64_t numel, const float* grads2_dev, int64_t numel2, float max_norm, float* norm_coef_out_dev,
                      float* ws256_dev, void* stream);
int fc_adam_ema_step(float* params_dev, const float* grads_dev, float* exp_avg_dev, float* exp_avg_sq_dev, float* ema_dev, int64_t numel,
                     const float* clip_coef_dev, float lr, float beta1, float beta2, float eps, int step, float ema_decay, int apply_adam,
                     void* stream);
int fc_adam_ema_step_guarded(float* params_dev, const float* grads_dev, float* exp_avg_dev, float* exp_avg_sq_dev, float* ema_dev, int64_t numel,
                             const float* clip_coef_dev, float lr, float beta1, float beta2, float eps, int step, float ema_decay, int apply_adam,
                             const int* skip_flag_dev, void* stream);
int fc_debug_conv_wgrad(const float* src0, int c0, const float* src1, int c1, const float* dy, int cout, int batch, int hs, int ws, int ksize,
                        int pad, int stride, int upsample, float* dw_out, float* db_out, void* stream);

typedef struct fc_vae fc_vae;
int fc_vae_create(int device, fc_vae** out);
void fc_vae_destroy(fc_vae* v);
int fc_vae_param_count(const fc_vae* v);
int64_t fc_vae_param_numel(const fc_vae* v);
int fc_vae_param_info(const fc_vae* v, int i, const char** name, int64_t shape[4], int64_t* offset);
int fc_vae_load_params(fc_vae* v, const float* flat, int64_t numel, int on_device, void* stream);
int fc_vae_reserve_encode(fc_vae* v, int max_batch, int height, int width);
int fc_vae_reserve_decode(fc_vae* v, int max_batch, int lat_height, int lat_width);
int fc_vae_encode(fc_vae* v, const float* x_dev, float* mean_out_dev, int batch, int height, int width, void* stream);
int fc_vae_decode(fc_vae* v, const float* z_dev, float* x_out_dev, int batch, int lat_height, int lat_width, void* stream);
int fc_vae_set_precision(fc_vae* v, int mode);
double fc_vae_flops_per_sample(const fc_vae* v, int decode);
int fc_vae_plan_launches(const fc_vae* v, int decode);
int fc_vae_op_info(const fc_vae* v, int decode, int i, const char** kernel, const char** module, double* flops_per_sample);
int fc_vae_profile_ops(fc_vae* v, int decode, const float* in_dev, float* out_dev, int batch, int repeats, float* ms_out, int n_out,
                       void* stream);
int fc_vae_op_bytes(const fc_vae* v, int decode, int i, double* bytes_per_sample, double* bytes_per_launch);
int fc_vae_debug_taps(fc_vae* v, int on);
int fc_vae_debug_tensor(const fc_vae* v, int decode, const char* name, const float** ptr, int* channels, int* height, int* width);

typedef struct fc_vqvae fc_vqvae;
int fc_vqvae_create(int in_channels, int hidden_channels, int num_downsamples, int internal_dim, int vq_embedding_dim, int decoder_nonlocal,
                    int device, fc_vqvae** out);
int fc_vqvae_create_ex(int in_channels, int hidden_channels, int num_downsamples, int internal_dim, int vq_embedding_dim,
                       int decoder_nonlocal, int natten_layout, int device, fc_vqvae** out);
int fc_na2d(const float* qkv_nhwc_dev, float* out_nhwc_dev, const float* gamma_dev, int batch, int height, int width, int channels,
            int heads, int kernel_size, int layout_mode, void* stream);
void fc_vqvae_destroy(fc_vqvae* v);
// ... 57 lines not shown
```

Before: 894.0 samples/s.

## Add compile-time geometry conv1 flavours and planned linear-attention block counts

Adds compile-time geometry keys for lean conv1 flavours (3x3, stride 1, stats, optional concat and residual) so patch size, indexing and output addressing become constants rather than runtime magic divisions. Separately, the linear-attention context and apply kernels get shape-specific template variants (NB/TT splits) for C=32/64 at n=256/1024, plus route logging for debugging. This is meant to cut integer index overhead and pick better work splits, at the cost of more kernel instantiations and more complex dispatch matching.

```diff
diff --git a/flocoder_amd/_binding.py b/flocoder_amd/_binding.py
--- a/flocoder_amd/_binding.py
+++ b/flocoder_amd/_binding.py
@@ -59,6 +59,7 @@
     "fc_debug_set_stamp_op": (_i, [_i, _vp]),
     "fc_debug_conv_routes": (_i, [_i]),
     "fc_debug_conv_routes_read": (_i, [C.c_char_p, _i]),
+    "fc_debug_linattn_routes_read": (_i, [C.c_char_p, _i]),
     "fc_debug_conv": (_i, [_vp, _i, _vp, _i, _vp, _vp, _vp, _vp, _vp, _i, _pi, _pf, _i, _i, _i, _i, _i, _i, _i, _i, _i, _i, _i, _pf, _vp]),
     "fc_debug_set_fused_tail": (_i, [_i]),
     "fc_unet_fused_tail_errors": (_i, [_vp, C.POINTER(_i)]),
diff --git a/flocoder_amd/csrc/common.h b/flocoder_amd/csrc/common.h
--- a/flocoder_amd/csrc/common.h
+++ b/flocoder_amd/csrc/common.h
@@ -205,6 +205,8 @@
 int linattn_fused_tiles(int n);
 float linattn_fused_nt(int n, int C);
 int linattn_fused_launch(const LaArgs& a, hipStream_t s);
+void linattn_route_log_set(bool on);
+std::string linattn_route_log_get();
 bool linattn_fused_meeting_ok(int B, int n, int C);
 int linattn_sample_init();
 bool linattn_sample_supported(int n, int C, int heads);
diff --git a/flocoder_amd/csrc/conv_dev.h b/flocoder_amd/csrc/conv_dev.h
--- a/flocoder_amd/csrc/conv_dev.h
+++ b/flocoder_amd/csrc/conv_dev.h
@@ -102,6 +102,7 @@
 constexpr int geo_TWl(int k) { return (k >> 3) & 7; }
 constexpr int geo_cpg(int k) { return 1 << ((k >> 6) & 15); }
 constexpr int geo_Tst(int k) { return (k >> 10) & 63; }
+constexpr bool geo_conv1_mask(int FL) { return (FL & ~(FL_W4 | FL_STAMP)) == FL_STATS || (FL & ~(FL_W4 | FL_STAMP)) == (FL_STATS | FL_CAT | FL_RES); }
 
 template <int WM, int WN, int WK, int MT, int NT, int FL = FL_ALL, int GEO = 0>
 __device__ __forceinline__ void conv_epilogue(const ConvDev& p, f32x16 (&acc)[MT][NT], f32x16 (&accr)[MT][NT], float* smem, int tid, int lane,
@@ -112,8 +113,11 @@
     const int half = lane >> 5, l31 = lane & 31;
     const int wk = wave % WK, wn = (wave / WK) % WN, wm = wave / (WK * WN);
     constexpr bool GEOC = GEO != 0;
-    static_assert(!GEOC || (FL != FL_ALL && (FL & FL_FIN) && (FL & FL_STATS) && !(FL & (FL_MULTI | FL_POST | FL_RES))), "a geometry key belongs to a lean Block-closing flavour");
-    static_assert(!GEOC || (geo_Tst(GEO) >= 1 && geo_TB(GEO) * (geo_cpg(GEO) >= BN ? 1 : BN / geo_cpg(GEO)) * geo_Tst(GEO) * 2 <= 512), "one granule per thread");
+    constexpr bool GEO1 = GEOC && !(FL & FL_FIN);
+    static_assert(!GEOC || (FL != FL_ALL && (FL & FL_STATS) && !(FL & (FL_MULTI | FL_POST)) && ((FL & FL_FIN) ? !(FL & FL_RES) : geo_conv1_mask(FL))),
+                  "a geometry key belongs to a lean Block-closing flavour or to a lean conv1 flavour");
+    static_assert(!GEOC || geo_Tst(GEO) >= 1, "statistics slots of the key");
+    static_assert(!GEOC || GEO1 || geo_TB(GEO) * (geo_cpg(GEO) >= BN ? 1 : BN / geo_cpg(GEO)) * geo_Tst(GEO) * 2 <= 512, "one granule per thread");
     const int g_TB = GEOC ? geo_TB(GEO) : p.TB;
     const int g_TWl = GEOC ? geo_TWl(GEO) : p.TWl;
     const int g_tbsh = GEOC ? geo_log2(BM / geo_TB(GEO)) : p.TWl + p.THl;
@@ -172,6 +176,7 @@
         const int m = (wm * MT + mt) * 32 + (r & 3) + 8 * (r >> 2) + 4 * half;
         const int tw = m & (TW - 1), th = (m >> g_TWl) & (TH - 1), tb = m >> g_tbsh;
         const int b = b0 + tb;
+        if (GEO1) return b < a.B ? (b * a.H + y0 + th) * a.W + x0 + tw : -1;
         return b < a.B ? (b * (a.H << a.out_sh) + ((y0 + th) << a.out_sh) + a.out_oy) * (a.W << a.out_sh) + ((x0 + tw) << a.out_sh) + a.out_ox : -1;
     };
     if (FL & FL_STAMP) conv_stamp(p, 6);
@@ -519,7 +524,9 @@
                 const int m = i / Q4, c4 = (i - m * Q4) * 4, n = n0 + c4;
                 const int tw = m & (TW - 1), th = (m >> g_TWl) & (TH - 1), tb = m >> g_tbsh;
                 const int b = b0 + tb;
-                if (b < a.B && n < Cout) {
+                if (GEO1) {
+                    if (b < a.B) *reinterpret_cast<float4*>(gout + (size_t)((b * a.H + y0 + th) * a.W + x0 + tw) * Cout + n) = *reinterpret_cast<const float4*>(ot + m * OS + c4);
+                } else if (b < a.B && n < Cout) {
                     const float4 v = *reinterpret_cast<const float4*>(ot + m * OS + c4);
                     *reinterpret_cast<float4*>(gout + (size_t)((b * (a.H << a.out_sh) + ((y0 + th) << a.out_sh) + a.out_oy) * (a.W << a.out_sh) + ((x0 + tw) << a.out_sh) + a.out_ox) * Cout + n) = v;
                 }
diff --git a/flocoder_amd/csrc/conv_pipe.hip b/flocoder_amd/csrc/conv_pipe.hip
--- a/flocoder_amd/csrc/conv_pipe.hip
+++ b/flocoder_amd/csrc/conv_pipe.hip
@@ -70,8 +70,10 @@
 
 constexpr int kFinGeomGroups = 4, kWWSlots = 8;
 
-template <int WM, int WN, int WK, int MT, int NT, int CC, int NPL, int KS, int NL, int FL = FL_ALL, int PREC = 0, int GEO = 0>
+template <int WM, int WN, int WK, int MT, int NT, int CC, int NPL, int KS, int NL, int FL = FL_ALL, int PREC = 0, int GEOF = 0, int GEOK1 = 0>
 __global__ void __launch_bounds__(256 + 64 * NL) conv_pipe_kernel(const ConvDev p_kernarg) {
+    static_assert(!(GEOF && GEOK1) && (!GEOF || (FL & FL_FIN)) && (!GEOK1 || !(FL & FL_FIN)), "one key per flavour, of its own kind");
+    constexpr int GEO = GEOF != 0 ? GEOF : GEOK1;
     ConvDev p;
     conv_params_from_lanes(p);
     constexpr int NTHR = 256 + 64 * NL, LT = 64 * NL;
@@ -103,20 +105,23 @@
     const int half = lane >> 5, l31 = lane & 31;
     const int wk = wave % WK, wn = (wave / WK) % WN, wm = wave / (WK * WN);
 
-    const int bid = conv_parity_select(p, xcd_remap(blockIdx.x, p.nblocks));
-    const int mt_i = p.ntiles == 1 ? bid : (p.magic_nt ? (int)__umulhi((unsigned)bid, p.magic_nt) : bid / p.ntiles);
-    const int nt_i = bid - mt_i * p.ntiles;
+    constexpr bool GEOC = GEO != 0, GEO1 = GEOC && !(FL & FL_FIN);
+    constexpr int G1_NT = GEO1 ? geo_cpg(GEO) * kFinGeomGroups / BN : 1;
+    static_assert(!GEO1 || (KS == 3 && geo_conv1_mask(FL) && geo_cpg(GEO) * kFinGeomGroups % BN == 0), "conv1 geometry flavours: 3x3, whole column tiles");
+    const int bid = GEO1 ? xcd_remap(blockIdx.x, p.nblocks) : conv_parity_select(p, xcd_remap(blockIdx.x, p.nblocks));
+    const int mt_i = GEO1 ? bid / G1_NT : (p.ntiles == 1 ? bid : (p.magic_nt ? (int)__umulhi((unsigned)bid, p.magic_nt) : bid / p.ntiles));
+    const int nt_i = bid - mt_i * (GEO1 ? G1_NT : p.ntiles);
     const int tx = mt_i & (p.tiles_x - 1), ty = (mt_i >> p.txl) & (p.tiles_y - 1), bg = mt_i >> (p.txl + p.tyl);
-    constexpr bool GEOC = GEO != 0;
     constexpr int BM = 32 * MT * WM;
-    static_assert(!GEOC || (!(FL & FL_CAT) && (FL & FL_XF) && geo_Tst(GEO) <= kPartPre), "geometry flavours: transform loader, one source");
+    static_assert(!GEOC || GEO1 || (!(FL & FL_CAT) && (FL & FL_XF) && geo_Tst(GEO) <= kPartPre), "Block-closing geometry flavours: transform loader, one source");
     const int g_TB = GEOC ? geo_TB(GEO) : p.TB;
     const int g_TWl = GEOC ? geo_TWl(GEO) : p.TWl;
     const int g_tbsh = GEOC ? geo_log2(BM / geo_TB(GEO)) : p.TWl + p.THl;
     const int g_THl = GEOC ? geo_log2(BM / geo_TB(GEO)) - geo_TWl(GEO) : p.THl;
     const int TW = 1 << g_TWl, TH = 1 << g_THl;
     const int b0 = bg * g_TB, y0 = ty * TH, x0 = tx * TW, n0 = nt_i * BN;
-    const int PW = p.PW, PHW = p.PH * p.PW;
+    constexpr int G1_PW = GEO1 ? (1 << geo_TWl(GEO)) + 2 : 1, G1_PHW = GEO1 ? (BM / geo_TB(GEO) / (1 << geo_TWl(GEO)) + 2) * G1_PW : 1;
+    const int PW = GEO1 ? G1_PW : p.PW, PHW = GEO1 ? G1_PHW : p.PH * p.PW;
     const int C0 = a.s0.C, C1 = a.s1.C, Cin = a.Cin, Cout = a.Cout;
     constexpr bool LEAN = FL != FL_ALL;
     const bool has_res = LEAN ? bool(FL & FL_RES) : a.res_out != nullptr;
@@ -305,7 +310,15 @@
             for (int k = 0; k < NPL; ++k) {
                 const int pix = ltid / Q + k * PIXSTEP;
                 e_po[k] = -1; e_lds[k] = -1; e_tb[k] = 0;
-                if (pix < p.P) {
+                if (GEO1) {
+                    if (pix < geo_TB(GEO) * G1_PHW) {
+                        const int tb = pix / G1_PHW, r = pix - tb * G1_PHW, py = r / G1_PW, px = r - py * G1_PW;
+                        const int iy = y0 - 1 + py, ix = x0 - 1 + px, b = b0 + tb;
+                        if (b < a.B && iy >= 0 && iy < a.Hs && ix >= 0 && ix < a.Ws) e_po[k] = (b * a.Hs + iy) * a.Ws + ix;
+                        e_lds[k] = pix * CS + (DB4 ? 8 * ((ltid % Q) >> 1) + 2 * ((ltid % Q) & 1) : q4);
+                        e_tb[k] = tb;
+                    }
+                } else if (pix < p.P) {
                     const int tb = fastdiv(pix, p.magic_phw), r = pix - tb * PHW, py = fastdiv(r, p.magic_pw), px = r - py * PW;
                     const int iy = y0 * a.stride - (a.pad_y >= 0 ? a.pad_y : a.pad) + py, ix = x0 * a.stride - (a.pad_x >= 0 ? a.pad_x : a.pad) + px, b = b0 + tb;
                     if (b < a.B && iy >= 0 && iy < Hin && ix >= 0 && ix < Win) e_po[k] = (b * a.Hs + (iy >> a.ups)) * a.Ws + (ix >> a.ups);
@@ -348,7 +361,7 @@
             }
         };
         f32x4 pv[NPL];
-        const int nk = __builtin_amdgcn_readfirstlane((p.P * Q + LT - 1) / LT);
+        const int nk = GEO1 ? (geo_TB(GEO) * G1_PHW * Q + LT - 1) / LT : __builtin_amdgcn_readfirstlane((p.P * Q + LT - 1) / LT);
         auto issue_patch = [&](int i, f32x4 (&pv)[NPL]) {
             const int c = i * CC + q4;
             const bool live = c < Cin, first = !(FL & FL_CAT) || c < C0;
@@ -437,7 +450,8 @@
         for (int mt = 0; mt < MT; ++mt) {
             const int m = (wm * MT + mt) * 32 + l31;
             const int tw = m & (TW - 1), th = (m >> g_TWl) & (TH - 1), tb = m >> g_tbsh;
-            abase[mt] = (tb * PHW + th * a.stride * PW + tw * a.stride) * CS + half;
+            const int st = GEO1 ? 1 : a.stride;
+            abase[mt] = (tb * PHW + th * st * PW + tw * st) * CS + half;
         }
         const int bbase = half * BN + wn * NT * 32 + l31;
         const int kk0 = wk * KPW;
@@ -603,7 +617,7 @@
                 }
             }
             if (has_res) {
-                const int tapoff = (a.pad * PW + a.pad) * CS;
+                const int tapoff = GEO1 ? (PW + 1) * CS : (a.pad * PW + a.pad) * CS;
 #pragma unroll
                 for (int kk = 0; kk < KPW; ++kk) {
                     const int k = 2 * (kk0 + kk);
@@ -722,14 +736,14 @@
 void conv_route_log_set(bool on) { std::lock_guard<std::mutex> lk(g_route_mu); g_route_on = on; if (on) g_route_log.clear(); }
 std::string conv_route_log_get() { std::lock_guard<std::mutex> lk(g_route_mu); return g_route_log; }
 
-template <int WM, int WN, int WK, int MT, int NT, int CC, int NPL, int KS, int NL, int FL = FL_ALL, int PREC = 0, int GEO = 0>
+template <int WM, int WN, int WK, int MT, int NT, int CC, int NPL, int KS, int NL, int FL = FL_ALL, int PREC = 0, int GEOF = 0, int GEOK1 = 0>
 static int launch_pipe(const ConvDev& d, int grid, size_t lds, hipStream_t s, int* occ) {
     if (!occ && g_route_on) {
         std::lock_guard<std::mutex> lk(g_route_mu);
-        const int v[12] = {WM, WN, WK, MT, NT, CC, NPL, KS, NL, FL, PREC, GEO};
-        for (int i = 0; i < 12; ++i) g_route_log += std::to_string(v[i]) + (i < 11 ? " " : "\n");
-    }
-    return launch_or_query((conv_pipe_kernel<WM, WN, WK, MT, NT, CC, NPL, KS, NL, FL, PREC, GEO>), 256 + 64 * NL, d, grid, lds, s, occ);
+        const int v[13] = {WM, WN, WK, MT, NT, CC, NPL, KS, NL, FL, PREC, GEOF, GEOK1};
+        for (int i = 0; i < 13; ++i) g_route_log += std::to_string(v[i]) + (i < 12 ? " " : "\n");
+    }
+    return launch_or_query((conv_pipe_kernel<WM, WN, WK, MT, NT, CC, NPL, KS, NL, FL, PREC, GEOF, GEOK1>), 256 + 64 * NL, d, grid, lds, s, occ);
 }
 
 template <int FL>
@@ -852,6 +866,58 @@
     return -1;
 }
 
+constexpr int kConv1Up = FL_STATS | FL_CAT | FL_RES;
+#define FC_CONV1_GEOMS(X)                                                                                    \
+    X(TILE_M128N32, 4, 1, 1, 1, 1, 16, 4, 0, FL_STATS, geo_key(GEO_FAST, 1, 16, 8, 8))            \
+    X(TILE_M128N32, 4, 1, 1, 1, 1, 16, 4, 0, kConv1Up, geo_key(GEO_FAST, 1, 16, 8, 8))       \
+    X(TILE_M128N32, 4, 1, 1, 1, 1, 16, 4, 0, kConv1Up, geo_key(GEO_FAST, 1, 16, 16, 2))             \
+    X(TILE_M64N32K2, 2, 1, 2, 1, 1, 32, 8, 0, FL_STATS, geo_key(GEO_FAST, 1, 16, 8, 4))           \
+    X(TILE_M64N32K2, 2, 1, 2, 1, 1, 32, 8, 0, kConv1Up, geo_key(GEO_FAST, 1, 8, 32, 1))             \
+    X(TILE_M32N32K4, 1, 1, 4, 1, 1, 32, 8, FL_W4, FL_STATS, geo_key(GEO_FAST, 1, 8, 16, 2))       \
+    X(TILE_M32N32K4, 1, 1, 4, 1, 1, 32, 8, FL_W4, FL_STATS, geo_key(GEO_PAIR, 2, 4, 32, 1))       \
+    X(TILE_M32N32K4, 1, 1, 4, 1, 1, 32, 8, FL_W4, FL_STATS, geo_key(GEO_PAIR, 2, 4, 64, 2))  \
+    X(TILE_M32N32K4, 1, 1, 4, 1, 1, 32, 8, FL_W4, kConv1Up, geo_key(GEO_PAIR, 2, 4, 64, 2))
+
+static int conv1_geo_key(const ConvDev& d, int BM, int BN, bool pair_tile) {
+    const ConvArgs& a = d.a;
+    if (a.fin.gamma || !a.stats_out || a.stats_post || a.par4 || a.stats_tmul != 1 || a.stats_toff != 0 || d.any_xf || a.out_act || a.add || d.o_out < 0) return 0;
+    if (a.KS != 3 || a.stride != 1 || a.ups || a.pad != 1 || a.pad_y >= 0 || a.pad_x >= 0 || a.out_sh || a.out_oy || a.out_ox || a.Hs != a.H || a.Ws != a.W) return 0;
+    if (d.TB != 1 && d.TB != 2) return 0;
+    if (d.rps != BM / d.TB || (1 << (d.TWl + d.THl)) * d.TB != BM) return 0;
+    const int form = (pair_tile && d.TB == 2 && d.rps == 16) ? GEO_PAIR : (d.TB == 1 ? GEO_FAST : 0);
+    if (!form) return 0;
+    const int cpg = d.cpg, NPG = cpg >= BN ? cpg / BN : 1;
+    if (cpg < 1 || (cpg & (cpg - 1)) || cpg > (1 << 15) || d.cpgt != (cpg < BN ? cpg : BN) || d.NPG != NPG) return 0;
+    const int Tst = (d.TB > 1 ? 1 : d.tiles_x * d.tiles_y) * NPG;
+    if (Tst < 1 || Tst > 63) return 0;
+    if (a.Gout != kFinGeomGroups || a.Cout != kFinGeomGroups * cpg || a.Cout % BN || d.ntiles != a.Cout / BN) return 0;
+    const int TW = 1 << d.TWl, TH = 1 << d.THl;
+    if (d.PW != TW + 2 || d.PH != TH + 2 || d.P != d.TB * d.PH * d.PW) return 0;
+    return geo_key(form, d.TB, TW, cpg, Tst);
+}
+
+static int conv1_geom_attr() {
+#define X(T, WM, WN, WK, MT, NT, CC, NL, W4, MASK, GEO)                                                                                            \
+    FC_HIP(hipFuncSetAttribute(reinterpret_cast<const void*>(&conv_pipe_kernel<WM, WN, WK, MT, NT, CC, kLeanNPL, 3, NL, (MASK) | (W4), 0, 0, GEO>),    \
+                               hipFuncAttributeMaxDynamicSharedMemorySize, 160 * 1024));                                                           \
+    FC_HIP(hipFuncSetAttribute(reinterpret_cast<const void*>(&conv_pipe_kernel<WM, WN, WK, MT, NT, CC, kLeanNPL, 3, NL, (MASK) | (W4) | FL_STAMP, 0, 0, GEO>), \
+                               hipFuncAttributeMaxDynamicSharedMemorySize, 160 * 1024));
+    FC_CONV1_GEOMS(X)
+#undef X
+    return FC_OK;
+}
+
+static int conv1_geom_launch(const ConvDev& d, int tile, bool w4, int need, int grid, size_t lds, hipStream_t s, int* occ) {
+#define X(T, WM, WN, WK, MT, NT, CC, NL, W4, MASK, GEO)                                                                                        \
+    if (tile == T && (w4 ? FL_W4 : 0) == (W4) && (need & ~FL_STAMP) == (MASK) && d.P * (CC / 4) <= 64 * NL * kLeanNPL &&                       \
+        conv1_geo_key(d, 32 * MT * WM, 32 * NT * WN, WM * MT == 1 && WN * NT == 1) == (GEO))                                                   \
+        return (need & FL_STAMP) ? launch_pipe<WM, WN, WK, MT, NT, CC, kLeanNPL, 3, NL, (MASK) | (W4) | FL_STAMP, 0, 0, GEO>(d, grid, lds, s, occ) \
+                                 : launch_pipe<WM, WN, WK, MT, NT, CC, kLeanNPL, 3, NL, (MASK) | (W4), 0, 0, GEO>(d, grid, lds, s, occ);
+    FC_CONV1_GEOMS(X)
+#undef X
+    return -1;
+}
+
 #define FC_BF3_TILES(X, KS)                \
     X(TILE_M128N32, 4, 1, 1, 1, 1, 16, KS, 4)  \
     X(TILE_M128N64, 4, 1, 1, 1, 2, 16, KS, 4)  \
@@ -903,6 +969,7 @@
 #undef X
     FC_TRY((lean_attr<2, 0>()));
     FC_TRY(fin_geom_attr());
+    FC_TRY(conv1_geom_attr());
     done = true;
     return FC_OK;
 }
@@ -936,6 +1003,7 @@
                             (!d.a.res_out || d.a.res_w4);
             const size_t lds_ww = (w4 && (need & FL_FIN)) ? ww_lds(d, tile, lds) : 0;
             if (need & FL_FIN) r = fin_geom_launch(d, tile, w4, need, grid, lds, lds_ww, s, occ);
+            else if (need & FL_STATS) r = conv1_geom_launch(d, tile, w4, need, grid, lds, s, occ);
             if (lds_ww) {
 #define X(F) if (r == -1 && need == (F)) r = lean_launch_ww<(F)>(d, tile, grid, lds_ww, s, occ);
                 FC_LEAN_FLAVOURS_3(X)
@@ -970,6 +1038,10 @@
 int conv_pipe_launch(const ConvDev& d, int tile, int grid, size_t lds, hipStream_t s) { return conv_pipe_dispatch(d, tile, grid, lds, s, nullptr); }
 
 int conv_pipe_blocks_per_cu(const ConvDev& d, int tile, size_t lds) {
+    if (!d.a.fin.gamma) {
+        int occ = 0;
+        return conv_pipe_dispatch(d, tile, 1, lds, nullptr, &occ) == FC_OK ? occ : 0;
+    }
     static std::map<std::tuple<int, int, int, size_t, int, int>, int> cache;
     static std::mutex mu;
     const int mask = (d.a.fin.gamma ? FL_FIN : 0) | (d.a.res_out ? FL_RES : 0) | (d.a.stats_post ? FL_POST : 0) | (d.any_xf ? FL_XF : 0) |
diff --git a/flocoder_amd/csrc/linattn_fused.hip b/flocoder_amd/csrc/linattn_fused.hip
--- a/flocoder_amd/csrc/linattn_fused.hip
+++ b/flocoder_amd/csrc/linattn_fused.hip
@@ -1,4 +1,5 @@
 #include <cstdlib>
+#include <mutex>
 #include <string>
 
 #include "common.h"
@@ -254,19 +255,20 @@
     }
 }
 
-template <int NQ>
+template <int NQ, int NFIX = 0>
 __device__ __forceinline__ void fetch_xh(const LaArgs& a, int b, int r0, int lane, float4 (&pre)[NQ]) {
-    const int nn = r0 + (lane & 31);
-    const float* p = a.x + ((size_t)b * a.n + nn) * (NQ * 8) + (lane >> 5) * (NQ * 4);
+    const int nn = r0 + (lane & 31), n = NFIX ? NFIX : a.n;
+    const float* p = a.x + ((size_t)b * n + nn) * (NQ * 8) + (lane >> 5) * (NQ * 4);
 #pragma unroll
     for (int j = 0; j < NQ; ++j) {
+        if (NFIX) { pre[j] = *reinterpret_cast<const float4*>(p + 4 * j); continue; }
         pre[j] = make_float4(0.f, 0.f, 0.f, 0.f);
         if (nn < a.n) pre[j] = *reinterpret_cast<const float4*>(p + 4 * j);
     }
 }
-template <int NQ>
+template <int NQ, int NFIX = 0>
 __device__ __forceinline__ void norm_xh(const LaArgs& a, const float* Ab, const float* Bb, int r0, int lane, const float4 (&pre)[NQ], float (&xn)[NQ * 4]) {
-    const bool in = r0 + (lane & 31) < a.n;
+    const bool in = NFIX ? true : r0 + (lane & 31) < a.n;
     const float* ap = Ab + (lane >> 5) * (NQ * 4);
     const float* bp = Bb + (lane >> 5) * (NQ * 4);
 #pragma unroll
@@ -278,19 +280,27 @@
     }
 }
 
-template <int NQ, int NW>
+template <int NQ, int NW, int NB = 0>
 __global__ void __launch_bounds__(64 * NW) la_ctx_fast_kernel(const LaArgs a) {
     extern __shared__ __attribute__((aligned(16))) float sm[];
     constexpr int C = NQ * 8, H2 = C / 2, NT = 64 * NW;
+    constexpr bool FIX = NB != 0;
+    constexpr int NFIX = NB * 32, ITER = FIX ? NB / NW : 1;
+    static_assert(!FIX || (NB % NW == 0 && NB >= NW), "plan-shape instantiation: whole rounds of the workgroup's waves");
     float* Ab = sm;
     float* Bb = Ab + C;
     float* Et = Bb + C;
     float* sct = Et + NW * 32 * PS;
     float* mz = sct + NW * 32;
     const int h = blockIdx.x, b = blockIdx.y, tid = threadIdx.x, lane = tid & 63, wave = tid >> 6, half = lane >> 5, l31 = lane & 31;
-    const int nblk = (a.n + 31) >> 5;
-    float4 pre[NQ];
-    if (wave < nblk) fetch_xh<NQ>(a, b, wave * 32, lane, pre);
+    const int nblk = FIX ? NB : (a.n + 31) >> 5;
+    float4 pre[ITER][NQ];
+    if constexpr (FIX) {
+#pragma unroll
+        for (int it = 0; it < ITER; ++it) fetch_xh<NQ, NFIX>(a, b, (wave + it * NW) * 32, lane, pre[it]);
+    } else {
+        if (wave < nblk) fetch_xh<NQ>(a, b, wave * 32, lane, pre[0]);
+    }
     PartPre pp;
     partials_request(a.xf, b, 0, pp);
     const float pg = tid < C ? a.xf.gamma[tid] : 0.f, pbt = tid < C ? a.xf.beta[tid] : 0.f;
@@ -313,11 +323,7 @@
 #pragma unroll
     for (int r = 0; r < 16; ++r) cacc[r] = 0.f;
     float m_run = -INFINITY, z_run = 0.f;
-    for (int rb = wave; rb < nblk; rb += NW) {
-        const int r0 = rb * 32;
-        float xn[H2];
-        norm_xh<NQ>(a, Ab, Bb, r0, lane, pre, xn);
-        if (rb + NW < nblk) fetch_xh<NQ>(a, b, r0 + 32 * NW, lane, pre);
+    auto tile = [&](const int r0, const float (&xn)[H2]) {
         f32x16 ak, av;
 #pragma unroll
         for (int r = 0; r < 16; ++r) { ak[r] = 0.f; av[r] = 0.f; }
@@ -328,14 +334,14 @@
         }
         float bm = -INFINITY;
 #pragma unroll
-        for (int r = 0; r < 16; ++r) if (r0 + acc_row(r, half) < a.n) bm = fmaxf(bm, ak[r]);
+        for (int r = 0; r < 16; ++r) if (FIX || r0 + acc_row(r, half) < a.n) bm = fmaxf(bm, ak[r]);
         bm = fmaxf(bm, __shfl_xor(bm, 32));
         const float m_new = fmaxf(m_run, bm);
         const float sc = __expf(m_run - m_new);
         float zs = 0.f;
 #pragma unroll
         for (int r = 0; r < 16; ++r) {
-            const float e = (r0 + acc_row(r, half) < a.n) ? __expf(ak[r] - m_new) : 0.f;
+            const float e = (FIX || r0 + acc_row(r, half) < a.n) ? __expf(ak[r] - m_new) : 0.f;
             zs += e;
             ak[r] = e;
         }
@@ -346,6 +352,23 @@
         for (int r = 0; r < 16; ++r) cacc[r] *= sc;
 #pragma unroll
         for (int r = 0; r < 16; ++r) cacc = FC_MFMA(av[r], ak[r], cacc);
+    };
+    if constexpr (FIX) {
+#pragma unroll
+        for (int it = 0; it < ITER; ++it) {
+            const int r0 = (wave + it * NW) * 32;
+            float xn[H2];
+            norm_xh<NQ, NFIX>(a, Ab, Bb, r0, lane, pre[it], xn);
+            tile(r0, xn);
+        }
+    } else {
+        for (int rb = wave; rb < nblk; rb += NW) {
+            const int r0 = rb * 32;
+            float xn[H2];
+            norm_xh<NQ>(a, Ab, Bb, r0, lane, pre[0], xn);
+            if (rb + NW < nblk) fetch_xh<NQ>(a, b, r0 + 32 * NW, lane, pre[0]);
+            tile(r0, xn);
+        }
     }
     if (half == 0) { mz[(wave * 2) * 32 + l31] = m_run; mz[(wave * 2 + 1) * 32 + l31] = z_run; }
     __syncthreads();
@@ -372,25 +395,29 @@
 
 constexpr int AS = 20;
 __device__ __forceinline__ int acc_reg(int row) { return (row & 3) + 4 * (row >> 3); }
-template <int NQ, int CT>
-__global__ void __launch_bounds__(256) la_apply_fast_kernel(const LaArgs a, int T, float n_t) {
+template <int NQ, int CT, int TT = 0>
+__global__ void __launch_bounds__(256) la_apply_fast_kernel(const LaArgs a, int T_rt, float n_t) {
     extern __shared__ __attribute__((aligned(16))) float sm[];
     constexpr int C = NQ * 8, H2 = C / 2, SQ = H2 + 4, WO = CT * 32;
+    constexpr bool FIX = TT != 0;
+    constexpr int NFIX = TT * 128;
+    static_assert(TT <= kPartPre, "one granule pair per tile, polled by 2 TT threads");
+    const int T = FIX ? TT : T_rt, n = FIX ? NFIX : a.n;
     float* Ab = sm;
     float* Bb = Ab + C;
     float* WqL = Bb + C;
     float* ctxL = WqL + LHEADS * 64 * SQ;
     float* WoL = ctxL + LHEADS * 64 * AS;
-    __shared__ float red[4];
+    __shared__ float red[4], red2[4];
     __shared__ unsigned epoch_s;
     __shared__ float gv[2 * kPartPre];
     const int tile = blockIdx.x, b = blockIdx.y, tid = threadIdx.x, lane = tid & 63, wave = tid >> 6, half = lane >> 5, l31 = lane & 31;
     const int r0 = tile * 128 + wave * 32, nn = r0 + l31;
-    const bool in = nn < a.n;
+    const bool in = FIX ? true : nn < a.n;
     unsigned arrival = 0;
     if (a.gran && tid == 0) arrival = __hip_atomic_fetch_add(a.sync + b, 1u, __ATOMIC_RELAXED, __HIP_MEMORY_SCOPE_AGENT);
     float4 pre[NQ];
-    fetch_xh<NQ>(a, b, r0, lane, pre);
+    fetch_xh<NQ, NFIX>(a, b, r0, lane, pre);
     PartPre pp;
     partials_request(a.xf, b, 0, pp);
     const float pg = tid < C ? a.xf.gamma[tid] : 0.f, pbt = tid < C ? a.xf.beta[tid] : 0.f;
@@ -446,11 +473,11 @@
             const float4 z = make_float4(0.f, 0.f, 0.f, 0.f);
             pbias[ct][g] = z; rs[ct][g] = z;
             if (c < C && a.bout) pbias[ct][g] = *reinterpret_cast<const float4*>(a.bout + c);
-            if (a.gran && c < C && in) rs[ct][g] = *reinterpret_cast<const float4*>(a.x + ((size_t)b * a.n + nn) * C + c);
+            if (a.gran && c < C && in) rs[ct][g] = *reinterpret_cast<const float4*>(a.x + ((size_t)b * n + nn) * C + c);
         }
     __syncthreads();
     float xn[H2];
-    norm_xh<NQ>(a, Ab, Bb, r0, lane, pre, xn);
+    norm_xh<NQ, NFIX>(a, Ab, Bb, r0, lane, pre, xn);
     const float scale = 0.17677669529663687f;
     f32x16 y[CT];
 #pragma unroll
@@ -519,8 +546,19 @@
                 S += v0; Q += v0 * v0; S += v1; Q += v1 * v1; S += v2; Q += v2 * v2; S += v3; Q += v3 * v3;
             }
         }
-    const float St = block_sum(S, red);
-    const float Qt = block_sum(Q, red);
+    float St, Qt;
+    if constexpr (FIX) {
+#pragma unroll
+        for (int o = 32; o > 0; o >>= 1) { S += __shfl_xor(S, o); Q += __shfl_xor(Q, o); }
+        __syncthreads();
+        if (lane == 0) { red[wave] = S; red2[wave] = Q; }
+        __syncthreads();
+        St = red[0] + red[1] + red[2] + red[3];
+        Qt = red2[0] + red2[1] + red2[2] + red2[3];
+    } else {
+        St = block_sum(S, red);
+        Qt = block_sum(Q, red);
+    }
     if (a.gran) {
         const unsigned epoch = epoch_s;
         float4 g2[CT][4], b2[CT][4];
@@ -572,7 +610,7 @@
                 { const float A = rstd * gg.y, Bc = bb.y - mean * A; ov.y = (A * y[ct][4 * g + 1] + Bc) + rr.y; }
                 { const float A = rstd * gg.z, Bc = bb.z - mean * A; ov.z = (A * y[ct][4 * g + 2] + Bc) + rr.z; }
                 { const float A = rstd * gg.w, Bc = bb.w - mean * A; ov.w = (A * y[ct][4 * g + 3] + Bc) + rr.w; }
-                if (in && c < C) *reinterpret_cast<float4*>(a.out + ((size_t)b * a.n + nn) * C + c) = ov;
+                if (in && c < C) *reinterpret_cast<float4*>(a.out + ((size_t)b * n + nn) * C + c) = ov;
             }
         return;
     }
@@ -587,23 +625,65 @@
 #pragma unroll
         for (int g = 0; g < 4; ++g) {
             const int c = ct * 32 + 8 * g + 4 * half;
-            if (in && c < C) *reinterpret_cast<float4*>(a.y + ((size_t)b * a.n + nn) * C + c) = make_float4(y[ct][4 * g], y[ct][4 * g + 1], y[ct][4 * g + 2], y[ct][4 * g + 3]);
+            if (in && c < C) *reinterpret_cast<float4*>(a.y + ((size_t)b * n + nn) * C + c) = make_float4(y[ct][4 * g], y[ct][4 * g + 1], y[ct][4 * g + 2], y[ct][4 * g + 3]);
         }
 }
 
 static size_t la_ctx_fast_lds(int C, int NW) { return (size_t)(2 * C + NW * 32 * PS + 32 * NW + 64 * NW) * sizeof(float); }
 static int la_ctx_waves(int n) { return n >= 256 ? 8 : 4; }
 static size_t la_apply_fast_lds(int C, int CT) { return (size_t)(2 * C + LHEADS * 64 * (C / 2 + 4) + LHEADS * 64 * AS + LHEADS * CT * 64 * AS) * sizeof(float); }
+static int la_plan_nb(int C, int n) {
+    if (C == 32 && n == 1024) return 32;
+    if (C == 32 && n == 256) return 8;
+    if (C == 64 && n == 256) return 8;
+    return 0;
+}
+static std::mutex g_la_route_mu;
+static bool g_la_route_on = false;
+static std::string g_la_route_log;
+void linattn_route_log_set(bool on) { std::lock_guard<std::mutex> lk(g_la_route_mu); g_la_route_on = on; if (on) g_la_route_log.clear(); }
+std::string linattn_route_log_get() { std::lock_guard<std::mutex> lk(g_la_route_mu); return g_la_route_log; }
+struct LaCtxSel { void (*fn)(const LaArgs); int NB; };
+struct LaApplySel { void (*fn)(const LaArgs, int, float); int TT; };
+template <int NQ>
+static LaCtxSel la_ctx_fast_for(int n) {
+    if constexpr (NQ == 4) {
+        if (la_plan_nb(NQ * 8, n) == 32) return {la_ctx_fast_kernel<NQ, 8, 32>, 32};
+        if (la_plan_nb(NQ * 8, n) == 8) return {la_ctx_fast_kernel<NQ, 8, 8>, 8};
+    }
+    if constexpr (NQ == 8) {
+        if (la_plan_nb(NQ * 8, n) == 8) return {la_ctx_fast_kernel<NQ, 8, 8>, 8};
+    }
+    if (la_ctx_waves(n) == 8) return {la_ctx_fast_kernel<NQ, 8>, 0};
+    return {la_ctx_fast_kernel<NQ, 4>, 0};
+}
+template <int NQ>
+static LaApplySel la_apply_fast_for(int n) {
+    if constexpr (NQ == 4) {
+        if (la_plan_nb(NQ * 8, n) == 32) return {la_apply_fast_kernel<NQ, 1, 8>, 8};
+        if (la_plan_nb(NQ * 8, n) == 8) return {la_apply_fast_kernel<NQ, 1, 2>, 2};
+    }
+    if constexpr (NQ == 8) {
+        if (la_plan_nb(NQ * 8, n) == 8) return {la_apply_fast_kernel<NQ, 2, 2>, 2};
+    }
+    if constexpr (NQ * 8 <= 32) return {la_apply_fast_kernel<NQ, 1>, 0};
+    else return {la_apply_fast_kernel<NQ, 2>, 0};
+}
 template <int NQ>
 static int launch_fast(const LaArgs& a, hipStream_t s) {
-    if (la_ctx_waves(a.n) == 8) hipLaunchKernelGGL((la_ctx_fast_kernel<NQ, 8>), dim3(LHEADS, a.B), dim3(512), la_ctx_fast_lds(a.C, 8), s, a);
-    else hipLaunchKernelGGL((la_ctx_fast_kernel<NQ, 4>), dim3(LHEADS, a.B), dim3(256), la_ctx_fast_lds(a.C, 4), s, a);
+    const int NW = la_ctx_waves(a.n);
+    const LaCtxSel cs = la_ctx_fast_for<NQ>(a.n);
+    const LaApplySel as = la_apply_fast_for<NQ>(a.n);
+    if (g_la_route_on) {
+        std::lock_guard<std::mutex> lk(g_la_route_mu);
+        g_la_route_log += std::to_string(a.C) + " " + std::to_string(a.n) + " " + std::to_string(cs.NB) + " " + std::to_string(as.TT) + "\n";
+    }
+    hipLaunchKernelGGL(cs.fn, dim3(LHEADS, a.B), dim3(64 * NW), la_ctx_fast_lds(a.C, NW), s, a);
     FC_HIP(hipGetLastError());
     const int T = linattn_fused_tiles(a.n);
     const float n_t = linattn_fused_nt(a.n, a.C);
     const dim3 grid(cdiv(a.n, 128), a.B);
-    if (a.C <= 32) hipLaunchKernelGGL((la_apply_fast_kernel<NQ, 1>), grid, dim3(256), la_apply_fast_lds(a.C, 1), s, a, T, n_t);
-    else hipLaunchKernelGGL((la_apply_fast_kernel<NQ, 2>), grid, dim3(256), la_apply_fast_lds(a.C, 2), s, a, T, n_t);
+    hipLaunchKernelGGL(as.fn, grid, dim3(256), la_apply_fast_lds(a.C, a.C <= 32 ? 1 : 2), s, a, T, n_t);
     FC_HIP(hipGetLastError());
     return FC_OK;
 }
@@ -613,6 +693,10 @@
     FC_HIP(hipFuncSetAttribute(reinterpret_cast<const void*>(la_ctx_fast_kernel<NQ, 8>), hipFuncAttributeMaxDynamicSharedMemorySize, 160 * 1024));
     FC_HIP(hipFuncSetAttribute(reinterpret_cast<const void*>(la_apply_fast_kernel<NQ, 1>), hipFuncAttributeMaxDynamicSharedMemorySize, 160 * 1024 - 256));
     FC_HIP(hipFuncSetAttribute(reinterpret_cast<const void*>(la_apply_fast_kernel<NQ, 2>), hipFuncAttributeMaxDynamicSharedMemorySize, 160 * 1024 - 256));
+    for (int n : {256, 1024}) {
+        FC_HIP(hipFuncSetAttribute(reinterpret_cast<const void*>(la_ctx_fast_for<NQ>(n).fn), hipFuncAttributeMaxDynamicSharedMemorySize, 160 * 1024));
+        FC_HIP(hipFuncSetAttribute(reinterpret_cast<const void*>(la_apply_fast_for<NQ>(n).fn), hipFuncAttributeMaxDynamicSharedMemorySize, 160 * 1024 - 256));
+    }
     return FC_OK;
 }
 
@@ -646,10 +730,9 @@
 }
 
 template <int NQ>
-static int apply_blocks_per_cu(int C) {
+static int apply_blocks_per_cu(int C, int n) {
     int nb = 0;
-    const hipError_t e = C <= 32 ? hipOccupancyMaxActiveBlocksPerMultiprocessor(&nb, la_apply_fast_kernel<NQ, 1>, 256, la_apply_fast_lds(C, 1))
-                                 : hipOccupancyMaxActiveBlocksPerMultiprocessor(&nb, la_apply_fast_kernel<NQ, 2>, 256, la_apply_fast_lds(C, 2));
+    const hipError_t e = hipOccupancyMaxActiveBlocksPerMultiprocessor(&nb, la_apply_fast_for<NQ>(n).fn, 256, la_apply_fast_lds(C, C <= 32 ? 1 : 2));
     return e == hipSuccess ? nb : 0;
 }
 bool linattn_fused_meeting_ok(int B, int n, int C) {
@@ -659,7 +742,7 @@
     if (linattn_fused_init() != FC_OK) return false;
     int dev = 0, cus = 0;
     if (hipGetDevice(&dev) != hipSuccess || hipDeviceGetAttribute(&cus, hipDeviceAttributeMultiprocessorCount, dev) != hipSuccess) return false;
-    const int per = C == 8 ? apply_blocks_per_cu<1>(C) : C == 16 ? apply_blocks_per_cu<2>(C) : C == 32 ? apply_blocks_per_cu<4>(C) : apply_blocks_per_cu<8>(C);
+    const int per = C == 8 ? apply_blocks_per_cu<1>(C, n) : C == 16 ? apply_blocks_per_cu<2>(C, n) : C == 32 ? apply_blocks_per_cu<4>(C, n) : apply_blocks_per_cu<8>(C, n);
     return (long long)per * cus >= (long long)T * B;
 }
 
diff --git a/flocoder_amd/csrc/unet.hip b/flocoder_amd/csrc/unet.hip
--- a/flocoder_amd/csrc/unet.hip
+++ b/flocoder_amd/csrc/unet.hip
@@ -1054,9 +1054,15 @@
     return FC_OK;
 }
 
-int fc_debug_conv_routes(int on) { conv_route_log_set(on != 0); return FC_OK; }
+int fc_debug_conv_routes(int on) { conv_route_log_set(on != 0); linattn_route_log_set(on != 0); return FC_OK; }
 int fc_debug_conv_routes_read(char* buf, int cap) {
     const std::string r = conv_route_log_get();
+    if (buf && cap > 0) { const size_t n = r.size() < (size_t)cap - 1 ? r.size() : (size_t)cap - 1; memcpy(buf, r.data(), n); buf[n] = 0; }
+    return (int)r.size();
+}
+
+int fc_debug_linattn_routes_read(char* buf, int cap) {
+    const std::string r = linattn_route_log_get();
     if (buf && cap > 0) { const size_t n = r.size() < (size_t)cap - 1 ? r.size() : (size_t)cap - 1; memcpy(buf, r.data(), n); buf[n] = 0; }
     return (int)r.size();
 }
diff --git a/include/flocoder_amd.h b/include/flocoder_amd.h
--- a/include/flocoder_amd.h
+++ b/include/flocoder_amd.h
@@ -152,6 +152,7 @@
 int fc_debug_set_conv_stamps(void* buf_dev);
 int fc_debug_conv_routes(int on);
 int fc_debug_conv_routes_read(char* buf, int cap);
+int fc_debug_linattn_routes_read(char* buf, int cap);
 int fc_debug_set_stamp_op(int op_index, void* buf_dev);
 int fc_debug_set_conv_precision(int mode);
 int fc_debug_conv(const float* src0_nhwc, int c0, const float* src1_nhwc, int c1, const float* w_oihw_dev, const float* bias_dev,
```

Result: faster. 917.1 samples/s, median of 6 (+2.6%).
